# sanje2v/DualSuperResLearningForSemSeg

Measured on AMD Instinct MI355X. Metric: stage-3 train images/sec at 256x512->512x1024, higher is better.
Workload: dtype f32; 1 GPU; DSRL stage 3 (ResNet-101 OS16 + ASPP + SSSR/SISR decoders + FA loss), full train step, random-init weights, 256x512 input -> 512x1024 logits; global_batch=8, per_gpu_batch=8, parallelism=dp1, optimizer=SGD m0.9 wd5e-4 lr0.006

## Files before the change

dualsuperreslearningforsemseg_amd/_lib.py:

```python
import ctypes as C
import os

import torch

_HERE = os.path.dirname(os.path.abspath(__file__))
LIB_PATH = os.path.join(_HERE, 'libdsrl_hip.so')

fp = C.c_void_p
i32 = C.c_int
i64 = C.c_int64
u64 = C.c_uint64
u32 = C.c_uint32
f32 = C.c_float
sz = C.c_size_t
stream_t = C.c_void_p

_conv_shape = [i32] * 10


class WgradProblem(C.Structure):
    _fields_ = [('x', C.c_void_p), ('dy', C.c_void_p), ('dw', C.c_void_p)] + [(n, C.c_int32) for n in
                ('ldx', 'lddy', 'N', 'H', 'W', 'C', 'K', 'R', 'S', 'stride', 'pad', 'dil')] + [('x_amax', C.c_void_p), ('dy_amax', C.c_void_p)]


PROTOTYPES = {
    'dsrl_version': (i32, []),
    'dsrl_last_error': (C.c_char_p, []),
    'dsrl_device_check': (i32, [C.POINTER(i32)]),
    'dsrl_conv2d_fwd_workspace_bytes': (sz, _conv_shape),
    'dsrl_conv2d_fwd': (i32, [fp, i32, fp, fp, fp, i32] + _conv_shape + [fp, sz, stream_t]),
    'dsrl_conv2d_fwd_stats_parts': (i32, _conv_shape),
    'dsrl_conv2d_fwd_stats': (i32, [fp, i32, fp, fp, fp, i32] + _conv_shape + [fp, sz, fp, i32, stream_t]),
    'dsrl_conv2d_dgrad_workspace_bytes': (sz, _conv_shape),
    'dsrl_conv2d_transposed_filter_floats': (sz, [i32] * 4),
    'dsrl_conv2d_transpose_filter': (i32, [fp, fp, i32, i32, i32, i32, stream_t]),
    'dsrl_conv2d_transpose_filters_batched': (i32, [fp, i32, i64, stream_t]),
    'dsrl_conv2d_filters_amax_segment_floats': (i32, []),
    'dsrl_conv2d_filters_amax_batched': (i32, [fp, i64, stream_t]),
    'dsrl_conv2d_dgrad': (i32, [fp, i32, fp, fp, fp, i32] + _conv_shape + [fp, sz, stream_t]),
    'dsrl_conv2d_dgrad_stats_parts': (i32, _conv_shape),
    'dsrl_conv2d_dgrad_bnstats': (i32, [fp, i32, fp, fp, fp, i32] + _conv_shape + [fp, sz, fp, i32, fp, i32, fp, fp, i32, fp, i32, i32, stream_t]),
    'dsrl_conv2d_dgrad_accumulate': (i32, [fp, i32, fp, fp, fp, i32] + _conv_shape + [fp, sz, stream_t]),
    'dsrl_conv2d_wgrad_workspace_bytes': (sz, _conv_shape),
    'dsrl_conv2d_wgrad': (i32, [fp, i32, fp, i32, fp] + _conv_shape + [fp, sz, stream_t]),
    'dsrl_conv2d_wgrad_group_table_bytes': (sz, [i32]),
    'dsrl_conv2d_wgrad_group_workspace_bytes': (sz, [fp, i32]),
    'dsrl_conv2d_wgrad_group_plan': (i32, [fp, i32, fp, sz, fp, fp, sz]),
    'dsrl_conv2d_wgrad_group_launch': (i32, [fp, fp, stream_t]),
    'dsrl_amax': (i32, [fp, i32, i64, i32, fp, stream_t]),
    'dsrl_conv2d_fwd_amax': (i32, [fp, i32, fp, fp, fp, fp, fp, fp, i32] + _conv_shape + [fp, sz, fp, i32, stream_t]),
    'dsrl_conv2d_dgrad_amax': (i32, [fp, i32, fp, fp, fp, fp, fp, fp, i32] + _conv_shape + [fp, sz, fp, i32, fp, i32, fp, fp, i32, fp, i32, i32, stream_t]),
    'dsrl_conv2d_split_filters_batched': (i32, [fp, i32, i64, stream_t]),
    'dsrl_planes_lo_offset': (sz, [i64]),
    'dsrl_planes_bytes': (sz, [i64, i32]),
    'dsrl_split_planes': (i32, [fp, i32, i64, i32, fp, fp, i32, stream_t]),
    'dsrl_conv2d_filter_planes_batched': (i32, [fp, i32, i64, stream_t]),
    'dsrl_conv2d_fwd_planes': (i32, [fp, i32, fp, fp, fp, fp, fp, fp, fp, fp, i32] + _conv_shape + [fp, sz, fp, i32, stream_t]),
    'dsrl_conv2d_dgrad_planes': (i32, [fp, i32, fp, fp, fp, fp, fp, fp, fp, fp, i32] + _conv_shape + [fp, sz, fp, i32, fp, i32, fp, fp, i32, fp, i32, i32, stream_t]),
    'dsrl_conv2d_dgrad_planes_drop': (i32, [fp, i32, fp, fp, fp, fp, fp, fp, fp, fp, i32] + _conv_shape + [fp, sz, fp, i32, fp, i32, fp, fp, i32, f32, fp, i32, i32, stream_t]),
    'dsrl_conv2d_wgrad_amax': (i32, [fp, i32, fp, fp, i32, fp, fp] + _conv_shape + [fp, sz, stream_t]),
    'dsrl_conv_precision': (i32, [i32]),
    'dsrl_conv2d_inbounds_macs': (i64, _conv_shape),
    'dsrl_conv2d_rowfold_fwd_workspace_bytes': (sz, [i32] * 9),
    'dsrl_conv2d_rowfold_fwd': (i32, [fp, i32, fp, fp, fp, i32] + [i32] * 9 + [i64, fp, sz, stream_t]),
    'dsrl_conv2d_rowfold_wgrad_workspace_bytes': (sz, [i32] * 9),
    'dsrl_conv2d_rowfold_wgrad': (i32, [fp, i32, fp, i32, fp] + [i32] * 9 + [i64, fp, sz, stream_t]),
    'dsrl_pad_image_nhwc': (i32, [fp, i64, i64, i64, i64, fp] + [i32] * 9 + [stream_t]),
    'dsrl_colsum_workspace_bytes': (sz, [i64, i32]),
    'dsrl_colsum': (i32, [fp, i32, i64, i32, fp, fp, sz, stream_t]),
    'dsrl_bn_workspace_bytes': (sz, [i64, i32]),
    'dsrl_bn_stats_floats': (sz, [i32, i32, i32]),
    'dsrl_bn_stats': (i32, [fp, i32, i64, i32, f32, f32, fp, fp, fp, fp, fp, sz, stream_t]),
    'dsrl_bn_invstd_from_var': (i32, [fp, i32, f32, fp, stream_t]),
    'dsrl_bn_apply': (i32, [fp, i32, fp, i32, i64, i32, fp, fp, fp, fp, fp, i32, i32, f32, u64, u32, fp, stream_t]),
    'dsrl_bn_fused_max_blocks': (i32, [i32]),
    'dsrl_bn_fused_barrier_timeouts': (i32, [C.POINTER(i64)]),
    'dsrl_bn_train_fwd_from_stats': (i32, [fp, i32, fp, i32, i64, i32, f32, f32, fp, fp, fp, fp, fp, fp, fp, i32, i32, f32, u64, u32, fp, i32, fp, stream_t]),
    'dsrl_bn_train_fwd': (i32, [fp, i32, fp, i32, i64, i32, f32, f32, fp, fp, fp, fp, fp, fp, fp, i32, i32, f32, u64, u32, fp, sz, fp, stream_t]),
    'dsrl_bn_bwd': (i32, [fp, i32, fp, i32, fp, i32, fp, i32, fp, i32, i64, i32, fp, fp, fp, fp, fp, i32, f32, i32, fp, sz, fp, stream_t]),
    'dsrl_bn_bwd_from_stats': (i32, [fp, i32, fp, i32, fp, i32, fp, i32, fp, i32, i64, i32, fp, fp, fp, fp, fp, i32, i32, fp, i32, fp, stream_t]),
    'dsrl_bn_bwd_from_stats_drop': (i32, [fp, i32, fp, i32, fp, i32, fp, i32, fp, i32, i64, i32, fp, fp, fp, fp, fp, i32, f32, i32, fp, i32, fp, stream_t]),
    'dsrl_bn_bwd_from_stats_res_parts': (i32, [i64, i32, i32]),
    'dsrl_bn_bwd_from_stats_res': (i32, [fp, i32, fp, i32, fp, i32, fp, i32, fp, i32, i64, i32, fp, fp, fp, fp, fp, i32, f32, i32, fp, i32, fp, fp, i32, fp, fp, fp, i32, stream_t]),
    'dsrl_dropout_fwd': (i32, [fp, i32, fp, i32, i64, i32, f32, u64, u32, stream_t]),
    'dsrl_dropout_bwd': (i32, [fp, i32, fp, i32, i64, i32, f32, u64, u32, stream_t]),
    'dsrl_bilinear_ac_fwd': (i32, [fp, i32, fp, i32, i32, i32, i32, i32, i32, i32, stream_t]),
    'dsrl_bilinear_ac_bwd_workspace_bytes': (sz, [i32] * 6),
    'dsrl_bilinear_ac_bwd': (i32, [fp, i32, fp, i32, i32, i32, i32, i32, i32, i32, fp, sz, stream_t]),
    'dsrl_global_avgpool_fwd': (i32, [fp, i32, fp, i32, i32, i32, stream_t]),
    'dsrl_global_avgpool_bwd': (i32, [fp, fp, i32, i32, i32, i32, stream_t]),
    'dsrl_maxpool3x3s2_fwd': (i32, [fp, fp, fp, i32, i32, i32, i32, stream_t]),
    'dsrl_maxpool3x3s2_bwd': (i32, [fp, fp, fp, i32, i32, i32, i32, stream_t]),
    'dsrl_convt2x2_fwd': (i32, [fp, fp, fp, fp, i32, i32, i32, i32, i32, stream_t]),
    'dsrl_convt2x2_bwd_workspace_bytes': (sz, [i32] * 5),
    'dsrl_convt2x2_bwd': (i32, [fp, fp, fp, fp, fp, fp, i32, i32, i32, i32, i32, fp, sz, stream_t]),
    'dsrl_convt2x2_fwd_ce_supported': (i32, [fp, fp, i32, i32, i32, i32, i32]),
    'dsrl_convt2x2_fwd_ce_workspace_bytes': (sz, [i32, i32, i32]),
    'dsrl_convt2x2_fwd_ce': (i32, [fp, fp, fp, fp, i32, i32, i32, i32, i32, fp, i32, fp, fp, fp, sz, stream_t]),
    'dsrl_convt2x2_bwd_ce_supported': (i32, [fp, fp, fp, i32, i32, i32, i32, i32]),
    'dsrl_convt2x2_bwd_ce': (i32, [fp, fp, fp, fp, i32, fp, fp, fp, i32, fp, fp, fp, i32, i32, i32, i32, i32, fp, sz, stream_t]),
    'dsrl_pixel_shuffle_fwd': (i32, [fp, fp, i32, i32, i32, i32, i32, stream_t]),
    'dsrl_pixel_shuffle_bwd': (i32, [fp, fp, i32, i32, i32, i32, i32, stream_t]),
    'dsrl_pointwise_strided_fwd': (i32, [fp, fp, fp, i32, i32, i32, i32, i32, stream_t]),
    'dsrl_pointwise_strided_bwd_workspace_bytes': (sz, [i32] * 5),
    'dsrl_pointwise_strided_bwd': (i32, [fp, fp, fp, fp, fp, i32, i32, i32, i32, i32, i32, fp, sz, stream_t]),
    'dsrl_copy2d': (i32, [fp, i32, fp, i32, i64, i32, stream_t]),
    'dsrl_cat_channels_supported': (i32, [fp, fp, fp, i32, fp, i32, i64]),
    'dsrl_cat_channels': (i32, [fp, fp, fp, i32, fp, i32, i64, fp, stream_t]),
    'dsrl_nchw_to_nhwc': (i32, [fp, fp, i32, i32, i32, i32, i32, stream_t]),
    'dsrl_ce_workspace_bytes': (sz, [i64]),
    'dsrl_ce_fwd': (i32, [fp, i32, fp, i64, i32, i32, fp, fp, sz, stream_t]),
    'dsrl_ce_bwd': (i32, [fp, i32, fp, i64, i32, i32, fp, fp, fp, i32, stream_t]),
    'dsrl_mse_workspace_bytes': (sz, [i64]),
    'dsrl_mse_fwd': (i32, [fp, fp, i64, fp, fp, sz, stream_t]),
    'dsrl_mse_bwd': (i32, [fp, fp, i64, fp, fp, stream_t]),
    'dsrl_ce_fused_workspace_bytes': (sz, [i64]),
    'dsrl_ce_fused': (i32, [fp, i32, fp, i64, i32, i32, fp, i32, fp, fp, fp, sz, stream_t]),
    'dsrl_mse_fused': (i32, [fp, fp, i64, f32, fp, fp, fp, fp, sz, stream_t]),
    'dsrl_loss_mix': (i32, [fp, fp, fp, f32, f32, fp, fp, stream_t]),
    'dsrl_fa_saved_floats': (sz, [i32] * 5),
    'dsrl_fa_workspace_bytes': (sz, [i32] * 5),
    'dsrl_fa_fwd': (i32, [fp, fp, i32, i32, i32, i32, i64, i64, i64, i64, i32, i32, fp, fp, fp, sz, stream_t]),
    'dsrl_fa_bwd': (i32, [fp, fp, i32, i32, i32, i32, i64, i64, i64, i64, i32, i32, fp, fp, fp, fp, fp, sz, stream_t]),
    'dsrl_seg_metrics': (i32, [fp, i32, fp, i64, i32, i32, fp, stream_t]),
    'dsrl_sssr_tail_predict_supported': (i32, [i32] * 6),
    'dsrl_sssr_tail_predict_workspace_bytes': (sz, [i32] * 3),
    'dsrl_sssr_tail_predict': (i32, [fp, i32] + [i32] * 6 + [fp] * 9 + [i32, fp, fp, fp, fp, sz, stream_t]),
    'dsrl_fingerprint_segment_words': (i32, []),
    'dsrl_fingerprint_segments': (i32, [fp, i64, fp, fp, fp, i32, stream_t]),
    'dsrl_class_map_visualize': (i32, [fp, fp, fp, fp, fp, i32, i32, i32, i32, C.c_double, stream_t]),
    'dsrl_prepare_batch': (i32, [fp, fp, fp, C.POINTER(f32), C.POINTER(f32), fp, fp, fp, i32, i32, i32, i32, i32, stream_t]),
    'dsrl_augment_geometry': (i32, [fp, fp, fp, fp, fp, fp, i32, i32, i32, stream_t]),
    'dsrl_prepare_batch_augmented': (i32, [fp, fp, fp, C.POINTER(f32), C.POINTER(f32), fp, fp, fp, i32, i32, i32, i32, i32, fp, stream_t]),
    'dsrl_sgd_step': (i32, [fp, fp, fp, i64, f32, f32, f32, f32, stream_t]),
    'dsrl_sgd_step_dev': (i32, [fp, fp, fp, i64, fp, stream_t]),
    'dsrl_sgd_step_dev_segments': (i32, [fp, fp, fp, fp, i64, fp, stream_t]),
    'dsrl_nan_check': (i32, [fp, i64, fp, stream_t]),
    'dsrl_rng_bind_device_key': (i32, [fp]),
    'dsrl_rng_advance_key': (i32, [fp, stream_t]),
    'dsrl_prof_enable': (i32, [i32]),
    'dsrl_prof_read': (i32, [i32, C.POINTER(i64), C.POINTER(C.c_double), C.POINTER(C.c_double)]),
    'dsrl_prof_read_bytes': (i32, [i32, C.POINTER(C.c_double)]),
    'dsrl_prof_kernel_name': (C.c_char_p, [i32]),
}

_lib = None


class DsrlHipError(RuntimeError):
    pass


def load():
    global _lib
    if _lib is not None:
        return _lib
    if not os.path.isfile(LIB_PATH):
        raise DsrlHipError(f'{LIB_PATH} not found: build it with `python -c "import __graft_entry__ as g; g.build()"` '
                           f'or `make -C {os.path.join(_HERE, "csrc")}` - there is no fallback path')
    lib = C.CDLL(LIB_PATH)
# ... 35 lines not shown
```

dualsuperreslearningforsemseg_amd/csrc/bn.hip:

```cpp
#include "common.h"
#include <algorithm>
#include <initializer_list>
#include <atomic>
#include <mutex>
#include <stdlib.h>

struct SeedArg { unsigned long long value; const unsigned long long* dev; };

namespace dsrl {

constexpr int kMaxRowBlocks = 256;

static int row_blocks(int64_t P) { return (int)std::max<int64_t>(1, std::min<int64_t>(kMaxRowBlocks, ceil_div(P, 32))); }

__global__ __launch_bounds__(256) void bn_partial_kernel(const float* __restrict__ x, int ld, long long P, int C, long long rows_per_block,
                                                          float* __restrict__ part, int nbx) {
    __shared__ float sh[3][256];
    const ChanMap m = chan_map(C, blockIdx.y);
    const long long row0 = blockIdx.x * rows_per_block, row1 = min(P, row0 + rows_per_block);
    float n = 0.f, s1 = 0.f, s2 = 0.f, k0 = 0.f;
    if (m.c >= 0) {
        long long p = row0 + m.slot;
        if (p < row1) k0 = x[p * ld + m.c];
#pragma unroll 4
// ... 613 lines not shown
        if (p < row1) {
            const float4 dv = LD4(dy, p, lddy, q), xv = LD4(x, p, ldx, q);
            float4 yv = make_float4(1.f, 1.f, 1.f, 1.f);
            if (need_y) yv = LD4(y, p, ldy, q);
            g[i] = make_float4(masked_grad(dv.x, yv.x, relu, drop_p, ks), masked_grad(dv.y, yv.y, relu, drop_p, ks),
                               masked_grad(dv.z, yv.z, relu, drop_p, ks), masked_grad(dv.w, yv.w, relu, drop_p, ks));
            xh[i] = make_float4((xv.x - mu[0]) * is[0], (xv.y - mu[1]) * is[1], (xv.z - mu[2]) * is[2], (xv.w - mu[3]) * is[3]);
            sg[0] += g[i].x; sgx[0] += g[i].x * xh[i].x; sg[1] += g[i].y; sgx[1] += g[i].y * xh[i].y;
            sg[2] += g[i].z; sgx[2] += g[i].z * xh[i].z; sg[3] += g[i].w; sgx[3] += g[i].w * xh[i].w;
            if (dres) ST4(dres, p, lddr, q) = g[i];
        } else {
            g[i] = make_float4(0.f, 0.f, 0.f, 0.f); xh[i] = g[i];
        }
    }
#pragma unroll
    for (int sft = 8; sft < 64; sft <<= 1) {
#pragma unroll
        for (int j = 0; j < 4; ++j) { sg[j] += __shfl_xor(sg[j], sft); sgx[j] += __shfl_xor(sgx[j], sft); }
    }
    if ((tid & 63) < 8) {
#pragma unroll
        for (int j = 0; j < 4; ++j) { shw[wave][0][j][l8] = sg[j]; shw[wave][1][j][l8] = sgx[j]; }
    }
    __syncthreads();
    if (tid < 32) {
        const int j = tid & 3, c8 = tid >> 2;
        float a = 0.f, b = 0.f;
#pragma unroll
        for (int w = 0; w < kFusedNW; ++w) { a += shw[w][0][j][c8]; b += shw[w][1][j][c8]; }
        const long long o = (long long)slab * C + grp * 32 + tid;
        st_agent(part + o, a); st_agent(part + (long long)slabs * C + o, b);
    }
    const bool arrived = grid_barrier(gridDim.x);
    {
        const int ch = tid & 31, k = tid >> 5;
        const float* pa = part + grp * 32 + ch;
        const float* pb = pa + (long long)slabs * C;
        double a = 0, b = 0;
        for (int base = k; base < slabs; base += 4 * kFusedNS) {
            float va[4], vb[4];
#pragma unroll
            for (int u = 0; u < 4; ++u) {
                const int sl = min(base + kFusedNS * u, slabs - 1);
                va[u] = ld_agent(pa + (long long)sl * C); vb[u] = ld_agent(pb + (long long)sl * C);
            }
#pragma unroll
            for (int u = 0; u < 4; ++u)
                if (base + kFusedNS * u < slabs) { a += va[u]; b += vb[u]; }
        }
        shm[k][0][ch] = a; shm[k][1][ch] = b;
    }
    __syncthreads();
    if (tid < 32) {
        double a = 0, b = 0;
#pragma unroll
        for (int k = 0; k < kFusedNS; ++k) { a += shm[k][0][tid]; b += shm[k][1][tid]; }
        const float inv_n = 1.f / (float)P;
        fin[0][tid] = !arrived ? __builtin_nanf("") : (training ? (float)a * inv_n : 0.f); fin[1][tid] = training ? (float)b * inv_n : 0.f;
        if (slab == 0) {
            const int c = grp * 32 + tid;
            if (dbeta) dbeta[c] = (float)a;
            if (dgamma) dgamma[c] = (float)b;
        }
    }
    __syncthreads();
    float gi[4], mb[4], mg[4];
#pragma unroll
    for (int j = 0; j < 4; ++j) { gi[j] = gamma[4 * q + j] * is[j]; mb[j] = fin[0][4 * l8 + j]; mg[j] = fin[1][4 * l8 + j]; }
    unsigned am = 0u;
#pragma unroll
    for (int i = 0; i < kFusedMaxPasses; ++i) {
        const int p = row0 + rr + kFusedRL * i;
        if (p >= row1) continue;
        const float4 d = make_float4(gi[0] * (g[i].x - mb[0] - xh[i].x * mg[0]), gi[1] * (g[i].y - mb[1] - xh[i].y * mg[1]),
                                     gi[2] * (g[i].z - mb[2] - xh[i].z * mg[2]), gi[3] * (g[i].w - mb[3] - xh[i].w * mg[3]));
        ST4(dx, p, lddx, q) = d;
        am = abs_bits4(am, d.x, d.y, d.z, d.w);
    }
    amax_publish(am, dx_amax);
}


constexpr int kMergeRows = 4;
template <int THREADS>
__global__ __launch_bounds__(THREADS) void bn_stats_apply_kernel(const float* __restrict__ x, int ldx, float* __restrict__ y, int ldy, int P, int C,
                                                              int groups, int rows_per_slab, float eps, float momentum,
                                                              float* __restrict__ mean_out, float* __restrict__ invstd_out, float* __restrict__ rm, float* __restrict__ rv,
                                                              const float* __restrict__ gamma, const float* __restrict__ beta,
                                                              const float* __restrict__ res, int ldr, int relu, float drop_p, SeedArg seed_arg, unsigned rng_stream,
                                                              const float* __restrict__ part, int nparts, unsigned* __restrict__ y_amax) {
    const unsigned long long seed = seed_arg.dev ? *seed_arg.dev : seed_arg.value;
    constexpr int KG = THREADS / 32, RP = THREADS / 8;
    __shared__ double shm[KG][3][32];
    __shared__ float fin[2][32];
    const int grp = blockIdx.x % groups, slab = blockIdx.x / groups;
    const int tid = threadIdx.x, l8 = tid & 7, rr = tid >> 3;
    const int q = grp * 8 + l8;
    const int row0 = slab * rows_per_slab, row1 = min(P, row0 + rows_per_slab), p0 = row0 + rr;
    float4 xv0 = make_float4(0.f, 0.f, 0.f, 0.f), rv0 = xv0;
    if (p0 < row1) {
        xv0 = LD4(x, p0, ldx, q);
        if (res) rv0 = LD4(res, p0, ldr, q);
    }
    float gmv[4], btv[4];
#pragma unroll
    for (int j = 0; j < 4; ++j) { gmv[j] = gamma[4 * q + j]; btv[j] = beta[4 * q + j]; }
    {
        const int ch = tid & 31, k = tid >> 5;
        const float* pn = part + grp * 32 + ch;
        const float* pm_ = pn + (long long)nparts * C;
        const float* pq = pn + 2ll * nparts * C;
        const float mref = pm_[0];
        double N = 0, S = 0, T = 0;
        struct Batch { float n[kMergeRows], m[kMergeRows], q[kMergeRows]; };
        auto fetch = [&](int base, Batch& b) {
#pragma unroll
            for (int u = 0; u < kMergeRows; ++u) {
                const int sl = min(base + KG * u, nparts - 1);
                b.n[u] = pn[(long long)sl * C]; b.m[u] = pm_[(long long)sl * C]; b.q[u] = pq[(long long)sl * C];
            }
        };
        auto sum = [&](int base, const Batch& b) {
#pragma unroll
            for (int u = 0; u < kMergeRows; ++u) {
                const double nb = base + KG * u < nparts ? (double)b.n[u] : 0.0, d = (double)b.m[u] - (double)mref;
                N += nb; S += nb * d; T += (base + KG * u < nparts ? (double)b.q[u] : 0.0) + nb * d * d;
            }
        };
        Batch b0, b1;
        fetch(k, b0);
        for (int base = k; base < nparts; base += 2 * KG * kMergeRows) {
            const int mid = base + KG * kMergeRows;
            if (mid < nparts) fetch(mid, b1);
            sum(base, b0);
            if (mid < nparts) {
                if (mid + KG * kMergeRows < nparts) fetch(mid + KG * kMergeRows, b0);
                sum(mid, b1);
            }
        }
        shm[k][0][ch] = N; shm[k][1][ch] = S; shm[k][2][ch] = T;
        if (k == 0) fin[0][ch] = mref;
    }
    __syncthreads();
    if (tid < 32) {
        double N = 0, S = 0, T = 0;
#pragma unroll
        for (int k = 0; k < KG; ++k) { N += shm[k][0][tid]; S += shm[k][1][tid]; T += shm[k][2][tid]; }
        const double mu = N > 0 ? (double)fin[0][tid] + S / N : 0.0;
        const double Q = N > 0 ? fmax(T - S * S / N, 0.0) : 0.0;
        const double var = N > 0 ? Q / N : 0.0;
        const float is = (float)(1.0 / sqrt(var + (double)eps));
        fin[0][tid] = (float)mu; fin[1][tid] = is;
        if (slab == 0) {
            const int c = grp * 32 + tid;
            mean_out[c] = (float)mu; invstd_out[c] = is;
            if (rm) rm[c] = (float)((1.0 - momentum) * rm[c] + momentum * mu);
            if (rv) rv[c] = (float)((1.0 - momentum) * rv[c] + momentum * (N > 1 ? Q / (N - 1) : var));
        }
    }
    __syncthreads();
    float sc[4], sf[4];
#pragma unroll
    for (int j = 0; j < 4; ++j) { sc[j] = gmv[j] * fin[1][4 * l8 + j]; sf[j] = btv[j] - fin[0][4 * l8 + j] * sc[j]; }
    const float ks = drop_p > 0.f ? 1.f / (1.f - drop_p) : 1.f;
    unsigned am = 0u;
    auto row = [&](int p, const float4 xv, const float4 r) {
        float v[4] = {fmaf(xv.x, sc[0], sf[0]), fmaf(xv.y, sc[1], sf[1]), fmaf(xv.z, sc[2], sf[2]), fmaf(xv.w, sc[3], sf[3])};
        if (res) { v[0] += r.x; v[1] += r.y; v[2] += r.z; v[3] += r.w; }
        if (relu) {
#pragma unroll
            for (int j = 0; j < 4; ++j) v[j] = fmaxf(v[j], 0.f);
        }
        if (drop_p > 0.f) {
            const unsigned long long e = (unsigned long long)p * C + 4ull * q;
            unsigned r4[4];
            philox4x32_10((unsigned)(e >> 2), (unsigned)(e >> 34), rng_stream, 0u, (unsigned)seed, (unsigned)(seed >> 32), r4);
#pragma unroll
            for (int j = 0; j < 4; ++j) v[j] = ((float)(r4[j] >> 8) * 5.9604644775390625e-08f >= drop_p) ? v[j] * ks : 0.f;
        }
        ST4(y, p, ldy, q) = make_float4(v[0], v[1], v[2], v[3]);
        am = abs_bits4(am, v[0], v[1], v[2], v[3]);
    };
    if (p0 < row1) row(p0, xv0, rv0);
#pragma unroll 4
    for (int p = p0 + RP; p < row1; p += RP) {
        const float4 xv = LD4(x, p, ldx, q);
        float4 r = xv;
        if (res) r = LD4(res, p, ldr, q);
        row(p, xv, r);
    }
    amax_publish(am, y_amax);
}


constexpr int kStatsReduced = 32;
__global__ __launch_bounds__(256) void bn_stats_reduce_kernel(const float* __restrict__ part, int nparts, int C, float* __restrict__ out) {
    __shared__ double shm[8][3][32];
    __shared__ float ref[32];
    const int grp = blockIdx.x, rrow = blockIdx.y, tid = threadIdx.x, ch = tid & 31, k = tid >> 5;
    const int per = (nparts + kStatsReduced - 1) / kStatsReduced, p0 = rrow * per, p1 = min(nparts, p0 + per);
    const float* pn = part + grp * 32 + ch;
    const float* pm_ = pn + (long long)nparts * C;
    const float* pq = pn + 2ll * nparts * C;
    const float mref = p0 < p1 ? pm_[(long long)p0 * C] : 0.f;
    double N = 0, S = 0, T = 0;
    for (int base = p0 + k; base < p1; base += 32) {
        float vn[4], vm[4], vq[4];
#pragma unroll
        for (int u = 0; u < 4; ++u) {
            const int sl = min(base + 8 * u, p1 - 1);
            vn[u] = pn[(long long)sl * C]; vm[u] = pm_[(long long)sl * C]; vq[u] = pq[(long long)sl * C];
        }
#pragma unroll
        for (int u = 0; u < 4; ++u)
            if (base + 8 * u < p1) {
                const double nb = (double)vn[u], d = (double)vm[u] - (double)mref;
                N += nb; S += nb * d; T += (double)vq[u] + nb * d * d;
            }
    }
    shm[k][0][ch] = N; shm[k][1][ch] = S; shm[k][2][ch] = T;
    if (k == 0) ref[ch] = mref;
    __syncthreads();
    if (tid < 32) {
        N = S = T = 0;
#pragma unroll
        for (int kk = 0; kk < 8; ++kk) { N += shm[kk][0][tid]; S += shm[kk][1][tid]; T += shm[kk][2][tid]; }
        const double mu = N > 0 ? (double)ref[tid] + S / N : 0.0, Q = N > 0 ? fmax(T - S * S / N, 0.0) : 0.0;
        float* o = out + (long long)rrow * C + grp * 32 + tid;
        o[0] = (float)N; o[(long long)kStatsReduced * C] = (float)mu; o[2ll * kStatsReduced * C] = (float)Q;
    }
}
__global__ __launch_bounds__(256) void bn_bwd_stats_reduce_kernel(const float* __restrict__ part, int nparts, int C, float* __restrict__ out) {
    __shared__ double shm[8][2][32];
    const int grp = blockIdx.x, rrow = blockIdx.y, tid = threadIdx.x, ch = tid & 31, k = tid >> 5;
    const int per = (nparts + kStatsReduced - 1) / kStatsReduced, p0 = rrow * per, p1 = min(nparts, p0 + per);
    const float* pa = part + grp * 32 + ch;
    const float* pb = pa + (long long)nparts * C;
    double a = 0, b = 0;
    for (int base = p0 + k; base < p1; base += 32) {
        float va[4], vb[4];
#pragma unroll
        for (int u = 0; u < 4; ++u) {
            const int sl = min(base + 8 * u, p1 - 1);
            va[u] = pa[(long long)sl * C]; vb[u] = pb[(long long)sl * C];
        }
#pragma unroll
        for (int u = 0; u < 4; ++u)
            if (base + 8 * u < p1) { a += (double)va[u]; b += (double)vb[u]; }
    }
    shm[k][0][ch] = a; shm[k][1][ch] = b;
    __syncthreads();
    if (tid < 32) {
        a = b = 0;
#pragma unroll
        for (int kk = 0; kk < 8; ++kk) { a += shm[kk][0][tid]; b += shm[kk][1][tid]; }
        float* o = out + (long long)rrow * C + grp * 32 + tid;
        o[0] = (float)a; o[(long long)kStatsReduced * C] = (float)b;
    }
}

struct BnRes2 { const float* x; int ldx; const float* mean; const float* invstd; float* part; int nslabs; };
template <int THREADS, bool RES2 = false>
__global__ __launch_bounds__(THREADS) void bn_bwd_stats_apply_kernel(const float* __restrict__ x, int ldx, const float* __restrict__ y, int ldy,
                                                                  const float* __restrict__ dy, int lddy, float* __restrict__ dx, int lddx,
                                                                  float* __restrict__ dres, int lddr, int P, int C, int groups, int rows_per_slab,
                                                                  const float* __restrict__ mean, const float* __restrict__ invstd, const float* __restrict__ gamma,
                                                                  float* __restrict__ dgamma, float* __restrict__ dbeta, int relu, int training,
                                                                  const float* __restrict__ part, int nparts, unsigned* __restrict__ dx_amax, float ks, const BnRes2 r2) {
    constexpr int KG = THREADS / 32, RP = THREADS / 8;
    __shared__ double shm[KG][2][32];
    __shared__ float fin[2][32];
    const int grp = blockIdx.x % groups, slab = blockIdx.x / groups;
    const int tid = threadIdx.x, l8 = tid & 7, rr = tid >> 3;
    const int q = grp * 8 + l8;
    const int row0 = slab * rows_per_slab, row1 = min(P, row0 + rows_per_slab), p0 = row0 + rr;
    float4 dv0 = make_float4(0.f, 0.f, 0.f, 0.f), xv0 = dv0, yv0 = make_float4(1.f, 1.f, 1.f, 1.f), x2v0 = dv0;
    if (p0 < row1) {
        dv0 = LD4(dy, p0, lddy, q); xv0 = LD4(x, p0, ldx, q);
        if (relu) yv0 = LD4(y, p0, ldy, q);
        if constexpr (RES2) x2v0 = LD4(r2.x, p0, r2.ldx, q);
    }
    float mu2[4] = {0.f, 0.f, 0.f, 0.f}, is2[4] = {0.f, 0.f, 0.f, 0.f}, sg2[4] = {0.f, 0.f, 0.f, 0.f}, sgx2[4] = {0.f, 0.f, 0.f, 0.f};
    if constexpr (RES2) {
#pragma unroll
        for (int j = 0; j < 4; ++j) { mu2[j] = r2.mean[4 * q + j]; is2[j] = r2.invstd[4 * q + j]; }
    }
    float mu[4], is[4], gi[4];
#pragma unroll
    for (int j = 0; j < 4; ++j) { mu[j] = mean[4 * q + j]; is[j] = invstd[4 * q + j]; gi[j] = gamma[4 * q + j]; }
    {
        const int ch = tid & 31, k = tid >> 5;
        const float* pa = part + grp * 32 + ch;
        const float* pb = pa + (long long)nparts * C;
        double a = 0, b = 0;
        struct Batch { float a[kMergeRows], b[kMergeRows]; };
        auto fetch = [&](int base, Batch& t) {
#pragma unroll
            for (int u = 0; u < kMergeRows; ++u) {
                const int sl = min(base + KG * u, nparts - 1);
                t.a[u] = pa[(long long)sl * C]; t.b[u] = pb[(long long)sl * C];
            }
        };
        auto sum = [&](int base, const Batch& t) {
#pragma unroll
            for (int u = 0; u < kMergeRows; ++u)
                if (base + KG * u < nparts) { a += t.a[u]; b += t.b[u]; }
        };
        Batch b0, b1;
        fetch(k, b0);
        for (int base = k; base < nparts; base += 2 * KG * kMergeRows) {
            const int mid = base + KG * kMergeRows;
            if (mid < nparts) fetch(mid, b1);
            sum(base, b0);
            if (mid < nparts) {
                if (mid + KG * kMergeRows < nparts) fetch(mid + KG * kMergeRows, b0);
                sum(mid, b1);
            }
        }
        shm[k][0][ch] = a; shm[k][1][ch] = b;
    }
    __syncthreads();
    if (tid < 32) {
        double a = 0, b = 0;
#pragma unroll
        for (int k = 0; k < KG; ++k) { a += shm[k][0][tid]; b += shm[k][1][tid]; }
        const float inv_n = 1.f / (float)P;
        fin[0][tid] = training ? (float)a * inv_n : 0.f; fin[1][tid] = training ? (float)b * inv_n : 0.f;
        if (slab == 0) {
            const int c = grp * 32 + tid;
            if (dbeta) dbeta[c] = (float)a;
            if (dgamma) dgamma[c] = (float)b;
        }
    }
    __syncthreads();
    float mb[4], mg[4];
#pragma unroll
    for (int j = 0; j < 4; ++j) { gi[j] *= is[j]; mb[j] = fin[0][4 * l8 + j]; mg[j] = fin[1][4 * l8 + j]; }
    unsigned am = 0u;
    auto row = [&](int p, const float4 dv, const float4 xv, const float4 yv, const float4 x2v) {
        const float g0 = masked_grad(dv.x, yv.x, relu, 0.f, ks), g1 = masked_grad(dv.y, yv.y, relu, 0.f, ks);
        const float g2 = masked_grad(dv.z, yv.z, relu, 0.f, ks), g3 = masked_grad(dv.w, yv.w, relu, 0.f, ks);
        const float4 d = make_float4(gi[0] * (g0 - mb[0] - (xv.x - mu[0]) * is[0] * mg[0]), gi[1] * (g1 - mb[1] - (xv.y - mu[1]) * is[1] * mg[1]),
                                     gi[2] * (g2 - mb[2] - (xv.z - mu[2]) * is[2] * mg[2]), gi[3] * (g3 - mb[3] - (xv.w - mu[3]) * is[3] * mg[3]));
        ST4(dx, p, lddx, q) = d;
        am = abs_bits4(am, d.x, d.y, d.z, d.w);
        if (dres) ST4(dres, p, lddr, q) = make_float4(g0, g1, g2, g3);
        if constexpr (RES2) {
            sg2[0] += g0; sgx2[0] += g0 * ((x2v.x - mu2[0]) * is2[0]);
            sg2[1] += g1; sgx2[1] += g1 * ((x2v.y - mu2[1]) * is2[1]);
            sg2[2] += g2; sgx2[2] += g2 * ((x2v.z - mu2[2]) * is2[2]);
            sg2[3] += g3; sgx2[3] += g3 * ((x2v.w - mu2[3]) * is2[3]);
        }
    };
    if (p0 < row1) row(p0, dv0, xv0, yv0, x2v0);
#pragma unroll 2
    for (int p = p0 + RP; p < row1; p += RP) {
        const float4 dv = LD4(dy, p, lddy, q), xv = LD4(x, p, ldx, q);
        float4 yv = make_float4(1.f, 1.f, 1.f, 1.f);
        if (relu) yv = LD4(y, p, ldy, q);
        float4 x2v = xv;
        if constexpr (RES2) x2v = LD4(r2.x, p, r2.ldx, q);
        row(p, dv, xv, yv, x2v);
    }
    if constexpr (RES2) {
        __shared__ float r2s[THREADS / 64][2][32];
#pragma unroll
        for (int sft = 8; sft < 64; sft <<= 1)
#pragma unroll
            for (int j = 0; j < 4; ++j) { sg2[j] += __shfl_xor(sg2[j], sft); sgx2[j] += __shfl_xor(sgx2[j], sft); }
        if ((tid & 63) < 8) {
#pragma unroll
            for (int j = 0; j < 4; ++j) { r2s[tid >> 6][0][4 * l8 + j] = sg2[j]; r2s[tid >> 6][1][4 * l8 + j] = sgx2[j]; }
        }
        __syncthreads();
        if (tid < 64) {
            const int v = tid >> 5, c = tid & 31;
            float t = 0.f;
#pragma unroll
            for (int w = 0; w < THREADS / 64; ++w) t += r2s[w][v][c];
            r2.part[((long long)v * r2.nslabs + slab) * C + grp * 32 + c] = t;
        }
    }
    amax_publish(am, dx_amax);
}

constexpr int kFlatThreads = 512;
__device__ inline void flat_reduce(float (*sh)[4 * kFlatThreads], float (*sh2)[kFlatThreads], int nv, int C, int T, int phase0, float* out) {
    const int t = threadIdx.x, G = kFlatThreads / C, c = t % C, r = t / C;
    __syncthreads();
    if (r < G) {
        const int e0 = (c - phase0 + C) % C;
        for (int v = 0; v < nv; ++v) {
            float a = 0.f;
            for (int e = e0 + C * r; e < 4 * T; e += C * G) a += sh[v][e];
            sh2[v][r * C + c] = a;
        }
    }
    __syncthreads();
    const int G2 = G > 16 ? 16 : G;
    if (G > 16 && r < 16) {
        for (int v = 0; v < nv; ++v) {
            float a = 0.f;
            for (int q = r; q < G; q += 16) a += sh2[v][q * C + c];
            sh[v][r * C + c] = a;
        }
    }
    __syncthreads();
    if (t < C)
        for (int v = 0; v < nv; ++v) {
            float a = 0.f;
            for (int q = 0; q < G2; ++q) a += (G > 16 ? sh[v][q * C + t] : sh2[v][q * C + t]);
            out[v] = a;
        }
}
__global__ __launch_bounds__(kFlatThreads) void bn_partial_flat_kernel(const float* __restrict__ x, long long total4, long long P, int C, int T,
                                                                      long long per_block4, float* __restrict__ part, int nbx) {
    __shared__ float sh[3][4 * kFlatThreads];
    __shared__ float sh2[3][kFlatThreads];
    const int t = threadIdx.x;
    const long long b0 = min(total4, blockIdx.x * per_block4), b1 = min(total4, b0 + per_block4);
    const long long r0 = min(P - 1, (4 * b0) / C);
    const int phase0 = (int)((4 * b0) % C);
    float n = 0.f, s1[4] = {0.f, 0.f, 0.f, 0.f}, s2[4] = {0.f, 0.f, 0.f, 0.f};
    if (t < T) {
        float k0[4];
#pragma unroll
        for (int k = 0; k < 4; ++k) k0[k] = x[r0 * C + (phase0 + 4 * t + k) % C];
        const float4* x4 = reinterpret_cast<const float4*>(x);
#pragma unroll 4
        for (long long f = b0 + t; f < b1; f += T) {
            const float4 v = x4[f];
            const float d0 = v.x - k0[0], d1 = v.y - k0[1], d2 = v.z - k0[2], d3 = v.w - k0[3];
            s1[0] += d0; s2[0] += d0 * d0; s1[1] += d1; s2[1] += d1 * d1; s1[2] += d2; s2[2] += d2 * d2; s1[3] += d3; s2[3] += d3 * d3;
            n += 1.f;
        }
    }
#pragma unroll
    for (int k = 0; k < 4; ++k) { sh[0][4 * t + k] = n; sh[1][4 * t + k] = s1[k]; sh[2][4 * t + k] = s2[k]; }
    float tot[3];
    flat_reduce(sh, sh2, 3, C, T, phase0, tot);
    if (t < C) {
        float mean = 0.f, m2 = 0.f;
// ... 198 lines not shown
    if (int e = bind_stream_device(st)) return e;
    const int nbx = row_blocks(P);
    const long long rpb = ceil_div(P, nbx);
    if (vec4_ok(C, {ldx}, {x}))
        hipLaunchKernelGGL(bn_partial4_kernel, dim3(nbx, (unsigned)ceil_div(C / 4, 256)), dim3(256), 0, st, x, ldx, (long long)P, C, rpb, (float*)ws, nbx);
    else if (const int T = flat_stride(C, P, {ldx}, {x}))
        hipLaunchKernelGGL(bn_partial_flat_kernel, dim3(nbx), dim3(kFlatThreads), 0, st, x, (long long)(P * C / 4), (long long)P, C, T,
                           (long long)ceil_div(P * C / 4, (int64_t)nbx), (float*)ws, nbx);
    else
        hipLaunchKernelGGL(bn_partial_kernel, dim3(nbx, (unsigned)ceil_div(C, 256)), dim3(256), 0, st, x, ldx, (long long)P, C, rpb, (float*)ws, nbx);
    if (int e = launch_status("bn_partial_kernel")) return e;
    hipLaunchKernelGGL(bn_finalize_kernel, dim3((unsigned)ceil_div(C, 8)), dim3(256), 0, st, (const float*)ws, nbx, C, eps, momentum, mean, invstd, running_mean, running_var);
    return launch_status("bn_finalize_kernel");
}

extern "C" int dsrl_bn_invstd_from_var(const float* running_var, int C, float eps, float* invstd, dsrl_stream_t stream) {
    DSRL_REQUIRE(running_var && invstd && C > 0, DSRL_E_BADARG, "bn_invstd_from_var: bad arguments");
    hipStream_t st = (hipStream_t)stream;
    if (int e = bind_stream_device(st)) return e;
    hipLaunchKernelGGL(invstd_from_var_kernel, dim3((unsigned)ceil_div(C, 256)), dim3(256), 0, st, running_var, C, eps, invstd);
    return launch_status("invstd_from_var_kernel");
}

extern "C" int dsrl_bn_apply(const float* x, int ldx, float* y, int ldy, int64_t P, int C, const float* mean, const float* invstd,
                             const float* gamma, const float* beta, const float* residual, int ldr, int relu, float drop_p,
                             uint64_t seed, uint32_t rng_stream, uint32_t* y_amax, dsrl_stream_t stream) {
    DSRL_REQUIRE(x && y && mean && invstd && gamma && beta && P > 0 && C > 0 && ldx >= C && ldy >= C, DSRL_E_BADARG, "bn_apply: bad arguments");
    DSRL_REQUIRE(drop_p >= 0.f && drop_p < 1.f, DSRL_E_BADARG, "bn_apply: dropout p=%f outside [0,1)", drop_p);
    hipStream_t st = (hipStream_t)stream;
    if (int e = bind_stream_device(st)) return e;
    if (vec4_ok(C, {ldx, ldy, residual ? ldr : 0}, {x, y, residual}))
        hipLaunchKernelGGL(bn_apply4_kernel, apply_grid4(P, C), dim3(256), 0, st, x, ldx, y, ldy, (long long)P, C, mean, invstd, gamma, beta, residual, ldr,
                           relu, drop_p, seed_arg(seed), (unsigned)rng_stream, y_amax);
    else if (const int T = flat_stride(C, P, {ldx, ldy, residual ? ldr : C}, {x, y, residual}))
        hipLaunchKernelGGL(bn_apply_flat_kernel, dim3((unsigned)std::max<int64_t>(1, std::min<int64_t>(2048, ceil_div(P * C / 4, (int64_t)T * 2)))), dim3(kFlatThreads), 0, st,
                           x, y, (long long)(P * C / 4), C, T, mean, invstd, gamma, beta, residual, relu, drop_p, seed_arg(seed), (unsigned)rng_stream, y_amax);
    else
        hipLaunchKernelGGL(bn_apply_kernel, apply_grid(P, C), dim3(256), 0, st, x, ldx, y, ldy, (long long)P, C, mean, invstd, gamma, beta, residual, ldr,
                           relu, drop_p, seed_arg(seed), (unsigned)rng_stream, y_amax);
    return launch_status("bn_apply_kernel");
}

extern "C" int dsrl_bn_fused_max_blocks(int max_blocks) {
    const int prev = g_fused_max_blocks.load();
    if (max_blocks >= -1) g_fused_max_blocks.store(max_blocks);
    return prev;
}

extern "C" int dsrl_bn_fused_barrier_timeouts(int64_t* count) {
    DSRL_REQUIRE(count, DSRL_E_BADARG, "bn_fused_barrier_timeouts: null pointer");
    unsigned int v = 0;
    if (hipMemcpyFromSymbol(&v, HIP_SYMBOL(g_grid_timeouts), sizeof(v)) != hipSuccess) return launch_status("hipMemcpyFromSymbol(g_grid_timeouts)");
    *count = (int64_t)v;
    static unsigned int seen[64] = {0};
    int dev = 0;
    if (hipGetDevice(&dev) != hipSuccess || dev < 0 || dev >= 64) dev = 0;
    if (v != seen[dev]) {
        const unsigned int zero = 0u;
        if (hipMemcpyToSymbol(HIP_SYMBOL(g_grid_count), &zero, sizeof(zero)) != hipSuccess) return launch_status("hipMemcpyToSymbol(g_grid_count)");
        seen[dev] = v;
    }
    return DSRL_OK;
}

extern "C" int dsrl_bn_train_fwd(const float* x, int ldx, float* y, int ldy, int64_t P, int C, float eps, float momentum, float* mean, float* invstd,
                                 float* running_mean, float* running_var, const float* gamma, const float* beta, const float* residual, int ldr,
                                 int relu, float drop_p, uint64_t seed, uint32_t rng_stream, void* ws, size_t ws_bytes, uint32_t* y_amax, dsrl_stream_t stream) {
    DSRL_REQUIRE(x && y && mean && invstd && gamma && beta && ws && P > 0 && C > 0 && ldx >= C && ldy >= C, DSRL_E_BADARG, "bn_train_fwd: bad arguments");
    DSRL_REQUIRE(drop_p >= 0.f && drop_p < 1.f, DSRL_E_BADARG, "bn_train_fwd: dropout p=%f outside [0,1)", drop_p);
    DSRL_REQUIRE(ws_bytes >= dsrl_bn_workspace_bytes(P, C), DSRL_E_WORKSPACE, "bn_train_fwd: workspace too small");
    const FusedPlan f = fused_plan(P, C);
    if (f.ok && vec4_ok(C, {ldx, ldy, residual ? ldr : 0}, {x, y, residual}) && bind_stream_device((hipStream_t)stream) == DSRL_OK &&
        fused_stream_ok((hipStream_t)stream)) {
        hipStream_t st = (hipStream_t)stream;
        hipLaunchKernelGGL(bn_fused_fwd_kernel, dim3(f.blocks), dim3(kFusedThreads), 0, st, x, ldx, y, ldy, (int)P, C, f.groups, f.slabs, f.rows_per_slab, eps, momentum,
                           mean, invstd, running_mean, running_var, gamma, beta, residual, ldr, relu, drop_p, seed_arg(seed), (unsigned)rng_stream,
                           (float*)ws, y_amax);
        return launch_status("bn_fused_fwd_kernel");
    }
    if (int e = dsrl_bn_stats(x, ldx, P, C, eps, momentum, mean, invstd, running_mean, running_var, ws, ws_bytes, stream)) return e;
    return dsrl_bn_apply(x, ldx, y, ldy, P, C, mean, invstd, gamma, beta, residual, ldr, relu, drop_p, seed, rng_stream, y_amax, stream);
}

extern "C" int dsrl_bn_train_fwd_from_stats(const float* x, int ldx, float* y, int ldy, int64_t P, int C, float eps, float momentum, float* mean, float* invstd,
                                            float* running_mean, float* running_var, const float* gamma, const float* beta, const float* residual, int ldr,
                                            int relu, float drop_p, uint64_t seed, uint32_t rng_stream, float* stats, int stats_parts, uint32_t* y_amax,
                                            dsrl_stream_t stream) {
    DSRL_REQUIRE(x && y && mean && invstd && gamma && beta && stats && P > 0 && P < (1ll << 31) && C > 0 && ldx >= C && ldy >= C, DSRL_E_BADARG, "bn_train_fwd_from_stats: bad arguments");
    DSRL_REQUIRE(stats_parts > 0 && stats_parts <= 4096, DSRL_E_BADARG, "bn_train_fwd_from_stats: %d row blocks of partials (1..4096)", stats_parts);
    DSRL_REQUIRE(C % 32 == 0 && vec4_ok(C, {ldx, ldy, residual ? ldr : 0}, {x, y, residual}), DSRL_E_UNSUPPORTED,
                 "bn_train_fwd_from_stats: C (%d) must be a multiple of 32, strides multiples of 4, pointers 16-byte aligned", C);
    DSRL_REQUIRE(drop_p >= 0.f && drop_p < 1.f, DSRL_E_BADARG, "bn_train_fwd_from_stats: dropout p=%f outside [0,1)", drop_p);
    hipStream_t st = (hipStream_t)stream;
    if (int e = bind_stream_device(st)) return e;
    const int groups = C / 32;
    if (stats_parts > 256) {
        float* red = stats + 3ll * stats_parts * C;
        hipLaunchKernelGGL(bn_stats_reduce_kernel, dim3((unsigned)groups, kStatsReduced), dim3(256), 0, st, (const float*)stats, stats_parts, C, red);
        if (int e = launch_status("bn_stats_reduce_kernel")) return e;
        stats = red; stats_parts = kStatsReduced;
    }
    const int T = stats_apply_threads(P, C, stats_parts), rows_per_slab = stats_apply_rows(P, groups, T), slabs = (int)ceil_div(P, (int64_t)rows_per_slab);
    auto go = [&](auto kern) {
        hipLaunchKernelGGL(kern, dim3((unsigned)(groups * slabs)), dim3(T), 0, st, x, ldx, y, ldy, (int)P, C, groups, rows_per_slab, eps, momentum,
                           mean, invstd, running_mean, running_var, gamma, beta, residual, ldr, relu, drop_p, seed_arg(seed), (unsigned)rng_stream, stats, stats_parts, y_amax);
    };
    if (T == 1024) go(bn_stats_apply_kernel<1024>); else if (T == 512) go(bn_stats_apply_kernel<512>); else go(bn_stats_apply_kernel<256>);
    return launch_status("bn_stats_apply_kernel");
}

extern "C" int dsrl_bn_bwd(const float* x, int ldx, const float* y, int ldy, const float* dy, int lddy, float* dx, int lddx,
                           float* dresidual, int lddr, int64_t P, int C, const float* mean, const float* invstd, const float* gamma,
                           float* dgamma, float* dbeta, int relu, float drop_p, int training, void* ws, size_t ws_bytes, uint32_t* dx_amax, dsrl_stream_t stream) {
    DSRL_REQUIRE(x && dy && dx && mean && invstd && gamma && ws && P > 0 && C > 0, DSRL_E_BADARG, "bn_bwd: bad arguments");
    DSRL_REQUIRE(y || !(relu || drop_p > 0.f), DSRL_E_BADARG, "bn_bwd: forward output needed for the relu/dropout mask");
    DSRL_REQUIRE(ws_bytes >= dsrl_bn_workspace_bytes(P, C), DSRL_E_WORKSPACE, "bn_bwd: workspace too small");
    hipStream_t st = (hipStream_t)stream;
    if (int e = bind_stream_device(st)) return e;
    const bool v4 = vec4_ok(C, {ldx, y ? ldy : 0, lddy, lddx, dresidual ? lddr : 0}, {x, y, dy, dx, dresidual});
    const FusedPlan f = fused_plan(P, C);
    if (f.ok && v4 && fused_stream_ok(st)) {
        hipLaunchKernelGGL(bn_fused_bwd_kernel, dim3(f.blocks), dim3(kFusedThreads), 0, st, x, ldx, y, ldy, dy, lddy, dx, lddx, dresidual, lddr, (int)P, C,
                           f.groups, f.slabs, f.rows_per_slab, mean, invstd, gamma, dgamma, dbeta, relu, drop_p, training, (float*)ws, dx_amax);
        return launch_status("bn_fused_bwd_kernel");
    }
    const int nbx = row_blocks(P);
    const long long rpb = ceil_div(P, nbx);
    float* part = (float*)ws;
    float* sums = part + 3ll * nbx * C;
    if (v4)
        hipLaunchKernelGGL(bn_bwd_partial4_kernel, dim3(nbx, (unsigned)ceil_div(C / 4, 256)), dim3(256), 0, st, x, ldx, y, ldy, dy, lddy, (long long)P, C, rpb,
                           mean, invstd, relu, drop_p, part, nbx);
    else if (const int T = flat_stride(C, P, {ldx, y ? ldy : C, lddy}, {x, y, dy}))
        hipLaunchKernelGGL(bn_bwd_partial_flat_kernel, dim3(nbx), dim3(kFlatThreads), 0, st, x, y, dy, (long long)(P * C / 4), C, T,
                           (long long)ceil_div(P * C / 4, (int64_t)nbx), mean, invstd, relu, drop_p, part, nbx);
    else
        hipLaunchKernelGGL(bn_bwd_partial_kernel, dim3(nbx, (unsigned)ceil_div(C, 256)), dim3(256), 0, st, x, ldx, y, ldy, dy, lddy, (long long)P, C, rpb,
                           mean, invstd, relu, drop_p, part, nbx);
    if (int e = launch_status("bn_bwd_partial_kernel")) return e;
    hipLaunchKernelGGL(bn_bwd_finalize_kernel, dim3((unsigned)ceil_div(C, 8)), dim3(256), 0, st, (const float*)part, nbx, C, sums, dgamma, dbeta);
    if (int e = launch_status("bn_bwd_finalize_kernel")) return e;
    if (v4)
        hipLaunchKernelGGL(bn_bwd_apply4_kernel, apply_grid4(P, C), dim3(256), 0, st, x, ldx, y, ldy, dy, lddy, dx, lddx, dresidual, lddr, (long long)P, C,
                           mean, invstd, gamma, (const float*)sums, relu, drop_p, training, dx_amax);
    else
        hipLaunchKernelGGL(bn_bwd_apply_kernel, apply_grid(P, C), dim3(256), 0, st, x, ldx, y, ldy, dy, lddy, dx, lddx, dresidual, lddr, (long long)P, C,
                           mean, invstd, gamma, (const float*)sums, relu, drop_p, training, dx_amax);
    return launch_status("bn_bwd_apply_kernel");
}

extern "C" int dsrl_bn_bwd_from_stats(const float* x, int ldx, const float* y, int ldy, const float* dy, int lddy, float* dx, int lddx,
                                      float* dresidual, int lddr, int64_t P, int C, const float* mean, const float* invstd, const float* gamma,
                                      float* dgamma, float* dbeta, int relu, int training, float* stats, int stats_parts, uint32_t* dx_amax,
                                      dsrl_stream_t stream) {
    return dsrl_bn_bwd_from_stats_drop(x, ldx, y, ldy, dy, lddy, dx, lddx, dresidual, lddr, P, C, mean, invstd, gamma, dgamma, dbeta, relu, 0.f, training, stats, stats_parts,
                                       dx_amax, stream);
}
static int bwd_from_stats_slabs(int64_t P, int C, int stats_parts) {
    const int parts = stats_parts > 256 ? kStatsReduced : stats_parts, groups = C / 32, T = stats_apply_threads(P, C, parts);
    return (int)ceil_div(P, (int64_t)stats_apply_rows(P, groups, T));
}
extern "C" int dsrl_bn_bwd_from_stats_res_parts(int64_t P, int C, int stats_parts) {
    return (P > 0 && P < (1ll << 31) && C > 0 && C % 32 == 0 && stats_parts > 0 && stats_parts <= 4096) ? bwd_from_stats_slabs(P, C, stats_parts) : 0;
}
static int bn_bwd_from_stats_impl(const float* x, int ldx, const float* y, int ldy, const float* dy, int lddy, float* dx, int lddx,
                                  float* dresidual, int lddr, int64_t P, int C, const float* mean, const float* invstd, const float* gamma,
                                  float* dgamma, float* dbeta, int relu, float drop_p, int training, float* stats, int stats_parts, uint32_t* dx_amax,
                                  dsrl_stream_t stream, const BnRes2* res2);
extern "C" int dsrl_bn_bwd_from_stats_drop(const float* x, int ldx, const float* y, int ldy, const float* dy, int lddy, float* dx, int lddx,
                                           float* dresidual, int lddr, int64_t P, int C, const float* mean, const float* invstd, const float* gamma,
                                           float* dgamma, float* dbeta, int relu, float drop_p, int training, float* stats, int stats_parts, uint32_t* dx_amax,
                                           dsrl_stream_t stream) {
    return bn_bwd_from_stats_impl(x, ldx, y, ldy, dy, lddy, dx, lddx, dresidual, lddr, P, C, mean, invstd, gamma, dgamma, dbeta, relu, drop_p, training, stats, stats_parts,
                                  dx_amax, stream, nullptr);
}
extern "C" int dsrl_bn_bwd_from_stats_res(const float* x, int ldx, const float* y, int ldy, const float* dy, int lddy, float* dx, int lddx,
                                          float* dresidual, int lddr, int64_t P, int C, const float* mean, const float* invstd, const float* gamma,
                                          float* dgamma, float* dbeta, int relu, float drop_p, int training, float* stats, int stats_parts, uint32_t* dx_amax,
                                          const float* res_x, int res_ldx, const float* res_mean, const float* res_invstd, float* res_stats, int res_parts,
                                          dsrl_stream_t stream) {
    DSRL_REQUIRE(dresidual && res_x && res_mean && res_invstd && res_stats && res_ldx >= C && res_ldx % 4 == 0 && ((uintptr_t)res_x % 16) == 0, DSRL_E_BADARG,
                 "bn_bwd_from_stats_res: the residual branch's input / statistics / partials buffer are required (stride a multiple of 4, 16-byte aligned)");
    DSRL_REQUIRE(res_parts > 0 && res_parts == dsrl_bn_bwd_from_stats_res_parts(P, C, stats_parts), DSRL_E_BADARG,
                 "bn_bwd_from_stats_res: this launch writes %d row blocks of sums, the caller expects %d (dsrl_bn_bwd_from_stats_res_parts)",
                 dsrl_bn_bwd_from_stats_res_parts(P, C, stats_parts), res_parts);
    const BnRes2 r2{res_x, res_ldx, res_mean, res_invstd, res_stats, res_parts};
    return bn_bwd_from_stats_impl(x, ldx, y, ldy, dy, lddy, dx, lddx, dresidual, lddr, P, C, mean, invstd, gamma, dgamma, dbeta, relu, drop_p, training, stats, stats_parts,
                                  dx_amax, stream, &r2);
}
static int bn_bwd_from_stats_impl(const float* x, int ldx, const float* y, int ldy, const float* dy, int lddy, float* dx, int lddx,
                                  float* dresidual, int lddr, int64_t P, int C, const float* mean, const float* invstd, const float* gamma,
                                  float* dgamma, float* dbeta, int relu, float drop_p, int training, float* stats, int stats_parts, uint32_t* dx_amax,
                                  dsrl_stream_t stream, const BnRes2* res2) {
    DSRL_REQUIRE(drop_p >= 0.f && drop_p < 1.f && (drop_p == 0.f || relu), DSRL_E_BADARG, "bn_bwd_from_stats_drop: dropout p=%f needs the ReLU mask (y > 0)", drop_p);
    const float ks = drop_p > 0.f ? 1.f / (1.f - drop_p) : 1.f;
    DSRL_REQUIRE(x && dy && dx && mean && invstd && gamma && stats && P > 0 && P < (1ll << 31) && C > 0, DSRL_E_BADARG, "bn_bwd_from_stats: bad arguments");
    DSRL_REQUIRE(y || !relu, DSRL_E_BADARG, "bn_bwd_from_stats: forward output needed for the relu mask");
    DSRL_REQUIRE(stats_parts > 0 && stats_parts <= 4096, DSRL_E_BADARG, "bn_bwd_from_stats: %d row blocks of partials (1..4096)", stats_parts);
    DSRL_REQUIRE(C % 32 == 0 && vec4_ok(C, {ldx, y ? ldy : 0, lddy, lddx, dresidual ? lddr : 0}, {x, y, dy, dx, dresidual}), DSRL_E_UNSUPPORTED,
                 "bn_bwd_from_stats: C (%d) must be a multiple of 32, strides multiples of 4, pointers 16-byte aligned", C);
    hipStream_t st = (hipStream_t)stream;
    if (int e = bind_stream_device(st)) return e;
    const int groups = C / 32;
    if (stats_parts > 256) {
        float* red = stats + 2ll * stats_parts * C;
        hipLaunchKernelGGL(bn_bwd_stats_reduce_kernel, dim3((unsigned)groups, kStatsReduced), dim3(256), 0, st, (const float*)stats, stats_parts, C, red);
        if (int e = launch_status("bn_bwd_stats_reduce_kernel")) return e;
        stats = red; stats_parts = kStatsReduced;
    }
    const int T = stats_apply_threads(P, C, stats_parts), rows_per_slab = stats_apply_rows(P, groups, T), slabs = (int)ceil_div(P, (int64_t)rows_per_slab);
    BnRes2 r2{};
    if (res2) { r2 = *res2; DSRL_REQUIRE(r2.nslabs == slabs, DSRL_E_BADARG, "bn_bwd_from_stats_res: %d slabs launched, %d expected", slabs, r2.nslabs); }
    auto go = [&](auto kern) {
        hipLaunchKernelGGL(kern, dim3((unsigned)(groups * slabs)), dim3(T), 0, st, x, ldx, y, ldy, dy, lddy, dx, lddx, dresidual, lddr, (int)P, C,
                           groups, rows_per_slab, mean, invstd, gamma, dgamma, dbeta, relu, training, stats, stats_parts, dx_amax, ks, r2);
    };
    if (res2) { if (T == 1024) go(bn_bwd_stats_apply_kernel<1024, true>); else if (T == 512) go(bn_bwd_stats_apply_kernel<512, true>); else go(bn_bwd_stats_apply_kernel<256, true>); }
    else if (T == 1024) go(bn_bwd_stats_apply_kernel<1024>); else if (T == 512) go(bn_bwd_stats_apply_kernel<512>); else go(bn_bwd_stats_apply_kernel<256>);
    return launch_status("bn_bwd_stats_apply_kernel");
}

extern "C" int dsrl_colsum(const float* x, int ld, int64_t P, int C, float* out, void* ws, size_t ws_bytes, dsrl_stream_t stream) {
    DSRL_REQUIRE(x && out && ws && P > 0 && C > 0 && ld >= C, DSRL_E_BADARG, "colsum: bad arguments");
    DSRL_REQUIRE(ws_bytes >= dsrl_colsum_workspace_bytes(P, C), DSRL_E_WORKSPACE, "colsum: workspace too small");
    hipStream_t st = (hipStream_t)stream;
    if (int e = bind_stream_device(st)) return e;
    const int nbx = row_blocks(P);
    if (vec4_ok(C, {ld}, {x}))
        hipLaunchKernelGGL(colsum_partial4_kernel, dim3(nbx, (unsigned)ceil_div(C / 4, 256)), dim3(256), 0, st, x, ld, (long long)P, C, (long long)ceil_div(P, nbx), (float*)ws);
    else
        hipLaunchKernelGGL(colsum_partial_kernel, dim3(nbx, (unsigned)ceil_div(C, 256)), dim3(256), 0, st, x, ld, (long long)P, C, (long long)ceil_div(P, nbx), (float*)ws);
    if (int e = launch_status("colsum_partial_kernel")) return e;
    hipLaunchKernelGGL(colsum_finalize_kernel, dim3((unsigned)ceil_div(C, 32)), dim3(256), 0, st, (const float*)ws, nbx, C, out);
    return launch_status("colsum_finalize_kernel");
}

__global__ void rng_advance_kernel(unsigned long long* state) {
    if (threadIdx.x == 0 && blockIdx.x == 0) { state[1] += 1ull; state[0] = state[2] * 1000003ull + state[1]; }
}
extern "C" int dsrl_rng_bind_device_key(const uint64_t* dev_key) {
    int dev = 0;
    if (hipGetDevice(&dev) != hipSuccess || dev < 0 || dev >= 64) { set_error("rng_bind_device_key: no current HIP device"); (void)hipGetLastError(); return DSRL_E_LAUNCH; }
    g_rng_dev_key[dev].store((const unsigned long long*)dev_key);
    return DSRL_OK;
}
extern "C" int dsrl_rng_advance_key(uint64_t* state, dsrl_stream_t stream) {
    DSRL_REQUIRE(state && ((uintptr_t)state % 8) == 0, DSRL_E_BADARG, "rng_advance_key: state must be three 8-byte aligned 64-bit words on the device");
    hipStream_t st = (hipStream_t)stream;
    if (int e = bind_stream_device(st)) return e;
    hipLaunchKernelGGL(rng_advance_kernel, dim3(1), dim3(64), 0, st, (unsigned long long*)state);
    return launch_status("rng_advance_kernel");
}

namespace dsrl {
__global__ __launch_bounds__(256) void dropout_flat4_kernel(const float4* __restrict__ x, float4* __restrict__ y, unsigned total4, float p_drop, SeedArg seed_arg,
                                                             unsigned rng_stream) {
    const unsigned long long seed = seed_arg.dev ? *seed_arg.dev : seed_arg.value;
    const float ks = 1.f / (1.f - p_drop);
    for (unsigned i = blockIdx.x * 256u + threadIdx.x; i < total4; i += gridDim.x * 256u) {
        const float4 v = x[i];
        unsigned r[4];
        philox4x32_10(i, 0u, rng_stream, 0u, (unsigned)seed, (unsigned)(seed >> 32), r);
        float4 o;
        o.x = ((float)(r[0] >> 8) * 5.9604644775390625e-08f >= p_drop) ? v.x * ks : 0.f;
        o.y = ((float)(r[1] >> 8) * 5.9604644775390625e-08f >= p_drop) ? v.y * ks : 0.f;
        o.z = ((float)(r[2] >> 8) * 5.9604644775390625e-08f >= p_drop) ? v.z * ks : 0.f;
        o.w = ((float)(r[3] >> 8) * 5.9604644775390625e-08f >= p_drop) ? v.w * ks : 0.f;
        y[i] = o;
    }
}
}

static int dropout_common(const float* x, int ldx, float* y, int ldy, int64_t P, int C, float p, uint64_t seed, uint32_t rng_stream, dsrl_stream_t stream) {
    DSRL_REQUIRE(x && y && P > 0 && C > 0 && p >= 0.f && p < 1.f, DSRL_E_BADARG, "dropout: bad arguments");
    hipStream_t st = (hipStream_t)stream;
    if (int e = bind_stream_device(st)) return e;
    const long long total = (long long)P * C;
    if (ldx == C && ldy == C && total % 4 == 0 && total / 4 < (1ll << 32) && ((uintptr_t)x % 16) == 0 && ((uintptr_t)y % 16) == 0) {
        hipLaunchKernelGGL(dropout_flat4_kernel, dim3((unsigned)std::min<long long>(ceil_div(total / 4, 256), 8192)), dim3(256), 0, st, reinterpret_cast<const float4*>(x),
                           reinterpret_cast<float4*>(y), (unsigned)(total / 4), p, seed_arg(seed), (unsigned)rng_stream);
        return launch_status("dropout_flat4_kernel");
    }
// ... 11 lines not shown
```

dualsuperreslearningforsemseg_amd/csrc/conv_common.h:

```cpp
#pragma once
#include "common.h"

namespace dsrl {

using f32x16 = __attribute__((ext_vector_type(16))) float;
using bf16x8 = __attribute__((ext_vector_type(8))) __bf16;
using bf16x4 = __attribute__((ext_vector_type(4))) __bf16;
using f16x8 = __attribute__((ext_vector_type(8))) _Float16;
using f16x4 = __attribute__((ext_vector_type(4))) _Float16;

template <bool F16> struct Plane;
template <> struct Plane<false> {
    using v4 = bf16x4; using v8 = bf16x8;
    static __device__ __forceinline__ v4 cvt(const float* r) { return v4{(__bf16)r[0], (__bf16)r[1], (__bf16)r[2], (__bf16)r[3]}; }
    static __device__ __forceinline__ void residual(float* r, v4 t) {
#pragma unroll
        for (int e = 0; e < 4; ++e) r[e] -= (float)t[e];
    }
    static __device__ __forceinline__ f32x16 mfma(v8 a, v8 b, f32x16 c) { return __builtin_amdgcn_mfma_f32_32x32x16_bf16(a, b, c, 0, 0, 0); }
};
__device__ __forceinline__ float f16_resid_lo(unsigned t, float r) { float d; asm("v_fma_mix_f32 %0, %1, -1.0, %2 op_sel:[0,0,0] op_sel_hi:[1,0,0]" : "=v"(d) : "v"(t), "v"(r)); return d; }
__device__ __forceinline__ float f16_resid_hi(unsigned t, float r) { float d; asm("v_fma_mix_f32 %0, %1, -1.0, %2 op_sel:[1,0,0] op_sel_hi:[1,0,0]" : "=v"(d) : "v"(t), "v"(r)); return d; }
template <> struct Plane<true> {
    using v4 = f16x4; using v8 = f16x8;
    using f32x4 = __attribute__((ext_vector_type(4))) float;
    using u32x2 = __attribute__((ext_vector_type(2))) unsigned;
    static __device__ __forceinline__ v4 cvt(const float* r) { return __builtin_convertvector((f32x4{r[0], r[1], r[2], r[3]}), v4); }
    static __device__ __forceinline__ void residual(float* r, v4 t) {
        const u32x2 u = __builtin_bit_cast(u32x2, t);
        r[0] = f16_resid_lo(u.x, r[0]); r[1] = f16_resid_hi(u.x, r[1]); r[2] = f16_resid_lo(u.y, r[2]); r[3] = f16_resid_hi(u.y, r[3]);
    }
    static __device__ __forceinline__ f32x16 mfma(v8 a, v8 b, f32x16 c) { return __builtin_amdgcn_mfma_f32_32x32x16_f16(a, b, c, 0, 0, 0); }
};
__device__ __forceinline__ int amax_shift_of(unsigned fetched) {
    const unsigned u = amax_reduce(fetched);
    int ex = (int)((u >> 23) & 0xffu);
    if (ex == 0) ex = 1;
    return 14 - (ex - 127);
}
__device__ __forceinline__ int amax_shift(const unsigned* p) { return amax_shift_of(amax_fetch(p)); }

__device__ __forceinline__ int fast_div(int n, unsigned m, unsigned s) {
    const int q = (int)(__umulhi((unsigned)n, m) >> (s & 31u));
    return s == 255u ? n : q;
}

struct ConvArgs {
    const float* x; const float* w; const float* bias; float* y;
    int ldx, ldy;
    int N, H, W, C;
    int K;
    int R, S, Ho, Wo;
    int stride, pad, dil;
    int M;
    int cchunks;
    int splits;
    long long slab;
    unsigned x_bytes, w_bytes, y_bytes;
    int mtiles, ntiles, xcd_remap;
    int kg;
    int accumulate;
    float* stats;
    const float* bn_x; const float* bn_y; const float* bn_mean; const float* bn_invstd; float* bstats;
    int bn_ldx, bn_ldy, bn_relu;
    float bn_gscale;
    int bn_fast;
    int par, Hh, Wh, pbm;
    const unsigned* amax_a; const unsigned* amax_b;
    int w_split;
    unsigned mHW, sHW, mW, sW, mNT, sNT;
    unsigned a_lo, b_lo;
    int planes;
    float* coop_slab; unsigned* tickets;
};
constexpr int kCoopMaxTiles = (kAmaxShardStride - 1) * kAmaxShards;
__host__ __device__ inline int coop_ticket_word(int t) { return kAmaxShardStride * (t / (kAmaxShardStride - 1)) + 1 + t % (kAmaxShardStride - 1); }
__device__ __forceinline__ int dgrad_pix(const ConvArgs& a, int m) {
    const int t = m / a.pbm, p2 = a.par * a.par, c = t % p2, j = (t / p2) * a.pbm + (m - t * a.pbm);
    const int hw = a.Hh * a.Wh, n = j / hw, r = j - n * hw, hh = r / a.Wh, wh = r - hh * a.Wh;
    const int ph = c / a.par, pw = c - ph * a.par;
    return (n * a.Ho + hh * a.par + ph) * a.Wo + wh * a.par + pw;
}

__device__ inline int xcd_contiguous(int bid, int n) {
    const int q = n / kNumXCD, r = n % kNumXCD, xcd = bid % kNumXCD, local = bid / kNumXCD;
    return (xcd < r ? xcd * (q + 1) : r * (q + 1) + (xcd - r) * q) + local;
}

using u32x4 = __attribute__((ext_vector_type(4))) unsigned int;
constexpr unsigned kOOB = 0x80000000u;
__device__ inline float4 buf_load4(__amdgpu_buffer_rsrc_t r, unsigned off) {
    const u32x4 v = __builtin_amdgcn_raw_buffer_load_b128(r, (int)off, 0, 0);
    return make_float4(__uint_as_float(v.x), __uint_as_float(v.y), __uint_as_float(v.z), __uint_as_float(v.w));
}

struct WgradArgs {
    const float* x; const float* dy; float* dw;
    int ldx, lddy;
    int N, H, W, C, K, R, S, Ho, Wo, stride, pad, dil;
    long long P;
    unsigned x_bytes, dy_bytes;
    int ctiles;
    int psplits;
    long long slab;
    int taps[64]; int ntaps;
    int xcd_remap;
    int kctiles;
    unsigned mHW, sHW, mW, sW;
    int kg;
    int nblocks;
    float* dw_final;
    int rblocks;
    const unsigned* amax_dy; const unsigned* amax_x;
    int no_ident;
};

bool wgrad3_eligible(int N, int H, int W, int C, int K, int R, int S, int stride, int pad, int dil, int npl, bool f16);
void wgrad3_tile(int& bm, int& bn);
int launch_wgrad3(const WgradArgs& a, int npl, hipStream_t st);
int launch_wgrad3_group(const WgradArgs* table, const int* starts, int nprob, int grid, int npl, int dil, hipStream_t st);

bool planes_cfg_supported(int cfg, int kg);
int launch_planes_igemm(const ConvArgs& a, int cfg, bool dgrad, hipStream_t st);
bool sk_supported(int cfg, int kg, int npl, bool f16, bool w_split);
size_t sk_lds_bytes();
int launch_sk_igemm(const ConvArgs& a, bool dgrad, bool str1, int npl, hipStream_t st);
__host__ __device__ inline long long planes_lo_offset(long long elems) { return (elems * 2 + 255) / 256 * 256; }

}
```

dualsuperreslearningforsemseg_amd/csrc/conv_igemm.hip:

```cpp
#include "common.h"
#include "conv_common.h"
#include <algorithm>
#include <atomic>
#include <stdlib.h>
#include <string.h>
#include <mutex>
#include <vector>

namespace dsrl {

static std::atomic<int> g_conv_precision{-1};
constexpr int BK = 32;
constexpr int LDS_LD = 36;

template <int MR, int NR, int WGM, int WGN, bool DGRAD, int MINW = 2, bool = false>
__global__ __launch_bounds__(256, MINW) void conv_igemm_f32_kernel(const ConvArgs a) {
    constexpr int BM = 32 * MR * WGM, BN = 32 * NR * WGN;
    constexpr int A_IT = BM / 32, B_IT = BN / 32;
    extern __shared__ __attribute__((aligned(16))) float smem[];

    const int tid = threadIdx.x;
    const int lane = tid & 63;
    const int wave = __builtin_amdgcn_readfirstlane(tid >> 6);
    const int wm = wave / WGN, wn = wave % WGN;
// ... 1386 lines not shown
        const long long total = (long long)p.M * K;
        if (stats != nullptr) {
            DSRL_REQUIRE(fwd_stats_parts(p, conv_planes(PASS_FWD)) == stats_parts && stats_parts > 0 && ldy % 4 == 0 && ((uintptr_t)y % 16) == 0 &&
                         (bias == nullptr || ((uintptr_t)bias % 16) == 0), DSRL_E_BADARG,
                         "conv2d_fwd_stats: this split-K launch writes %d row blocks of partials (ldy a multiple of 4, y 16-byte aligned), the caller expects %d",
                         fwd_stats_parts(p, conv_planes(PASS_FWD)), stats_parts);
            hipLaunchKernelGGL(splitk_reduce_stats_kernel, dim3((unsigned)(stats_parts * (K / 32))), dim3(256), 0, st,
                               (const float*)ws, p.splits, a.slab, p.M, K, bias, y, ldy, stats);
            return launch_status("splitk_reduce_stats_kernel");
        }
        hipLaunchKernelGGL(splitk_reduce_kernel, dim3((unsigned)std::min<long long>(ceil_div(total, 256), 4096)), dim3(256), 0, st,
                           (const float*)ws, p.splits, a.slab, p.M, K, bias, y, ldy);
        return launch_status("splitk_reduce_kernel");
    }
    if (stats != nullptr) {
        DSRL_REQUIRE(fwd_stats_parts(p, conv_planes(PASS_FWD)) == stats_parts && stats_parts > 0, DSRL_E_BADARG,
                     "conv2d_fwd_stats: this launch writes %d row blocks of partials, the caller expects %d (dsrl_conv2d_fwd_stats_parts)",
                     fwd_stats_parts(p, conv_planes(PASS_FWD)), stats_parts);
        a.stats = stats;
    }
    a.y = y; a.ldy = ldy; a.bias = bias;
    return launch_igemm<false>(a, p.cfg, st);
}

extern "C" int dsrl_conv2d_fwd(const float* x, int ldx, const float* w, const float* bias, float* y, int ldy,
                               int N, int H, int W, int C, int K, int R, int S, int stride, int pad, int dil,
                               void* ws, size_t ws_bytes, dsrl_stream_t stream) {
    return fwd_impl(x, ldx, w, bias, y, ldy, N, H, W, C, K, R, S, stride, pad, dil, ws, ws_bytes, stream, nullptr, 0);
}
extern "C" int dsrl_conv2d_fwd_stats(const float* x, int ldx, const float* w, const float* bias, float* y, int ldy,
                                     int N, int H, int W, int C, int K, int R, int S, int stride, int pad, int dil,
                                     void* ws, size_t ws_bytes, float* stats, int stats_parts, dsrl_stream_t stream) {
    DSRL_REQUIRE(stats != nullptr, DSRL_E_BADARG, "conv2d_fwd_stats: null statistics buffer");
    return fwd_impl(x, ldx, w, bias, y, ldy, N, H, W, C, K, R, S, stride, pad, dil, ws, ws_bytes, stream, stats, stats_parts);
}

static int pad4(int v) { return (v + 3) & ~3; }
static size_t dgrad_wt_bytes(int C, int K, int R, int S) { return align_up((size_t)C * pad4(K) * R * S * sizeof(float), 256); }

extern "C" size_t dsrl_conv2d_dgrad_workspace_bytes(int N, int H, int W, int C, int K, int R, int S, int stride, int pad, int dil) {
    const int Ho = out_size(H, R, stride, pad, dil), Wo = out_size(W, S, stride, pad, dil);
    if (Ho <= 0 || Wo <= 0) return 0;
    return with_amax_scratch(dgrad_wt_bytes(C, K, R, S) + plan_fwd_ws(N, Ho, Wo, pad4(K), C, R, S, H, W));
}

extern "C" size_t dsrl_conv2d_transposed_filter_floats(int C, int K, int R, int S) { return (size_t)C * R * S * pad4(K); }
extern "C" int dsrl_conv2d_transpose_filter(const float* w, float* wt, int C, int K, int R, int S, dsrl_stream_t stream) {
    DSRL_REQUIRE(w && wt && C > 0 && K > 0 && R > 0 && S > 0, DSRL_E_BADARG, "conv2d_transpose_filter: bad arguments");
    hipStream_t st = (hipStream_t)stream;
    if (int e = bind_stream_device(st)) return e;
    const int Kp = pad4(K);
    hipLaunchKernelGGL(weight_transpose_kernel, dim3((unsigned)ceil_div(C, 32), (unsigned)ceil_div(Kp, 32), (unsigned)(R * S)), dim3(256), 0, st, w, wt, K, Kp, R * S, C);
    return launch_status("weight_transpose_kernel");
}

extern "C" int dsrl_conv2d_split_filters_batched(const int64_t* table, int n, int64_t total_tiles, dsrl_stream_t stream) {
    DSRL_REQUIRE(table && n > 0 && total_tiles > 0 && total_tiles < (1ll << 31), DSRL_E_BADARG, "conv2d_split_filters_batched: bad arguments");
    hipStream_t st = (hipStream_t)stream;
    if (int e = bind_stream_device(st)) return e;
    hipLaunchKernelGGL(weight_split_batched_kernel, dim3((unsigned)ceil_div(total_tiles, (int64_t)kWtTilesPerBlock)), dim3(256), 0, st, (const long long*)table, n,
                       (long long)total_tiles);
    return launch_status("weight_split_batched_kernel");
}

extern "C" int dsrl_conv2d_transpose_filters_batched(const int64_t* table, int n, int64_t total_tiles, dsrl_stream_t stream) {
    DSRL_REQUIRE(table && n > 0 && total_tiles > 0 && total_tiles < (1ll << 31), DSRL_E_BADARG, "conv2d_transpose_filters_batched: bad arguments");
    hipStream_t st = (hipStream_t)stream;
    if (int e = bind_stream_device(st)) return e;
    hipLaunchKernelGGL(weight_transpose_batched_kernel, dim3((unsigned)ceil_div(total_tiles, (int64_t)kWtTilesPerBlock)), dim3(256), 0, st, (const long long*)table, n,
                       (long long)total_tiles);
    return launch_status("weight_transpose_batched_kernel");
}

extern "C" int dsrl_conv2d_filters_amax_segment_floats(void) { return kAmaxSegFloats; }
extern "C" int dsrl_conv2d_filters_amax_batched(const int64_t* table, int64_t nseg, dsrl_stream_t stream) {
    DSRL_REQUIRE(table && nseg > 0 && nseg < (1ll << 31), DSRL_E_BADARG, "conv2d_filters_amax_batched: bad arguments");
    hipStream_t st = (hipStream_t)stream;
    if (int e = bind_stream_device(st)) return e;
    hipLaunchKernelGGL(weight_amax_batched_kernel, dim3((unsigned)nseg), dim3(256), 0, st, (const long long*)table);
    return launch_status("weight_amax_batched_kernel");
}

struct DgradBn { const float* x; const float* y; const float* mean; const float* invstd; float* stats; int ldx, ldy, relu; float gscale = 1.f; };
static int dgrad_impl(const float* dy, int lddy, const float* w, const float* wt_in, float* dx, int lddx,
                      int N, int H, int W, int C, int K, int R, int S, int stride, int pad, int dil,
                      void* ws, size_t ws_bytes, dsrl_stream_t stream, int accumulate, const DgradBn* bn = nullptr,
                      const unsigned* dy_amax = nullptr, const unsigned* w_amax = nullptr, const void* wt_split = nullptr,
                      const void* dy_planes = nullptr, const void* wt_planes = nullptr) {
    if (int e = check_conv(dy, w, dx, N, H, W, C, K, R, S, stride, pad, dil)) return e;
    const int Kp = pad4(K);
    DSRL_REQUIRE(lddy % 4 == 0 && ((uintptr_t)dy % 16) == 0, DSRL_E_UNSUPPORTED,
                 "conv2d_dgrad: lddy (%d) must be a multiple of 4 and dy 16-byte aligned", lddy);
    DSRL_REQUIRE(lddy >= Kp && lddx >= C, DSRL_E_BADARG, "conv2d_dgrad: ld smaller than (padded) channel count");
    hipStream_t st = (hipStream_t)stream;
    if (int e = bind_stream_device(st)) return e;
    const int Ho = out_size(H, R, stride, pad, dil), Wo = out_size(W, S, stride, pad, dil);
    const FwdPlan p = plan_dgrad(N, Ho, Wo, Kp, C, R, S, H, W, conv_planes(PASS_DGRAD), stride);
    const size_t wtb = dgrad_wt_bytes(C, K, R, S);
    DSRL_REQUIRE(ws && ws_bytes >= wtb + p.ws, DSRL_E_WORKSPACE, "conv2d_dgrad: workspace %zu < %zu", ws_bytes, wtb + p.ws);
    const float* wt = wt_in;
    float* slabs = (float*)((char*)ws + wtb);
    const bool use_planes = conv_f16() && dy_planes != nullptr && wt_planes != nullptr && dy_amax != nullptr && w_amax != nullptr && stride == 1 && K % 8 == 0 &&
                            planes_usable(K, lddy, dy_planes, wt_planes) && planes_cfg_supported((int)p.cfg, p.kg) && !(p.coop && p.splits > 1);
    const bool use_split = conv_f16() && wt_split != nullptr && w_amax != nullptr;
    if (wt == nullptr && use_planes) wt = (const float*)wt_planes;
    if (wt == nullptr && use_split) wt = (const float*)wt_split;
    if (wt == nullptr) {
        hipLaunchKernelGGL(weight_transpose_kernel, dim3((unsigned)ceil_div(C, 32), (unsigned)ceil_div(Kp, 32), (unsigned)(R * S)), dim3(256), 0, st,
                           w, (float*)ws, K, Kp, R * S, C);
        if (int e = launch_status("weight_transpose_kernel")) return e;
        wt = (const float*)ws;
    }
    ConvArgs a{};
    a.x = dy; a.w = wt; a.ldx = lddy; a.N = N; a.H = Ho; a.W = Wo; a.C = Kp; a.K = C; a.R = R; a.S = S; a.Ho = H; a.Wo = W;
    a.stride = stride; a.pad = pad; a.dil = dil; a.M = p.M; a.cchunks = p.cchunks; a.splits = p.splits; a.kg = p.kg; a.slab = (long long)p.M * C;
    {
        const long long xb = span_bytes((long long)N * Ho * Wo, lddy, Kp), wb = (long long)C * R * S * Kp * 4, yb = p.splits > 1 ? (long long)p.M * C * 4 : span_bytes(p.M, lddx, C);
        DSRL_REQUIRE_31(xb, "conv2d_dgrad(dy)"); DSRL_REQUIRE_31(wb, "conv2d_dgrad(w)"); DSRL_REQUIRE_31(yb, "conv2d_dgrad(dx)");
        a.x_bytes = (unsigned)xb; a.w_bytes = (unsigned)wb; a.y_bytes = (unsigned)yb;
    }
    if (conv_f16()) {
        OperandAmax am{dy_amax, w_amax};
        if (int e = resolve_amax(am, dy, lddy, (long long)N * Ho * Wo, Kp, w, C, (long long)K * R * S, C, ws, ws_bytes, wtb + p.ws, st, "conv2d_dgrad")) return e;
        a.amax_a = am.a; a.amax_b = am.b;
        if (wt_split != nullptr && w_amax != nullptr) {
            DSRL_REQUIRE(((uintptr_t)wt_split % 16) == 0, DSRL_E_BADARG, "conv2d_dgrad: unaligned pre-split filter");
            a.w = (const float*)wt_split; a.w_split = 1;
        }
        if (use_planes) {
            const long long pe = (long long)N * Ho * Wo * lddy, we = (long long)C * R * S * K;
            a.planes = conv_planes(PASS_DGRAD); a.w_split = 0;
            a.x = (const float*)dy_planes; a.w = (const float*)wt_planes;
            a.x_bytes = (unsigned)(span_bytes((long long)N * Ho * Wo, lddy, K) / 2); a.w_bytes = (unsigned)(we * 2);
            a.a_lo = (unsigned)planes_lo_offset(pe); a.b_lo = (unsigned)planes_lo_offset(we);
        }
    }
    ProfScope prof(prof_family(PASS_DGRAD), 2.0 * (double)dsrl_conv2d_inbounds_macs(N, H, W, C, K, R, S, stride, pad, dil), 4.0 * ((double)N * H * W * C + (double)K * R * S * C + (double)N * out_size(H, R, stride, pad, dil) * out_size(W, S, stride, pad, dil) * K), st);
    prof.shape("dgrad", N, H, W, C, K, R, stride, pad, dil);
    if (p.splits > 1 && !(p.coop && a.amax_a != nullptr && !a.planes && stride == 1)) {
        DSRL_REQUIRE(bn == nullptr, DSRL_E_UNSUPPORTED, "conv2d_dgrad: BatchNorm sums asked from a split-K launch that reduces through slabs");
        a.y = slabs; a.ldy = C; a.bias = nullptr;
        if (int e = launch_igemm<true>(a, p.cfg, st)) return e;
        const long long total = (long long)p.M * C;
        hipLaunchKernelGGL(splitk_reduce_kernel, dim3((unsigned)std::min<long long>(ceil_div(total, 256), 4096)), dim3(256), 0, st,
                           (const float*)slabs, p.splits, a.slab, p.M, C, (const float*)nullptr, dx, lddx, accumulate);
        return launch_status("splitk_reduce_kernel");
    }
    if (p.splits > 1) {
        a.coop_slab = slabs; a.tickets = const_cast<unsigned*>(a.amax_a);
        a.y_bytes = (unsigned)span_bytes(p.M, lddx, C);
    }
    a.y = dx; a.ldy = lddx; a.bias = nullptr; a.accumulate = accumulate;
    if (stride > 1 && conv_planes(PASS_DGRAD) && H % stride == 0 && W % stride == 0 && (W / stride) % 32 == 0 && knob("DSRL_DGRAD_PARITY", 1)) {
        int bm, bn_; cfg_dims(p.cfg, bm, bn_);
        const long long Mc = (long long)N * (H / stride) * (W / stride);
        if (Mc % bm == 0) { a.par = stride; a.Hh = H / stride; a.Wh = W / stride; a.pbm = bm; }
    }
    if (bn) {
        a.bn_x = bn->x; a.bn_y = bn->y; a.bn_mean = bn->mean; a.bn_invstd = bn->invstd; a.bstats = bn->stats; a.bn_ldx = bn->ldx; a.bn_ldy = bn->ldy; a.bn_relu = bn->relu;
        a.bn_gscale = bn->gscale;
        a.bn_fast = a.par == 0 && C % 4 == 0 && bn->ldx % 4 == 0 && (!bn->relu || bn->ldy % 4 == 0) && ((uintptr_t)bn->x % 16) == 0 && (!bn->relu || ((uintptr_t)bn->y % 16) == 0) &&
                    ((uintptr_t)bn->mean % 16) == 0 && ((uintptr_t)bn->invstd % 16) == 0 && ((uintptr_t)bn->stats % 16) == 0;
    }
    return launch_igemm<true>(a, p.cfg, st);
}

extern "C" int dsrl_conv2d_dgrad(const float* dy, int lddy, const float* w, const float* wt_in, float* dx, int lddx,
                                 int N, int H, int W, int C, int K, int R, int S, int stride, int pad, int dil,
                                 void* ws, size_t ws_bytes, dsrl_stream_t stream) {
    return dgrad_impl(dy, lddy, w, wt_in, dx, lddx, N, H, W, C, K, R, S, stride, pad, dil, ws, ws_bytes, stream, 0);
}
extern "C" int dsrl_conv2d_dgrad_stats_parts(int N, int H, int W, int C, int K, int R, int S, int stride, int pad, int dil) {
    const int Ho = out_size(H, R, stride, pad, dil), Wo = out_size(W, S, stride, pad, dil);
    if (Ho <= 0 || Wo <= 0) return 0;
    const int npl = conv_planes(PASS_DGRAD);
    return fwd_stats_parts(plan_dgrad(N, Ho, Wo, pad4(K), C, R, S, H, W, npl, stride), npl, true);
}
extern "C" int dsrl_conv2d_dgrad_bnstats(const float* dy, int lddy, const float* w, const float* wt_in, float* dx, int lddx,
                                         int N, int H, int W, int C, int K, int R, int S, int stride, int pad, int dil,
                                         void* ws, size_t ws_bytes, const float* bn_x, int bn_ldx, const float* bn_y, int bn_ldy,
                                         const float* bn_mean, const float* bn_invstd, int bn_relu, float* bstats, int stats_parts, int accumulate,
                                         dsrl_stream_t stream) {
    DSRL_REQUIRE(bn_x && bn_mean && bn_invstd && bstats && (bn_y || !bn_relu) && bn_ldx >= C && (!bn_relu || bn_ldy >= C), DSRL_E_BADARG, "conv2d_dgrad_bnstats: bad BatchNorm arguments");
    DSRL_REQUIRE(dsrl_conv2d_dgrad_stats_parts(N, H, W, C, K, R, S, stride, pad, dil) == stats_parts && stats_parts > 0, DSRL_E_BADARG,
                 "conv2d_dgrad_bnstats: this launch writes %d row blocks of partials, the caller expects %d",
                 dsrl_conv2d_dgrad_stats_parts(N, H, W, C, K, R, S, stride, pad, dil), stats_parts);
    DgradBn bn{bn_x, bn_y, bn_mean, bn_invstd, bstats, bn_ldx, bn_ldy, bn_relu};
    return dgrad_impl(dy, lddy, w, wt_in, dx, lddx, N, H, W, C, K, R, S, stride, pad, dil, ws, ws_bytes, stream, accumulate ? 1 : 0, &bn);
}
extern "C" int dsrl_conv2d_dgrad_accumulate(const float* dy, int lddy, const float* w, const float* wt_in, float* dx, int lddx,
                                            int N, int H, int W, int C, int K, int R, int S, int stride, int pad, int dil,
                                            void* ws, size_t ws_bytes, dsrl_stream_t stream) {
    return dgrad_impl(dy, lddy, w, wt_in, dx, lddx, N, H, W, C, K, R, S, stride, pad, dil, ws, ws_bytes, stream, 1);
}

static void launch_wgrad(const WgradArgs& a_in, TileCfg cfg, int bm, int bn, dim3 grid, hipStream_t st) {
    const int npl = conv_planes(PASS_WGRAD);
    const bool f16 = conv_f16();
    if (npl) {
        WgradArgs a = a_in;
        make_magic(a.Ho * a.Wo, a.mHW, a.sHW);
        make_magic(a.Wo, a.mW, a.sW);
        const size_t stages = (size_t)2 * npl * 16 * ((bm * 2 + 64) + (bn * 2 + 64));
        const int kg = a.kg > 1 ? a.kg : 1;
        if (kg > 1) {
            const size_t lds = std::max(stages * kg, (size_t)kg * (bm / 32) * (bn / 32) / 4 * 16384 + 8192);
#define DSRL_LAUNCH_WKG(a_, b_, c_, d_, NPL_, KG_, F16_)                                                                            \
            {                                                                                                                        \
                static const hipError_t attr = hipFuncSetAttribute((const void*)conv_wgrad_split_kernel<a_, b_, c_, d_, NPL_, KG_, F16_>,  \
                                                                   hipFuncAttributeMaxDynamicSharedMemorySize, 144 * 1024);          \
                (void)attr;                                                                                                          \
                hipLaunchKernelGGL((conv_wgrad_split_kernel<a_, b_, c_, d_, NPL_, KG_, F16_>), grid, dim3(256 * KG_), lds, st, a);   \
            }
#define DSRL_WKG_BY_NPL(a_, b_, c_, d_, KG_) { if (f16 && npl == 1) DSRL_LAUNCH_WKG(a_, b_, c_, d_, 1, KG_, true) else if (f16) DSRL_LAUNCH_WKG(a_, b_, c_, d_, 2, KG_, true) else if (npl == 2) DSRL_LAUNCH_WKG(a_, b_, c_, d_, 2, KG_, false) else DSRL_LAUNCH_WKG(a_, b_, c_, d_, 3, KG_, false) }
            if (cfg == T64x64) DSRL_WKG_BY_NPL(1, 1, 2, 2, 2)
            else if (cfg == T128x64) DSRL_WKG_BY_NPL(2, 1, 2, 2, 2)
            else if (cfg == T64x128) DSRL_WKG_BY_NPL(1, 2, 2, 2, 2)
            else DSRL_WKG_BY_NPL(2, 2, 2, 2, 2)
#undef DSRL_WKG_BY_NPL
#undef DSRL_LAUNCH_WKG
            return;
        }
        const size_t lds = stages;
#define DSRL_LAUNCH_WGRAD(a_, b_, c_, d_)                                                                           \
        if (f16 && npl == 1) hipLaunchKernelGGL((conv_wgrad_split_kernel<a_, b_, c_, d_, 1, 1, true>), grid, dim3(256), lds, st, a); \
        else if (f16) hipLaunchKernelGGL((conv_wgrad_split_kernel<a_, b_, c_, d_, 2, 1, true>), grid, dim3(256), lds, st, a); \
        else if (npl == 2) hipLaunchKernelGGL((conv_wgrad_split_kernel<a_, b_, c_, d_, 2>), grid, dim3(256), lds, st, a); \
        else hipLaunchKernelGGL((conv_wgrad_split_kernel<a_, b_, c_, d_, 3>), grid, dim3(256), lds, st, a);
        DSRL_CFG_SWITCH(cfg, DSRL_LAUNCH_WGRAD)
#undef DSRL_LAUNCH_WGRAD
        return;
    }
    const size_t lds = (size_t)32 * (bm + bn) * sizeof(float);
#define DSRL_LAUNCH_WGRAD(a_, b_, c_, d_) hipLaunchKernelGGL((conv_wgrad_f32_kernel<a_, b_, c_, d_>), grid, dim3(256), lds, st, a_in)
    DSRL_CFG_SWITCH(cfg, DSRL_LAUNCH_WGRAD)
#undef DSRL_LAUNCH_WGRAD
}

namespace dsrl {
struct WgPlan { int Ho, Wo; long long P; TileCfg cfg; int bm, bn, ktiles, ctiles, psplits; TapList tl; size_t ws; bool w3; };
static int w3_psplits(long long tiles, long long chunks) {
    const int forced = knob("DSRL_FORCE_PSPLITS", 0);
    if (forced > 0) return (int)std::max<long long>(1, std::min<long long>(forced, chunks));
    long long sp = std::max<long long>(1, 2 * kNumCU / std::max<long long>(tiles, 1));
    sp = std::min(sp, std::max<long long>(1, chunks / 8));
    return (int)std::max<long long>(1, std::min<long long>(sp, 128));
}
static WgPlan plan_wgrad(int N, int H, int W, int C, int K, int R, int S, int stride, int pad, int dil) {
    WgPlan p; p.Ho = out_size(H, R, stride, pad, dil); p.Wo = out_size(W, S, stride, pad, dil);
    p.P = (long long)N * p.Ho * p.Wo;
    p.cfg = pick_cfg_wgrad(K, C);
    int bm, bn; cfg_dims(p.cfg, bm, bn); p.bm = bm; p.bn = bn;
    p.ktiles = (int)ceil_div(K, bm); p.ctiles = (int)ceil_div(C, bn);
    p.tl.n = 0;
    for (int r = 0; r < R; ++r)
        for (int s = 0; s < S; ++s)
            if (valid_count(H, p.Ho, stride, pad, r * dil) > 0 && valid_count(W, p.Wo, stride, pad, s * dil) > 0) p.tl.taps[p.tl.n++] = r * S + s;
    const long long chunks = ceil_div(p.P, 32);
    p.w3 = p.tl.n == 9 && wgrad3_eligible(N, H, W, C, K, R, S, stride, pad, dil, conv_planes(PASS_WGRAD), conv_f16());
    if (p.w3) {
        wgrad3_tile(p.bm, p.bn);
        p.ktiles = (int)ceil_div(K, p.bm); p.ctiles = (int)ceil_div(C, p.bn);
        p.psplits = w3_psplits((long long)p.ktiles * p.ctiles, chunks);
        p.ws = p.psplits > 1 ? (size_t)p.psplits * K * R * S * C * sizeof(float) : 0;
        return p;
    }
// ... 29 lines not shown
    a.x = x; a.dy = dy; a.ldx = ldx; a.lddy = lddy; a.N = N; a.H = H; a.W = W; a.C = C; a.K = K; a.R = R; a.S = S; a.Ho = p.Ho; a.Wo = p.Wo;
    a.stride = stride; a.pad = pad; a.dil = dil; a.P = p.P; a.ctiles = p.ctiles; a.psplits = p.psplits; a.slab = (long long)K * RS * C;
    {
        const long long xb = span_bytes((long long)N * H * W, ldx, C), db = span_bytes(p.P, lddy, pad4(K));
        DSRL_REQUIRE_31(xb, "conv2d_wgrad(x)"); DSRL_REQUIRE_31(db, "conv2d_wgrad(dy)");
        a.x_bytes = (unsigned)xb; a.dy_bytes = (unsigned)db; a.no_ident = wgrad_no_ident();
    }
    a.ntaps = p.tl.n;
    for (int i = 0; i < p.tl.n; ++i) a.taps[i] = p.tl.taps[i];
    if (conv_f16()) {
        OperandAmax am{dy_amax, x_amax};
        if (int e = resolve_amax(am, dy, lddy, p.P, pad4(K), x, ldx, (long long)N * H * W, C, ws, ws_bytes, p.ws, st, "conv2d_wgrad")) return e;
        a.amax_dy = am.a; a.amax_x = am.b;
    }
    if (p.w3) {
        a.psplits = p.psplits; a.kg = 1;
        a.dw = p.psplits > 1 ? (float*)ws : dw;
        a.kctiles = p.ktiles * p.ctiles; a.xcd_remap = knob("DSRL_XCD_REMAP", 1);
        a.nblocks = a.kctiles * a.psplits;
        make_magic(a.Ho * a.Wo, a.mHW, a.sHW);
        make_magic(a.Wo, a.mW, a.sW);
        ProfScope prof(prof_family(PASS_WGRAD), 2.0 * (double)dsrl_conv2d_inbounds_macs(N, H, W, C, K, R, S, stride, pad, dil), 4.0 * ((double)N * H * W * C + (double)K * R * S * C + (double)p.P * K), st);
        prof.shape("wgrad", N, H, W, C, K, R, stride, pad, dil);
        if (int e = launch_wgrad3(a, conv_planes(PASS_WGRAD), st)) return e;
        if (p.psplits > 1) {
            const long long total = (long long)K * p.tl.n * (C / 4);
            hipLaunchKernelGGL(wgrad_reduce_kernel, dim3((unsigned)std::min<long long>(ceil_div(total, 256), 4096)), dim3(256), 0, st,
                               (const float*)ws, p.psplits, a.slab, dw, K, RS, C, p.tl);
            return launch_status("wgrad_reduce_kernel");
        }
        return DSRL_OK;
    }
    int psplits = p.psplits, kg = 1;
    if (conv_planes(PASS_WGRAD)) {
        const int npl = conv_planes(PASS_WGRAD);
        const int maxkg = (p.cfg == T64x64 || p.cfg == T128x64 || p.cfg == T64x128 || p.cfg == T128x128) ? 2 : 1;
        const int forced = knob("DSRL_FORCE_WGRAD_KG", 0);
        kg = forced > 0 ? std::min(forced, maxkg) : ((RS == 1 && psplits >= 4) ? std::min(2, maxkg) : 1);
        if (kg == 3) kg = 2;
        while (kg > 1 && (size_t)kg * 2 * npl * 16 * ((p.bm * 2 + 64) + (p.bn * 2 + 64)) > 144 * 1024) kg /= 2;
        psplits = (int)ceil_div(psplits, kg);
    }
    a.psplits = psplits; a.kg = kg;
    a.dw = psplits > 1 ? (float*)ws : dw;
    a.kctiles = p.ktiles * p.ctiles; a.xcd_remap = knob("DSRL_XCD_REMAP", 1);
    dim3 grid((unsigned)(a.kctiles * p.tl.n * psplits));
    ProfScope prof(prof_family(PASS_WGRAD), 2.0 * (double)dsrl_conv2d_inbounds_macs(N, H, W, C, K, R, S, stride, pad, dil), 4.0 * ((double)N * H * W * C + (double)K * R * S * C + (double)N * out_size(H, R, stride, pad, dil) * out_size(W, S, stride, pad, dil) * K), st);
    prof.shape("wgrad", N, H, W, C, K, R, stride, pad, dil);
    launch_wgrad(a, p.cfg, p.bm, p.bn, grid, st);
    if (int e = launch_status("conv_wgrad kernel")) return e;
    if (psplits > 1) {
        const long long total = (long long)K * p.tl.n * (C / 4);
        hipLaunchKernelGGL(wgrad_reduce_kernel, dim3((unsigned)std::min<long long>(ceil_div(total, 256), 4096)), dim3(256), 0, st,
                           (const float*)ws, psplits, a.slab, dw, K, RS, C, p.tl);
        return launch_status("wgrad_reduce_kernel");
    }
    return DSRL_OK;
}
extern "C" int dsrl_conv2d_wgrad(const float* x, int ldx, const float* dy, int lddy, float* dw,
                                 int N, int H, int W, int C, int K, int R, int S, int stride, int pad, int dil,
                                 void* ws, size_t ws_bytes, dsrl_stream_t stream) {
    return wgrad_impl(x, ldx, dy, lddy, dw, N, H, W, C, K, R, S, stride, pad, dil, ws, ws_bytes, stream, nullptr, nullptr);
}

extern "C" int dsrl_amax(const float* x, int ld, int64_t P, int C, uint32_t* amax, dsrl_stream_t stream) {
    DSRL_REQUIRE(x && amax && ld >= C && C > 0 && P > 0, DSRL_E_BADARG, "amax: bad arguments");
    hipStream_t st = (hipStream_t)stream;
    if (int e = bind_stream_device(st)) return e;
    return launch_amax(x, ld, P, C, amax, st);
}
extern "C" int dsrl_conv2d_fwd_amax(const float* x, int ldx, const uint32_t* x_amax, const float* w, const uint32_t* w_amax, const void* w_split, const float* bias,
                                    float* y, int ldy, int N, int H, int W, int C, int K, int R, int S, int stride, int pad, int dil,
                                    void* ws, size_t ws_bytes, float* stats, int stats_parts, dsrl_stream_t stream) {
    return fwd_impl(x, ldx, w, bias, y, ldy, N, H, W, C, K, R, S, stride, pad, dil, ws, ws_bytes, stream, stats, stats_parts, x_amax, w_amax, w_split);
}
extern "C" int dsrl_conv2d_dgrad_amax(const float* dy, int lddy, const uint32_t* dy_amax, const float* w, const float* wt_in, const uint32_t* w_amax, const void* wt_split,
                                      float* dx, int lddx,
                                      int N, int H, int W, int C, int K, int R, int S, int stride, int pad, int dil,
                                      void* ws, size_t ws_bytes, const float* bn_x, int bn_ldx, const float* bn_y, int bn_ldy,
                                      const float* bn_mean, const float* bn_invstd, int bn_relu, float* bstats, int stats_parts, int accumulate,
                                      dsrl_stream_t stream) {
    if (bstats == nullptr)
        return dgrad_impl(dy, lddy, w, wt_in, dx, lddx, N, H, W, C, K, R, S, stride, pad, dil, ws, ws_bytes, stream, accumulate ? 1 : 0, nullptr, dy_amax, w_amax, wt_split);
    DSRL_REQUIRE(bn_x && bn_mean && bn_invstd && (bn_y || !bn_relu) && bn_ldx >= C && (!bn_relu || bn_ldy >= C), DSRL_E_BADARG, "conv2d_dgrad_amax: bad BatchNorm arguments");
    DSRL_REQUIRE(dsrl_conv2d_dgrad_stats_parts(N, H, W, C, K, R, S, stride, pad, dil) == stats_parts && stats_parts > 0, DSRL_E_BADARG,
                 "conv2d_dgrad_amax: this launch writes %d row blocks of partials, the caller expects %d",
                 dsrl_conv2d_dgrad_stats_parts(N, H, W, C, K, R, S, stride, pad, dil), stats_parts);
    DgradBn bn{bn_x, bn_y, bn_mean, bn_invstd, bstats, bn_ldx, bn_ldy, bn_relu};
    return dgrad_impl(dy, lddy, w, wt_in, dx, lddx, N, H, W, C, K, R, S, stride, pad, dil, ws, ws_bytes, stream, accumulate ? 1 : 0, &bn, dy_amax, w_amax, wt_split);
}
extern "C" int dsrl_conv2d_fwd_planes(const float* x, int ldx, const uint32_t* x_amax, const void* x_planes, const float* w, const uint32_t* w_amax, const void* w_split,
                                      const void* w_planes, const float* bias, float* y, int ldy, int N, int H, int W, int C, int K, int R, int S, int stride, int pad, int dil,
                                      void* ws, size_t ws_bytes, float* stats, int stats_parts, dsrl_stream_t stream) {
    return fwd_impl(x, ldx, w, bias, y, ldy, N, H, W, C, K, R, S, stride, pad, dil, ws, ws_bytes, stream, stats, stats_parts, x_amax, w_amax, w_split, x_planes, w_planes);
}
extern "C" int dsrl_conv2d_dgrad_planes(const float* dy, int lddy, const uint32_t* dy_amax, const void* dy_planes, const float* w, const float* wt_in, const uint32_t* w_amax,
                                        const void* wt_split, const void* wt_planes, float* dx, int lddx,
                                        int N, int H, int W, int C, int K, int R, int S, int stride, int pad, int dil,
                                        void* ws, size_t ws_bytes, const float* bn_x, int bn_ldx, const float* bn_y, int bn_ldy,
                                        const float* bn_mean, const float* bn_invstd, int bn_relu, float* bstats, int stats_parts, int accumulate,
                                        dsrl_stream_t stream) {
    return dsrl_conv2d_dgrad_planes_drop(dy, lddy, dy_amax, dy_planes, w, wt_in, w_amax, wt_split, wt_planes, dx, lddx, N, H, W, C, K, R, S, stride, pad, dil, ws, ws_bytes,
                                         bn_x, bn_ldx, bn_y, bn_ldy, bn_mean, bn_invstd, bn_relu, 0.f, bstats, stats_parts, accumulate, stream);
}
extern "C" int dsrl_conv2d_dgrad_planes_drop(const float* dy, int lddy, const uint32_t* dy_amax, const void* dy_planes, const float* w, const float* wt_in, const uint32_t* w_amax,
                                             const void* wt_split, const void* wt_planes, float* dx, int lddx,
                                             int N, int H, int W, int C, int K, int R, int S, int stride, int pad, int dil,
                                             void* ws, size_t ws_bytes, const float* bn_x, int bn_ldx, const float* bn_y, int bn_ldy,
                                             const float* bn_mean, const float* bn_invstd, int bn_relu, float bn_drop_p, float* bstats, int stats_parts, int accumulate,
                                             dsrl_stream_t stream) {
    DSRL_REQUIRE(bn_drop_p >= 0.f && bn_drop_p < 1.f && (bn_drop_p == 0.f || bn_relu), DSRL_E_BADARG, "conv2d_dgrad_planes_drop: dropout p=%f needs the ReLU mask (y > 0)", bn_drop_p);
    if (bstats == nullptr)
        return dgrad_impl(dy, lddy, w, wt_in, dx, lddx, N, H, W, C, K, R, S, stride, pad, dil, ws, ws_bytes, stream, accumulate ? 1 : 0, nullptr, dy_amax, w_amax, wt_split,
                          dy_planes, wt_planes);
    DSRL_REQUIRE(bn_x && bn_mean && bn_invstd && (bn_y || !bn_relu) && bn_ldx >= C && (!bn_relu || bn_ldy >= C), DSRL_E_BADARG, "conv2d_dgrad_planes: bad BatchNorm arguments");
    DSRL_REQUIRE(dsrl_conv2d_dgrad_stats_parts(N, H, W, C, K, R, S, stride, pad, dil) == stats_parts && stats_parts > 0, DSRL_E_BADARG,
                 "conv2d_dgrad_planes: this launch writes %d row blocks of partials, the caller expects %d",
                 dsrl_conv2d_dgrad_stats_parts(N, H, W, C, K, R, S, stride, pad, dil), stats_parts);
    DgradBn bn{bn_x, bn_y, bn_mean, bn_invstd, bstats, bn_ldx, bn_ldy, bn_relu};
    bn.gscale = bn_drop_p > 0.f ? 1.f / (1.f - bn_drop_p) : 1.f;
    return dgrad_impl(dy, lddy, w, wt_in, dx, lddx, N, H, W, C, K, R, S, stride, pad, dil, ws, ws_bytes, stream, accumulate ? 1 : 0, &bn, dy_amax, w_amax, wt_split,
                      dy_planes, wt_planes);
}
extern "C" int dsrl_conv2d_wgrad_amax(const float* x, int ldx, const uint32_t* x_amax, const float* dy, int lddy, const uint32_t* dy_amax, float* dw,
                                      int N, int H, int W, int C, int K, int R, int S, int stride, int pad, int dil,
                                      void* ws, size_t ws_bytes, dsrl_stream_t stream) {
    return wgrad_impl(x, ldx, dy, lddy, dw, N, H, W, C, K, R, S, stride, pad, dil, ws, ws_bytes, stream, x_amax, dy_amax);
}


namespace dsrl {
constexpr unsigned kGroupMagic = 0x44535247u;
constexpr int kGroupMaxProblems = 512, kGroupMaxLaunches = kNumCfg + 2;
constexpr int kCfgW3 = kNumCfg;
struct GroupLaunch { int cfg, first, count, grid; double flops, bytes; };
struct GroupHeader {
    unsigned magic; int n, nlaunch, npl, f16;
    GroupLaunch launch[kGroupMaxLaunches];
    int rgrid;
    long long args_off, starts_off, rstarts_off, used_bytes;
};
static size_t group_table_bytes(int n) {
    return align_up(sizeof(GroupHeader), 256) + align_up((size_t)n * sizeof(WgradArgs), 256) + 2 * align_up((size_t)(n + 1) * sizeof(int), 256);
}
static int group_target_px() { return std::max(256, knob("DSRL_WGRAD_GROUP_PX", 4096)); }
struct GroupItem { WgradArgs a; TileCfg cfg; int bm, bn; double cost, flops, bytes; size_t slab_bytes; };
static int group_psplits(long long P, int w3_px = 0) {
    const long long chunks = ceil_div(P, 32);
    if (w3_px > 0) {
        const int forced3 = knob("DSRL_FORCE_PSPLITS", 0), px = w3_px;
        long long sp3 = forced3 > 0 ? forced3 : (P + px / 2) / px;
        sp3 = std::max<long long>(1, std::min<long long>(sp3, std::max<long long>(1, chunks / 8)));
        return (int)std::min<long long>(sp3, 256);
    }
    const int forced = knob("DSRL_FORCE_PSPLITS", 0);
    long long sp = forced > 0 ? forced : (P + group_target_px() / 2) / group_target_px();
    sp = std::max<long long>(1, std::min<long long>(sp, std::max<long long>(1, chunks / 4)));
    return (int)std::min<long long>(sp, 256);
}
static int w3_group_px(const dsrl_wgrad_problem*, int, int) { return std::max(256, knob("DSRL_WGRAD3_PX", 2048)); }
static int group_item(const dsrl_wgrad_problem& q, int npl, GroupItem& it, const int* w3_px) {
    const int N = q.N, H = q.H, W = q.W, C = q.C, K = q.K, R = q.R, S = q.S, stride = q.stride, pad = q.pad, dil = q.dil;
    if (int e = check_conv(q.x, q.dy, q.dw, N, H, W, C, K, R, S, stride, pad, dil)) return e;
    DSRL_REQUIRE(C % 4 == 0 && q.ldx % 4 == 0 && q.lddy % 4 == 0 && q.lddy >= pad4(K) && ((uintptr_t)q.x % 16) == 0 && ((uintptr_t)q.dy % 16) == 0 && ((uintptr_t)q.dw % 16) == 0,
                 DSRL_E_UNSUPPORTED, "conv2d_wgrad_group: C (%d), ldx (%d), lddy (%d) must be multiples of 4 (lddy >= K rounded up to 4), pointers 16-byte aligned", C, q.ldx, q.lddy);
    const WgPlan p = plan_wgrad(N, H, W, C, K, R, S, stride, pad, dil);
    DSRL_REQUIRE(p.P < (1ll << 31), DSRL_E_UNSUPPORTED, "conv2d_wgrad_group: more than 2^31 output pixels");
    WgradArgs a{};
    a.x = q.x; a.dy = q.dy; a.ldx = q.ldx; a.lddy = q.lddy; a.N = N; a.H = H; a.W = W; a.C = C; a.K = K; a.R = R; a.S = S; a.Ho = p.Ho; a.Wo = p.Wo;
    a.stride = stride; a.pad = pad; a.dil = dil; a.P = p.P; a.ctiles = p.ctiles; a.slab = (long long)K * R * S * C;
    const long long xb = span_bytes((long long)N * H * W, q.ldx, C), db = span_bytes(p.P, q.lddy, pad4(K));
    DSRL_REQUIRE_31(xb, "conv2d_wgrad_group(x)"); DSRL_REQUIRE_31(db, "conv2d_wgrad_group(dy)");
    a.x_bytes = (unsigned)xb; a.dy_bytes = (unsigned)db; a.no_ident = wgrad_no_ident();
    a.ntaps = p.tl.n;
    for (int i = 0; i < p.tl.n; ++i) a.taps[i] = p.tl.taps[i];
    a.psplits = group_psplits(p.P, p.w3 ? w3_px[dil - 1] : 0);
    a.kg = 1; a.kctiles = p.ktiles * p.ctiles; a.xcd_remap = knob("DSRL_XCD_REMAP", 1);
    a.nblocks = p.w3 ? a.kctiles * a.psplits : a.kctiles * a.ntaps * a.psplits;
    a.dw_final = q.dw; a.dw = q.dw;
    a.rblocks = a.psplits > 1 ? (int)ceil_div((long long)K * a.ntaps * (C / 4), 1024) : 0;
    make_magic(a.Ho * a.Wo, a.mHW, a.sHW);
    make_magic(a.Wo, a.mW, a.sW);
    DSRL_REQUIRE(!conv_f16() || (q.x_amax != nullptr && q.dy_amax != nullptr), DSRL_E_BADARG,
                 "conv2d_wgrad_group: the f16x3 arithmetic needs x_amax / dy_amax of every problem (dsrl_amax measures a tensor)");
    a.amax_x = q.x_amax; a.amax_dy = q.dy_amax;
    it.a = a; it.cfg = p.w3 ? (TileCfg)(kCfgW3 + dil - 1) : p.cfg; it.bm = p.bm; it.bn = p.bn;
    it.cost = (double)p.P / a.psplits * p.bm * p.bn;
    it.flops = 2.0 * (double)dsrl_conv2d_inbounds_macs(N, H, W, C, K, R, S, stride, pad, dil);
    it.bytes = 4.0 * ((double)N * H * W * C + (double)K * R * S * C + (double)p.P * K);
    it.slab_bytes = a.psplits > 1 ? align_up((size_t)a.psplits * a.slab * sizeof(float), 256) : 0;
    (void)npl;
    return DSRL_OK;
}
}

extern "C" size_t dsrl_conv2d_wgrad_group_table_bytes(int n) { return n > 0 ? group_table_bytes(n) : 0; }

extern "C" size_t dsrl_conv2d_wgrad_group_workspace_bytes(const dsrl_wgrad_problem* problems, int n) {
// ... 269 lines not shown
```

dualsuperreslearningforsemseg_amd/csrc/conv_planes.hip:

```cpp
#include "common.h"
#include "conv_common.h"
#include "lds_dma.h"
#include <algorithm>

namespace dsrl {

template <int NPL> struct PlaneMfma;
template <> struct PlaneMfma<2> {
    template <int MR, int NR>
    static __device__ __forceinline__ void run(f32x16 (&acc)[MR][NR], const f16x8 (&fa)[MR][2], const f16x8 (&fb)[NR][2]) {
#pragma unroll
        for (int sum = 1; sum >= 0; --sum)
#pragma unroll
            for (int pa = 0; pa <= sum; ++pa)
#pragma unroll
                for (int i = 0; i < MR; ++i)
#pragma unroll
                    for (int j = 0; j < NR; ++j)
                        acc[i][j] = __builtin_amdgcn_mfma_f32_32x32x16_f16(fa[i][pa], fb[j][sum - pa], acc[i][j], 0, 0, 0);
    }
};
template <> struct PlaneMfma<1> {
    template <int MR, int NR>
    static __device__ __forceinline__ void run(f32x16 (&acc)[MR][NR], const f16x8 (&fa)[MR][1], const f16x8 (&fb)[NR][1]) {
// ... 244 lines not shown
    {
        const int sh = -(sh_a + sh_b);
#pragma unroll
        for (int i = 0; i < MR; ++i)
#pragma unroll
            for (int jj = 0; jj < NR; ++jj)
#pragma unroll
                for (int e = 0; e < 16; ++e) acc[i][jj][e] = __builtin_ldexpf(acc[i][jj][e], sh);
    }
    float mine[KG > 1 ? MR : 1][KG > 1 ? NR : 1][KG > 1 ? EPG : 1];
    if constexpr (KG > 1) {
#pragma unroll
        for (int g = 0; g < KG; ++g)
            if (grp == g) {
#pragma unroll
                for (int i = 0; i < MR; ++i)
#pragma unroll
                    for (int j = 0; j < NR; ++j)
#pragma unroll
                        for (int k = 0; k < EPG; ++k) mine[i][j][k] = acc[i][j][g * EPG + k];
            }
    }
    auto share = [&](int i, int j, int e) -> float { if constexpr (KG > 1) return mine[i][j][e]; else return acc[i][j][e]; };
    auto share_add = [&](int i, int j, int e, float v) { if constexpr (KG > 1) mine[i][j][e] += v; else acc[i][j][e] += v; };
    const int rowg = 8 * ((grp * EPG) >> 2);
    float* yout = a.y + (a.splits > 1 ? (long long)z * a.slab : 0ll);
    const __amdgpu_buffer_rsrc_t yr = __builtin_amdgcn_make_buffer_rsrc((void*)yout, 0, (int)a.y_bytes, 0x00020000);
    const int col = lane & 31, rq = (lane >> 5) * 4 + rowg;
#pragma unroll
    for (int j = 0; j < NR; ++j) {
        const int k = n0 + (wn * NR + j) * 32 + col;
        const bool kok = k < a.K;
        const float bv = (a.bias != nullptr && kok) ? a.bias[k] : 0.f;
#pragma unroll
        for (int i = 0; i < MR; ++i) {
            const int mb32 = m0 + (wm * MR + i) * 32, mb = mb32 + rq;
            if (a.accumulate && a.splits == 1) {
                float old[EPG];
#pragma unroll
                for (int e = 0; e < EPG; ++e) {
                    const int m = mb + (e & 3) + 8 * (e >> 2);
                    const unsigned off = (kok && m < a.M) ? ((unsigned)m * (unsigned)a.ldy + (unsigned)k) * 4u : kOOB;
                    old[e] = __uint_as_float(__builtin_amdgcn_raw_buffer_load_b32(yr, (int)off, 0, 0));
                }
#pragma unroll
                for (int e = 0; e < EPG; ++e) share_add(i, j, e, old[e]);
            }
#pragma unroll
            for (int e = 0; e < EPG; ++e) {
                const int m = mb + (e & 3) + 8 * (e >> 2);
                const unsigned off = (kok && m < a.M) ? ((unsigned)m * (unsigned)a.ldy + (unsigned)k) * 4u : kOOB;
                __builtin_amdgcn_raw_buffer_store_b32(__float_as_uint(share(i, j, e) + bv), yr, (int)off, 0, 0);
            }
        }
    }
    bool bstats_done = false;
    if constexpr (DGRAD && KG == 1) {
        if (a.bstats != nullptr && (a.splits == 1) && a.bn_fast) {
            constexpr int TR = 32 * MR, TC = 32 * NR, CQ = TC / 4, RSTEP = 64 / CQ, NIT = TR / RSTEP, NB = NIT < 8 ? NIT : 8;
            float* wt = reinterpret_cast<float*>(smem) + (size_t)wave * TR * TC;
            __syncthreads();
#pragma unroll
            for (int i = 0; i < MR; ++i)
#pragma unroll
                for (int j = 0; j < NR; ++j)
#pragma unroll
                    for (int e = 0; e < 16; ++e)
                        wt[(i * 32 + (e & 3) + 8 * (e >> 2) + 4 * (lane >> 5)) * TC + j * 32 + (lane & 31)] = acc[i][j][e];
            const int c4 = lane % CQ, r0_ = lane / CQ;
            const int kk = n0 + wn * TC + 4 * c4;
            const bool kok4 = kk < a.K;
            const float4 mu4 = kok4 ? *reinterpret_cast<const float4*>(a.bn_mean + kk) : make_float4(0.f, 0.f, 0.f, 0.f);
            const float4 is4 = kok4 ? *reinterpret_cast<const float4*>(a.bn_invstd + kk) : make_float4(0.f, 0.f, 0.f, 0.f);
            float sg[4] = {0.f, 0.f, 0.f, 0.f}, sgx[4] = {0.f, 0.f, 0.f, 0.f};
            const int mrow0 = m0 + wm * TR;
#pragma unroll
            for (int b0 = 0; b0 < NIT; b0 += NB) {
                float4 xv[NB], yv[NB];
#pragma unroll
                for (int u = 0; u < NB; ++u) {
                    const int m = mrow0 + r0_ + RSTEP * (b0 + u);
                    const bool ok = kok4 && m < a.M;
                    xv[u] = ok ? *reinterpret_cast<const float4*>(a.bn_x + (long long)m * a.bn_ldx + kk) : make_float4(0.f, 0.f, 0.f, 0.f);
                    yv[u] = (ok && a.bn_relu) ? *reinterpret_cast<const float4*>(a.bn_y + (long long)m * a.bn_ldy + kk) : make_float4(1.f, 1.f, 1.f, 1.f);
                }
#pragma unroll
                for (int u = 0; u < NB; ++u) {
                    const int row = r0_ + RSTEP * (b0 + u);
                    if (kok4 && mrow0 + row < a.M) {
                        const float4 gv = *reinterpret_cast<const float4*>(wt + row * TC + 4 * c4);
                        const float gs = a.bn_gscale;
                        const float g0 = (a.bn_relu && !(yv[u].x > 0.f)) ? 0.f : gv.x * gs, g1 = (a.bn_relu && !(yv[u].y > 0.f)) ? 0.f : gv.y * gs;
                        const float g2 = (a.bn_relu && !(yv[u].z > 0.f)) ? 0.f : gv.z * gs, g3 = (a.bn_relu && !(yv[u].w > 0.f)) ? 0.f : gv.w * gs;
                        sg[0] += g0; sgx[0] += g0 * ((xv[u].x - mu4.x) * is4.x);
                        sg[1] += g1; sgx[1] += g1 * ((xv[u].y - mu4.y) * is4.y);
                        sg[2] += g2; sgx[2] += g2 * ((xv[u].z - mu4.z) * is4.z);
                        sg[3] += g3; sgx[3] += g3 * ((xv[u].w - mu4.w) * is4.w);
                    }
                }
            }
#pragma unroll
            for (int sft = CQ; sft < 64; sft <<= 1)
#pragma unroll
                for (int q = 0; q < 4; ++q) { sg[q] += __shfl_xor(sg[q], sft); sgx[q] += __shfl_xor(sgx[q], sft); }
            if (lane < CQ && kok4) {
                const int nparts = a.mtiles * WGM, part = tile_m * WGM + wm;
                float* o = a.bstats + (long long)part * a.K + kk;
                *reinterpret_cast<float4*>(o) = make_float4(sg[0], sg[1], sg[2], sg[3]);
                *reinterpret_cast<float4*>(o + (long long)nparts * a.K) = make_float4(sgx[0], sgx[1], sgx[2], sgx[3]);
            }
            bstats_done = true;
        }
    }
    if (DGRAD && a.bstats != nullptr && a.splits == 1 && !bstats_done) {
        const int nparts = a.mtiles * WGM, part = tile_m * WGM + wm;
        float* ex = reinterpret_cast<float*>(smem) + (size_t)KG * MR * NR * 4 * NT * 4;
#pragma unroll
        for (int j = 0; j < NR; ++j) {
            const int k = n0 + (wn * NR + j) * 32 + col;
            const bool kok = k < a.K;
            const float mu = kok ? a.bn_mean[k] : 0.f, is = kok ? a.bn_invstd[k] : 0.f;
            float sg = 0.f, sgx = 0.f;
#pragma unroll
            for (int i = 0; i < MR; ++i) {
                float xv[EPG], yv[EPG];
                const int mb32 = m0 + (wm * MR + i) * 32;
#pragma unroll
                for (int e = 0; e < EPG; ++e) {
                    const int m = mb32 + rq + (e & 3) + 8 * (e >> 2);
                    const bool ok = kok && m < a.M;
                    const long long px = m;
                    xv[e] = ok ? a.bn_x[px * a.bn_ldx + k] : 0.f;
                    yv[e] = (ok && a.bn_relu) ? a.bn_y[px * a.bn_ldy + k] : 1.f;
                }
#pragma unroll
                for (int e = 0; e < EPG; ++e) {
                    const int m = mb32 + rq + (e & 3) + 8 * (e >> 2);
                    if (kok && m < a.M) {
                        const float g = (a.bn_relu && !(yv[e] > 0.f)) ? 0.f : share(i, j, e) * a.bn_gscale;
                        sg += g; sgx += g * ((xv[e] - mu) * is);
                    }
                }
            }
            sg += __shfl_xor(sg, 32); sgx += __shfl_xor(sgx, 32);
            if (KG == 1) {
                if (lane < 32 && kok) {
                    float* o = a.bstats + (long long)part * a.K + k;
                    o[0] = sg; o[(long long)nparts * a.K] = sgx;
                }
            } else if (lane < 32) {
                ex[(((grp * NW + wave) * NR + j) * 2 + 0) * 32 + lane] = sg;
                ex[(((grp * NW + wave) * NR + j) * 2 + 1) * 32 + lane] = sgx;
            }
        }
        if constexpr (KG > 1) {
            __syncthreads();
            if (grp == 0 && lane < 32) {
#pragma unroll
                for (int j = 0; j < NR; ++j) {
                    const int k = n0 + (wn * NR + j) * 32 + col;
                    float sg = 0.f, sgx = 0.f;
#pragma unroll
                    for (int g = 0; g < KG; ++g) {
                        sg += ex[(((g * NW + wave) * NR + j) * 2 + 0) * 32 + lane];
                        sgx += ex[(((g * NW + wave) * NR + j) * 2 + 1) * 32 + lane];
                    }
                    if (k < a.K) {
                        float* o = a.bstats + (long long)part * a.K + k;
                        o[0] = sg; o[(long long)nparts * a.K] = sgx;
                    }
                }
            }
        }
    }
    const bool stats_wave = !(KG > 1 && grp > 0);
    if (a.stats != nullptr && a.splits == 1) {
        const int nparts = a.mtiles, part = tile_m;
        float* mg = reinterpret_cast<float*>(smem) + (KG > 1 ? (size_t)KG * MR * NR * 4 * NT * 4 : 0);
        float sn[NR], sm[NR], sq[NR];
        if (stats_wave) {
#pragma unroll
            for (int j = 0; j < NR; ++j) {
                const int k = n0 + (wn * NR + j) * 32 + col;
                const bool kok = k < a.K;
                const float bv = (a.bias != nullptr && kok) ? a.bias[k] : 0.f;
                float n = 0.f, sum = 0.f;
#pragma unroll
                for (int i = 0; i < MR; ++i)
#pragma unroll
                    for (int e = 0; e < 16; ++e)
                        if (m0 + (wm * MR + i) * 32 + (lane >> 5) * 4 + (e & 3) + 8 * (e >> 2) < a.M) { n += 1.f; sum += acc[i][j][e] + bv; }
                n += __shfl_xor(n, 32); sum += __shfl_xor(sum, 32);
                const float mean = n > 0.f ? sum / n : 0.f;
                float q = 0.f;
#pragma unroll
                for (int i = 0; i < MR; ++i)
#pragma unroll
                    for (int e = 0; e < 16; ++e)
                        if (m0 + (wm * MR + i) * 32 + (lane >> 5) * 4 + (e & 3) + 8 * (e >> 2) < a.M) { const float d = acc[i][j][e] + bv - mean; q += d * d; }
                q += __shfl_xor(q, 32);
                sn[j] = n; sm[j] = mean; sq[j] = q;
                if (WGM > 1 && wm > 0 && lane < 32) {
                    float* o = mg + ((wm * (WGN * NR) + wn * NR + j) * 3) * 32 + lane;
                    o[0] = n; o[32] = mean; o[64] = q;
                }
            }
        }
        if constexpr (WGM > 1) __syncthreads();
        if (stats_wave && wm == 0 && lane < 32) {
#pragma unroll
            for (int j = 0; j < NR; ++j) {
                const int k = n0 + (wn * NR + j) * 32 + col;
                float na = sn[j], ma = sm[j], qa = sq[j];
#pragma unroll
                for (int w = 1; w < WGM; ++w) {
                    const float* o = mg + ((w * (WGN * NR) + wn * NR + j) * 3) * 32 + lane;
// ... 221 lines not shown
```

dualsuperreslearningforsemseg_amd/csrc/conv_split_kernel.h:

```cpp
#pragma once
#include "common.h"
#include "conv_common.h"

namespace dsrl {

template <int MR, int NR, int WGM, int WGN, bool DGRAD, int NPL, int KG = 1, int ARITH = 0, bool STR1 = false, bool COOP = false>
__global__ __launch_bounds__(64 * WGM * WGN * KG, KG == 1 ? 2 : 1)
void conv_igemm_split_kernel(const ConvArgs a) {
    const int stride = STR1 ? 1 : a.stride, par = STR1 ? 0 : a.par;
    constexpr bool F16 = ARITH != 0, PREB = ARITH == 2;
    constexpr int NT = 64 * WGM * WGN, RP = NT / 4;
    static_assert(NT == 256 || (NT == 512 && KG == 1), "4 waves per K group, or one group of 8 waves");
    static_assert(!F16 || NPL <= 2, "f16x3 carries two fp16 terms per operand, f16x1 one");
    using PT = Plane<F16>;
    using pl4 = typename PT::v4; using pl8 = typename PT::v8;
    const unsigned am_a = F16 ? amax_fetch(a.amax_a) : 0u, am_b = F16 ? amax_fetch(a.amax_b) : 0u;
    int sh_a = 0, sh_b = 0;
    constexpr int BM = 32 * MR * WGM, BN = 32 * NR * WGN;
    constexpr int A_IT = (BM + RP - 1) / RP, B_IT = (BN + RP - 1) / RP;
    constexpr int NV = A_IT + B_IT;
    constexpr bool FS = F16;
    constexpr int ROWB = FS ? 64 : 32;
    constexpr int STAGE = (BM + BN) * NPL * ROWB;
    extern __shared__ __attribute__((aligned(16))) float smem[];
// ... 412 lines not shown
            if constexpr (KG > 1) {
                if (!DGRAD && a.stats != nullptr) {
                    float* xch = reinterpret_cast<float*>(smem);
                    __syncthreads();
#pragma unroll
                    for (int i = 0; i < MR; ++i)
#pragma unroll
                        for (int j = 0; j < NR; ++j)
#pragma unroll
                            for (int k = 0; k < EPG; ++k) xch[((i * NR + j) * 16 + grp * EPG + k) * 256 + tid] = mine[i][j][k];
                    __syncthreads();
                    if (grp == 0) {
#pragma unroll
                        for (int i = 0; i < MR; ++i)
#pragma unroll
                            for (int j = 0; j < NR; ++j)
#pragma unroll
                                for (int e = 0; e < 16; ++e) acc[i][j][e] = xch[((i * NR + j) * 16 + e) * 256 + tid];
                    }
                }
            }
        }
    }
    const bool single = coop || a.splits == 1;
    float* yout = a.y + (!single ? (long long)z * a.slab : 0ll);
    const __amdgpu_buffer_rsrc_t yr = __builtin_amdgcn_make_buffer_rsrc((void*)yout, 0, (int)a.y_bytes, 0x00020000);
    const int col = lane & 31, rq = (lane >> 5) * 4 + rowg;
#pragma unroll
    for (int j = 0; j < NR; ++j) {
        const int k = n0 + (wn * NR + j) * 32 + col;
        const bool kok = k < a.K;
        const float bv = (a.bias != nullptr && kok) ? a.bias[k] : 0.f;
#pragma unroll
        for (int i = 0; i < MR; ++i) {
            const int mb32 = m0 + (wm * MR + i) * 32, mb = mb32 + rq;
            const int pix0 = (DGRAD && par) ? dgrad_pix(a, min(mb32, a.M - 1)) : mb32, pst = (DGRAD && par) ? par : 1;
            if (a.accumulate && single) {
                float old[EPG];
#pragma unroll
                for (int e = 0; e < EPG; ++e) {
                    const int m = mb + (e & 3) + 8 * (e >> 2);
                    const unsigned off = (kok && m < a.M) ? ((unsigned)(pix0 + (m - mb32) * pst) * (unsigned)a.ldy + (unsigned)k) * 4u : kOOB;
                    old[e] = __uint_as_float(__builtin_amdgcn_raw_buffer_load_b32(yr, (int)off, 0, 0));
                }
#pragma unroll
                for (int e = 0; e < EPG; ++e) share_add(i, j, e, old[e]);
            }
#pragma unroll
            for (int e = 0; e < EPG; ++e) {
                const int m = mb + (e & 3) + 8 * (e >> 2);
                const unsigned off = (kok && m < a.M) ? ((unsigned)(pix0 + (m - mb32) * pst) * (unsigned)a.ldy + (unsigned)k) * 4u : kOOB;
                __builtin_amdgcn_raw_buffer_store_b32(__float_as_uint(share(i, j, e) + bv), yr, (int)off, 0, 0);
            }
        }
    }
    bool bstats_done = false;
    if constexpr (DGRAD && KG == 1) {
        if (a.bstats != nullptr && single && a.bn_fast) {
            constexpr int TR = 32 * MR, TC = 32 * NR, CQ = TC / 4, RSTEP = 64 / CQ, NIT = TR / RSTEP, NB = NIT < 8 ? NIT : 8;
            float* wt = reinterpret_cast<float*>(smem) + (size_t)wave * TR * TC;
            __syncthreads();
#pragma unroll
            for (int i = 0; i < MR; ++i)
#pragma unroll
                for (int j = 0; j < NR; ++j)
#pragma unroll
                    for (int e = 0; e < 16; ++e)
                        wt[(i * 32 + (e & 3) + 8 * (e >> 2) + 4 * (lane >> 5)) * TC + j * 32 + (lane & 31)] = acc[i][j][e];
            const int c4 = lane % CQ, r0_ = lane / CQ;
            const int kk = n0 + wn * TC + 4 * c4;
            const bool kok4 = kk < a.K;
            const float4 mu4 = kok4 ? *reinterpret_cast<const float4*>(a.bn_mean + kk) : make_float4(0.f, 0.f, 0.f, 0.f);
            const float4 is4 = kok4 ? *reinterpret_cast<const float4*>(a.bn_invstd + kk) : make_float4(0.f, 0.f, 0.f, 0.f);
            float sg[4] = {0.f, 0.f, 0.f, 0.f}, sgx[4] = {0.f, 0.f, 0.f, 0.f};
            const int mrow0 = m0 + wm * TR;
#pragma unroll
            for (int b0 = 0; b0 < NIT; b0 += NB) {
                float4 xv[NB], yv[NB];
#pragma unroll
                for (int u = 0; u < NB; ++u) {
                    const int m = mrow0 + r0_ + RSTEP * (b0 + u);
                    const bool ok = kok4 && m < a.M;
                    xv[u] = ok ? *reinterpret_cast<const float4*>(a.bn_x + (long long)m * a.bn_ldx + kk) : make_float4(0.f, 0.f, 0.f, 0.f);
                    yv[u] = (ok && a.bn_relu) ? *reinterpret_cast<const float4*>(a.bn_y + (long long)m * a.bn_ldy + kk) : make_float4(1.f, 1.f, 1.f, 1.f);
                }
#pragma unroll
                for (int u = 0; u < NB; ++u) {
                    const int row = r0_ + RSTEP * (b0 + u);
                    if (kok4 && mrow0 + row < a.M) {
                        const float4 gv = *reinterpret_cast<const float4*>(wt + row * TC + 4 * c4);
                        const float gs = a.bn_gscale;
                        const float g0 = (a.bn_relu && !(yv[u].x > 0.f)) ? 0.f : gv.x * gs, g1 = (a.bn_relu && !(yv[u].y > 0.f)) ? 0.f : gv.y * gs;
                        const float g2 = (a.bn_relu && !(yv[u].z > 0.f)) ? 0.f : gv.z * gs, g3 = (a.bn_relu && !(yv[u].w > 0.f)) ? 0.f : gv.w * gs;
                        sg[0] += g0; sgx[0] += g0 * ((xv[u].x - mu4.x) * is4.x);
                        sg[1] += g1; sgx[1] += g1 * ((xv[u].y - mu4.y) * is4.y);
                        sg[2] += g2; sgx[2] += g2 * ((xv[u].z - mu4.z) * is4.z);
                        sg[3] += g3; sgx[3] += g3 * ((xv[u].w - mu4.w) * is4.w);
                    }
                }
            }
#pragma unroll
            for (int sft = CQ; sft < 64; sft <<= 1)
#pragma unroll
                for (int q = 0; q < 4; ++q) { sg[q] += __shfl_xor(sg[q], sft); sgx[q] += __shfl_xor(sgx[q], sft); }
            if (lane < CQ && kok4) {
                const int nparts = a.mtiles * WGM, part = tile_m * WGM + wm;
                float* o = a.bstats + (long long)part * a.K + kk;
                *reinterpret_cast<float4*>(o) = make_float4(sg[0], sg[1], sg[2], sg[3]);
                *reinterpret_cast<float4*>(o + (long long)nparts * a.K) = make_float4(sgx[0], sgx[1], sgx[2], sgx[3]);
            }
            bstats_done = true;
        }
    }
    if (DGRAD && a.bstats != nullptr && single && !bstats_done) {
        const int nparts = a.mtiles * WGM, part = tile_m * WGM + wm;
        float* ex = reinterpret_cast<float*>(smem) + (size_t)KG * MR * NR * 4 * 256 * 4;
#pragma unroll
        for (int j = 0; j < NR; ++j) {
            const int k = n0 + (wn * NR + j) * 32 + col;
            const bool kok = k < a.K;
            const float mu = kok ? a.bn_mean[k] : 0.f, is = kok ? a.bn_invstd[k] : 0.f;
            float sg = 0.f, sgx = 0.f;
#pragma unroll
            for (int i = 0; i < MR; ++i) {
                float xv[EPG], yv[EPG];
                const int mb32 = m0 + (wm * MR + i) * 32;
                const int pix0 = par ? dgrad_pix(a, min(mb32, a.M - 1)) : mb32, pst = par ? par : 1;
#pragma unroll
                for (int e = 0; e < EPG; ++e) {
                    const int m = mb32 + rq + (e & 3) + 8 * (e >> 2);
                    const bool ok = kok && m < a.M;
                    const long long px = pix0 + (m - mb32) * pst;
                    xv[e] = ok ? a.bn_x[px * a.bn_ldx + k] : 0.f;
                    yv[e] = (ok && a.bn_relu) ? a.bn_y[px * a.bn_ldy + k] : 1.f;
                }
#pragma unroll
                for (int e = 0; e < EPG; ++e) {
                    const int m = mb32 + rq + (e & 3) + 8 * (e >> 2);
                    if (kok && m < a.M) {
                        const float g = (a.bn_relu && !(yv[e] > 0.f)) ? 0.f : share(i, j, e) * a.bn_gscale;
                        sg += g; sgx += g * ((xv[e] - mu) * is);
                    }
                }
            }
            sg += __shfl_xor(sg, 32); sgx += __shfl_xor(sgx, 32);
            if (KG == 1) {
                if (lane < 32 && kok) {
                    float* o = a.bstats + (long long)part * a.K + k;
                    o[0] = sg; o[(long long)nparts * a.K] = sgx;
                }
            } else if (lane < 32) {
                ex[(((grp * 4 + wave) * NR + j) * 2 + 0) * 32 + lane] = sg;
                ex[(((grp * 4 + wave) * NR + j) * 2 + 1) * 32 + lane] = sgx;
            }
        }
        if constexpr (KG > 1) {
            __syncthreads();
            if (grp == 0 && lane < 32) {
#pragma unroll
                for (int j = 0; j < NR; ++j) {
                    const int k = n0 + (wn * NR + j) * 32 + col;
                    float sg = 0.f, sgx = 0.f;
#pragma unroll
                    for (int g = 0; g < KG; ++g) {
                        sg += ex[(((g * 4 + wave) * NR + j) * 2 + 0) * 32 + lane];
                        sgx += ex[(((g * 4 + wave) * NR + j) * 2 + 1) * 32 + lane];
                    }
                    if (k < a.K) {
                        float* o = a.bstats + (long long)part * a.K + k;
                        o[0] = sg; o[(long long)nparts * a.K] = sgx;
                    }
                }
            }
        }
    }
    const bool stats_wave = !(KG > 1 && grp > 0);
    if (a.stats != nullptr && single) {
        const int nparts = a.mtiles, part = tile_m;
        float* mg = reinterpret_cast<float*>(smem) + (KG > 1 ? (size_t)KG * MR * NR * 4 * 256 * 4 : 0);
        float sn[NR], sm[NR], sq[NR];
        if (stats_wave) {
#pragma unroll
            for (int j = 0; j < NR; ++j) {
                const int k = n0 + (wn * NR + j) * 32 + col;
                const bool kok = k < a.K;
                const float bv = (a.bias != nullptr && kok) ? a.bias[k] : 0.f;
                float n = 0.f, sum = 0.f;
#pragma unroll
                for (int i = 0; i < MR; ++i)
#pragma unroll
                    for (int e = 0; e < 16; ++e)
                        if (m0 + (wm * MR + i) * 32 + rq + (e & 3) + 8 * (e >> 2) < a.M) { n += 1.f; sum += acc[i][j][e] + bv; }
                n += __shfl_xor(n, 32); sum += __shfl_xor(sum, 32);
                const float mean = n > 0.f ? sum / n : 0.f;
                float q = 0.f;
#pragma unroll
                for (int i = 0; i < MR; ++i)
#pragma unroll
                    for (int e = 0; e < 16; ++e)
                        if (m0 + (wm * MR + i) * 32 + rq + (e & 3) + 8 * (e >> 2) < a.M) { const float d = acc[i][j][e] + bv - mean; q += d * d; }
                q += __shfl_xor(q, 32);
                sn[j] = n; sm[j] = mean; sq[j] = q;
                if (WGM > 1 && wm > 0 && lane < 32) {
                    float* o = mg + ((wm * (WGN * NR) + wn * NR + j) * 3) * 32 + lane;
                    o[0] = n; o[32] = mean; o[64] = q;
                }
            }
        }
        if constexpr (WGM > 1) __syncthreads();
        if (stats_wave && wm == 0 && lane < 32) {
#pragma unroll
            for (int j = 0; j < NR; ++j) {
                const int k = n0 + (wn * NR + j) * 32 + col;
                float na = sn[j], ma = sm[j], qa = sq[j];
#pragma unroll
                for (int w = 1; w < WGM; ++w) {
                    const float* o = mg + ((w * (WGN * NR) + wn * NR + j) * 3) * 32 + lane;
// ... 19 lines not shown
```

dualsuperreslearningforsemseg_amd/functional.py:

```python
import contextlib
import ctypes
import os
import sys
import weakref

import torch

from . import _lib
from ._lib import call, knob, query, DsrlHipError

CL = torch.channels_last


_raw_stream = getattr(torch._C, '_cuda_getCurrentRawStream', None)
_raw_device = getattr(torch._C, '_cuda_getDevice', None)


def _stream():
    if _raw_stream is not None and _raw_device is not None:
        return _raw_stream(_raw_device())
    return torch.cuda.current_stream().cuda_stream


_side = {}
# ... 477 lines not shown

_planes_holders = []


def drop_planes():
    for r in _planes_holders:
        t = r()
        if t is not None and hasattr(t, '_dsrl_planes'):
            try:
                del t._dsrl_planes
            except Exception:
                pass
    _planes_holders.clear()


def filter_planes(w, rec):
    from .filter_operands import table_row
    w = w_cl(w)
    K, C, R, S = w.shape
    nbytes = int(cquery('dsrl_planes_bytes', K * R * S * C, 2))
    wp = torch.empty(nbytes, device=w.device, dtype=torch.uint8)
    wtp = torch.empty(nbytes, device=w.device, dtype=torch.uint8)
    row, tiles = table_row(w.data_ptr(), K, R * S, C, 0, rec.data_ptr(), wtp.data_ptr(), wp.data_ptr(), pad_k=False)
    t = torch.tensor([row], dtype=torch.int64, device=w.device)
    call('dsrl_conv2d_filter_planes_batched', t.data_ptr(), 1, tiles, _stream())
    return wp, wtp


def _is_krsc(w):
    return w.is_contiguous(memory_format=CL) or (w.shape[2] == 1 and w.shape[3] == 1 and w.is_contiguous())


def w_cl(w):
    _need_gpu(w); _f32(w)
    return w if _is_krsc(w) else w.contiguous(memory_format=CL)


def _out_size(n, k, stride, pad, dil):
    return (n + 2 * pad - dil * (k - 1) - 1) // stride + 1


_rng_state = {'seed': 0x5EED, 'step': 0, 'current': 0}


def set_dropout_seed(seed):
    _rng_state['seed'] = int(seed) & 0xFFFFFFFFFFFF
    _rng_state['step'] = 0


def _derive(step):
    return (_rng_state['seed'] * 1000003 + step) & 0xFFFFFFFFFFFFFFFF


def peek_next_seed():
    return _derive(_rng_state['step'] + 1)


def begin_forward(training=True):
    if not training:
        return _rng_state['current']
    _rng_state['step'] += 1
    _rng_state['current'] = _derive(_rng_state['step'])
    return _rng_state['current']


def current_seed():
    return _rng_state['current']


grad_slots_enabled = knob('DSRL_GRAD_SLOTS', True)
outer_grad_slot = knob('DSRL_OUTER_SLOT', True)


class GradSlot:
    __slots__ = ('buf', 'closed', 'link')

    def __init__(self):
        self.buf, self.closed = None, False
        self.link = None


bn_bwd_stats_enabled = knob('DSRL_BN_BWD_STATS', True)
bn_bwd_stats_shared = knob('DSRL_BN_BWD_STATS_SHARED', True)


class BNLink:
    __slots__ = ('x', 'y_ptr', 'y_shape', 'mean', 'invstd', 'relu', 'valid', 'stats', 'parts', 'dx_ptr', 'shared', 'drop_p')

    def __init__(self, shared=False):
        self.x = self.mean = self.invstd = self.stats = None
        self.y_ptr, self.y_shape = 0, None
        self.relu, self.valid, self.parts, self.dx_ptr = False, False, 0, 0
        self.shared = shared
        self.drop_p = 0.0


class _Fork(torch.autograd.Function):
    @staticmethod
    def forward(ctx, x):
        return x.view_as(x)

    @staticmethod
    def backward(ctx, g):
        return g


def fork(x):
    y = _Fork.apply(x)
    a = carried_amax(x)
    if a is not None:
        set_amax(y, a)
    return y


class _Conv2d(torch.autograd.Function):
    @staticmethod
    def forward(ctx, x, w, bias, stride, pad, dil, gslot=None, stats_parts=0, in_link=None):
        ctx.set_materialize_grads(False)
        ctx.gslot = gslot
        ctx.in_link = in_link
        x_in = x
        x, ldx = pm_vec4(x)
        w_param = w
        w = w_cl(w)
        N, Cc, H, W = x.shape
        K, Cw, R, S = w.shape
        if Cw != Cc:
            raise DsrlHipError(f'conv2d: input has {Cc} channels, weight expects {Cw}')
        Ho, Wo = _out_size(H, R, stride, pad, dil), _out_size(W, S, stride, pad, dil)
        y = new_cl((N, K, Ho, Wo), x)
        shp = (N, H, W, Cc, K, R, S, stride, pad, dil)
        ws = _ws(cquery('dsrl_conv2d_fwd_workspace_bytes', *shp), x)
        if bias is not None:
            _need_gpu(bias)
        stats = None
        xa = wa = None
        if f16_mode():
            xa = amax_for(x_in, x, ldx)
            wa = _weight_amax(w_param)
        ctx.amax = (xa, wa)
        if stats_parts > 0:
            stats = torch.empty(cquery('dsrl_bn_stats_floats', 3, int(stats_parts), K), device=x.device, dtype=torch.float32)
        wsp = _weight_split(w_param) if wa is not None else None
        wpl = _weight_planes(w_param) if wa is not None else None
        if wpl is None and wa is not None and planes_wanted(x, ldx, Cc, K, R * S):
            w_param._dsrl_want_planes = True
        xp = planes_for(x_in, x, ldx, xa, R * S) if wpl is not None else None
        call('dsrl_conv2d_fwd_planes', x.data_ptr(), ldx, None if xa is None else xa.data_ptr(), None if xp is None else xp.data_ptr(), w.data_ptr(),
             None if wa is None else wa.data_ptr(), None if wsp is None else wsp.data_ptr(), None if wpl is None else wpl.data_ptr(),
             None if bias is None else bias.data_ptr(), y.data_ptr(), K, *shp, ws.data_ptr(), ws.numel(),
             None if stats is None else stats.data_ptr(), int(stats_parts), _stream())
        ctx.save_for_backward(x, w)
        ctx.shp = shp
        ctx.has_bias = bias is not None
        ctx.bparam = bias if isinstance(bias, torch.nn.Parameter) else None
        ctx.wparam = w_param if isinstance(w_param, torch.nn.Parameter) else None
        if stats is not None:
            ctx.mark_non_differentiable(stats)
            return y, stats
        return y

    @staticmethod
    def backward(ctx, dy, *_unused):
        if dy is None:
            return (None,) * 9
        x, w = ctx.saved_tensors
        shp = ctx.shp
        N, H, W, Cc, K, R, S, stride, pad, dil = shp
        dy_in = dy
        dy, lddy = pm_vec4(dy)
        ldx = _ld_of(x)
        dx = dw = db = None
        st = _stream()
        xa, wa = ctx.amax
        dya = None
        if f16_mode():
            dya = amax_for(dy_in, dy, lddy)
            if xa is None:
                xa = amax_for(x, x, ldx)
            if wa is not None and ctx.wparam is not None and _weight_amax(ctx.wparam) is None:
                wa = None
        p_ = lambda t_: None if t_ is None else t_.data_ptr()
        wtsp = _weight_split(ctx.wparam, True) if (wa is not None and ctx.wparam is not None) else None
        wtpl = _weight_planes(ctx.wparam, True) if (wa is not None and ctx.wparam is not None) else None
        dy_split_ok = planes_mode == 'all' or (_planes_npl() == 1 and dy.shape[0] * dy.shape[1] * dy.shape[2] * dy.shape[3] >= planes_min_elems)
        dyp = planes_for(dy_in, dy, lddy, dya, R * S, split_ok=dy_split_ok) if (wtpl is not None and ctx.needs_input_grad[0] and stride == 1 and K % 8 == 0) else None
        if ctx.needs_input_grad[1]:
            sink = _sink(ctx.wparam) if ctx.wparam is not None and _is_krsc(ctx.wparam) else None
            if sink is not None and wgrad_queue is not None:
                wp = ctx.wparam
                wgrad_queue.add(x, ldx, dy, lddy, sink, shp, lambda wp=wp: wp._dsrl_arena.written(wp), xa, dya)
            elif sink is not None and overlap_wgrad and ctx.needs_input_grad[0]:
                cur, side = torch.cuda.current_stream(), side_stream(x.device)
                side.wait_stream(cur)
                with torch.cuda.stream(side):
                    ws = _ws(cquery('dsrl_conv2d_wgrad_workspace_bytes', *shp), x)
                    call('dsrl_conv2d_wgrad_amax', x.data_ptr(), ldx, p_(xa), dy.data_ptr(), lddy, p_(dya), sink.data_ptr(), *shp, ws.data_ptr(), ws.numel(), side.cuda_stream)
                x.record_stream(side); dy.record_stream(side)
                ctx.wparam._dsrl_arena.written(ctx.wparam, side)
            else:
                dw = sink if sink is not None else torch.empty((K, Cc, R, S), device=x.device, dtype=torch.float32, memory_format=CL)
                ws = _ws(cquery('dsrl_conv2d_wgrad_workspace_bytes', *shp), x)
                call('dsrl_conv2d_wgrad_amax', x.data_ptr(), ldx, p_(xa), dy.data_ptr(), lddy, p_(dya), dw.data_ptr(), *shp, ws.data_ptr(), ws.numel(), st)
                if sink is not None:
                    ctx.wparam._dsrl_arena.written(ctx.wparam)
                    dw = None
        if ctx.needs_input_grad[0]:
            slot = ctx.gslot
            acc = (slot is not None and not slot.closed and slot.buf is not None and tuple(slot.buf.shape) == (N, Cc, H, W)
                   and slot.buf.is_contiguous(memory_format=CL))
            dx = slot.buf if acc else new_cl((N, Cc, H, W), x)
            if slot is not None and slot.link is not None and slot.link is not ctx.in_link and slot.link.stats is not None:
                slot.link.stats = None
            ws = _ws(cquery('dsrl_conv2d_dgrad_workspace_bytes', *shp), x)
            wt_ptr = None
            if ctx.wparam is not None:
                h = getattr(ctx.wparam, '_dsrl_operands', None)
                wt = None if h is None else h[0].fp32_transpose(h[1])
                if wt is not None:
                    wt_ptr = wt.data_ptr()
            link = ctx.in_link
            parts = 0
            final = (not acc and ctx.gslot is None) or (acc and getattr(link, 'shared', False))
            if (link is not None and link.valid and final and link.y_ptr == x.data_ptr() and link.y_shape == (N, Cc, H, W) and Cc % 32 == 0):
                parts = int(query('dsrl_conv2d_dgrad_stats_parts', *shp))
            if parts > 0:
                bstats = torch.empty(cquery('dsrl_bn_stats_floats', 2, parts, Cc), device=x.device, dtype=torch.float32)
                _, bld = pm(link.x)
                call('dsrl_conv2d_dgrad_planes_drop', dy.data_ptr(), lddy, p_(dya), p_(dyp), w.data_ptr(), wt_ptr, p_(wa), p_(wtsp), p_(wtpl), dx.data_ptr(), Cc, *shp,
                     ws.data_ptr(), ws.numel(), link.x.data_ptr(), bld, x.data_ptr(), ldx, link.mean.data_ptr(), link.invstd.data_ptr(), int(link.relu),
                     float(link.drop_p), bstats.data_ptr(), parts, int(acc), st)
                link.stats, link.parts, link.dx_ptr = bstats, parts, dx.data_ptr()
            else:
                call('dsrl_conv2d_dgrad_planes', dy.data_ptr(), lddy, p_(dya), p_(dyp), w.data_ptr(), wt_ptr, p_(wa), p_(wtsp), p_(wtpl), dx.data_ptr(), Cc, *shp,
                     ws.data_ptr(), ws.numel(), None, 0, None, 0, None, None, 0, None, 0, int(acc), st)
            if acc:
                dx = None
            elif slot is not None:
                if slot.buf is None:
                    slot.buf = dx
                else:
                    slot.closed = True
        if ctx.has_bias and ctx.needs_input_grad[2]:
            P = dy.shape[0] * dy.shape[2] * dy.shape[3]
            bsink = _sink_flat(ctx.bparam, K)
            db = bsink if bsink is not None else torch.empty(K, device=x.device, dtype=torch.float32)
            ws = _ws(cquery('dsrl_colsum_workspace_bytes', P, K), x)
            call('dsrl_colsum', dy.data_ptr(), lddy, P, K, db.data_ptr(), ws.data_ptr(), ws.numel(), st)
            if bsink is not None:
                _sunk(ctx.bparam); db = None
            else:
                db = _deliver(ctx.bparam, db)
        if dw is not None:
            dw = _deliver(ctx.wparam, dw)
        return dx, dw, db, None, None, None, None, None, None


class _StemConv(torch.autograd.Function):

    @staticmethod
    def forward(ctx, x, w, stride, pad):
        _need_gpu(x, w); _f32(x); _f32(w)
        N, Cc, H, W = x.shape
        K, _, R, S = w.shape
        Sp = (S + 7) & ~7 if S > 4 else 4
        Cf = Sp * 4
        Ho, Wo = _out_size(H, R, stride, pad, 1), _out_size(W, S, stride, pad, 1)
        Hp = max(H + 2 * pad, (Ho - 1) * stride + R)
        Wp = max(W + 2 * pad, (Wo - 1) * stride + Sp) + 1
        st = _stream()
        xp = torch.empty((N, Hp, Wp, 4), device=x.device, dtype=torch.float32)
        sn, sc, sh, sw = x.stride()
        call('dsrl_pad_image_nhwc', x.data_ptr(), sn, sc, sh, sw, xp.data_ptr(), N, Cc, H, W, 4, pad, pad, Hp, Wp, st)
        w2 = getattr(w, '_dsrl_stem_pad', None)
        if w2 is None or tuple(w2.shape) != (K, R, Sp, 4) or w2.device != x.device:
            w2 = torch.zeros((K, R, Sp, 4), device=x.device, dtype=torch.float32)
            if isinstance(w, torch.nn.Parameter):
                w._dsrl_stem_pad = w2
        w2[:, :, :S, :Cc] = w.detach().permute(0, 2, 3, 1)
        y = new_cl((N, K, Ho, Wo), x)
        macs = cquery('dsrl_conv2d_inbounds_macs', N, H, W, Cc, K, R, S, stride, pad, 1)
        shp = (N, Hp, Wp, Cf, K, R, stride, Ho, Wo)
        ws = _ws(cquery('dsrl_conv2d_rowfold_fwd_workspace_bytes', *shp), x)
        call('dsrl_conv2d_rowfold_fwd', xp.data_ptr(), 4, w2.data_ptr(), None, y.data_ptr(), K, *shp, macs, ws.data_ptr(), ws.numel(), st)
        ctx.save_for_backward(xp)
        ctx.cfg = (shp, macs, tuple(w.shape), Sp)
        ctx.wparam = w if isinstance(w, torch.nn.Parameter) else None
        return y

    @staticmethod
    def backward(ctx, dy):
        xp, = ctx.saved_tensors
        shp, macs, wshape, Sp = ctx.cfg
        K, Cc, R, S = wshape
        if ctx.needs_input_grad[0]:
            raise DsrlHipError('the image stem has no input-gradient kernel (the reference never differentiates w.r.t. the image)')
        dy, lddy = pm_vec4(dy)
        dw2 = torch.empty((K, R, Sp, 4), device=dy.device, dtype=torch.float32)
        ws = _ws(cquery('dsrl_conv2d_rowfold_wgrad_workspace_bytes', *shp), dy)
        call('dsrl_conv2d_rowfold_wgrad', xp.data_ptr(), 4, dy.data_ptr(), lddy, dw2.data_ptr(), *shp, macs, ws.data_ptr(), ws.numel(), _stream())
        dw = _deliver(ctx.wparam, dw2[:, :, :S, :Cc].permute(0, 3, 1, 2))
        return None, dw, None, None


def conv2d(x, weight, bias=None, stride=1, padding=0, dilation=1, grad_slot=None, in_link=None):
    if grad_slot is not None and x.shape[1] % 4 != 0:
        grad_slot.closed = True
        grad_slot = None
    if x.shape[1] < 4 and bias is None and dilation == 1 and not x.requires_grad:
        return _StemConv.apply(x, weight, int(stride), int(padding))
    if x.shape[1] % 4 != 0:
        padc = 4 - x.shape[1] % 4
        x = torch.nn.functional.pad(x, (0, 0, 0, 0, 0, padc))
        weight = torch.nn.functional.pad(weight, (0, 0, 0, 0, 0, padc))
    if in_link is not None and x.shape[1] % 4 == 0 and bn_bwd_stats_enabled:
        return _Conv2d.apply(x, weight, bias, int(stride), int(padding), int(dilation), grad_slot, 0, in_link)
    return _Conv2d.apply(x, weight, bias, int(stride), int(padding), int(dilation), grad_slot)


class _BNAct(torch.autograd.Function):
    @staticmethod
    def forward(ctx, x, gamma, beta, running_mean, running_var, training, momentum, eps, relu, drop_p, seed, rng_stream, residual, rslot=None,
                stats=None, stats_parts=0, out_link=None, res_link=None):
        ctx.rslot = rslot
        ctx.out_link = out_link
        ctx.res_link = res_link if (res_link is not None and res_link.valid and not res_link.relu and residual is not None
                                    and res_link.y_ptr == residual.data_ptr() and res_link.y_shape == tuple(x.shape)) else None
        x, ldx = pm(x)
        _need_gpu(gamma, beta, running_mean, running_var)
        N, Cc, H, W = x.shape
        P = N * H * W
        st = _stream()
        y = new_cl((N, Cc, H, W), x)
        ya = amax_slot(x.device) if f16_mode() else None
        ya_ptr = None if ya is None else ya.data_ptr()
        res_ptr, ldr = None, 0
        if residual is not None:
            residual, ldr = pm(residual)
            res_ptr = residual.data_ptr()
        if training:
            if P <= 1:
                raise ValueError(f'Expected more than 1 value per channel when training, got input size {tuple(x.shape)}')
            ws = _ws(cquery('dsrl_bn_workspace_bytes', P, Cc), x)
            mean = torch.empty(Cc, device=x.device, dtype=torch.float32)
            invstd = torch.empty_like(mean)
            if stats is not None and stats_parts > 0:
                call('dsrl_bn_train_fwd_from_stats', x.data_ptr(), ldx, y.data_ptr(), Cc, P, Cc, float(eps), float(momentum), mean.data_ptr(), invstd.data_ptr(),
                     None if running_mean is None else running_mean.data_ptr(), None if running_var is None else running_var.data_ptr(),
                     gamma.data_ptr(), beta.data_ptr(), res_ptr, ldr, int(relu), float(drop_p), int(seed), int(rng_stream),
                     stats.data_ptr(), int(stats_parts), ya_ptr, st)
            else:
                call('dsrl_bn_train_fwd', x.data_ptr(), ldx, y.data_ptr(), Cc, P, Cc, float(eps), float(momentum), mean.data_ptr(), invstd.data_ptr(),
                     None if running_mean is None else running_mean.data_ptr(), None if running_var is None else running_var.data_ptr(),
                     gamma.data_ptr(), beta.data_ptr(), res_ptr, ldr, int(relu), float(drop_p), int(seed), int(rng_stream),
                     ws.data_ptr(), ws.numel(), ya_ptr, st)
        else:
            mean = running_mean
            invstd = frozen_invstd(running_var, eps)
            if invstd is None:
                invstd = torch.empty(Cc, device=x.device, dtype=torch.float32)
                call('dsrl_bn_invstd_from_var', running_var.data_ptr(), Cc, float(eps), invstd.data_ptr(), st)
            call('dsrl_bn_apply', x.data_ptr(), ldx, y.data_ptr(), Cc, P, Cc, mean.data_ptr(), invstd.data_ptr(), gamma.data_ptr(), beta.data_ptr(),
                 res_ptr, ldr, int(relu), float(drop_p), int(seed), int(rng_stream), ya_ptr, st)
        if ya is not None:
            set_amax(y, ya)
        ctx.save_for_backward(x, y, mean, invstd, gamma)
        if out_link is not None and (drop_p == 0.0 or relu) and Cc % 32 == 0 and ldx == Cc:
            out_link.x, out_link.mean, out_link.invstd, out_link.relu, out_link.valid = x, mean, invstd, bool(relu), True
            out_link.y_ptr, out_link.y_shape, out_link.drop_p = y.data_ptr(), tuple(y.shape), float(drop_p)
        ctx.cfg = (bool(training), bool(relu), float(drop_p), residual is not None)
        ctx.gb = (gamma, beta) if isinstance(gamma, torch.nn.Parameter) and isinstance(beta, torch.nn.Parameter) else None
        return y

    @staticmethod
    def backward(ctx, dy):
        x, y, mean, invstd, gamma = ctx.saved_tensors
        training, relu, drop_p, has_res = ctx.cfg
        dy, lddy = pm(dy)
        _, ldx = pm(x)
        N, Cc, H, W = x.shape
        P = N * H * W
        dx = new_cl((N, Cc, H, W), x)
        dres = new_cl((N, Cc, H, W), x) if has_res else None
        sg = sb = None
        if ctx.gb is not None and ctx.needs_input_grad[1] and ctx.needs_input_grad[2]:
            sg = _sink(ctx.gb[0])
            sb = _sink(ctx.gb[1]) if sg is not None else None
        dgamma = sg if sg is not None else torch.empty(Cc, device=x.device, dtype=torch.float32)
        dbeta = sb if sb is not None else torch.empty(Cc, device=x.device, dtype=torch.float32)
        dxa = amax_slot(x.device) if f16_mode() else None
        dxa_ptr = None if dxa is None else dxa.data_ptr()
        link = ctx.out_link
        if link is not None and link.stats is not None and link.dx_ptr == dy.data_ptr() and lddy == Cc and (drop_p == 0.0 or relu):
            rl = ctx.res_link
            rparts = int(query('dsrl_bn_bwd_from_stats_res_parts', P, Cc, int(link.parts))) if (rl is not None and dres is not None and bn_res_stats_enabled) else 0
            if rparts > 0:
                rstats = torch.empty(cquery('dsrl_bn_stats_floats', 2, rparts, Cc), device=x.device, dtype=torch.float32)
                _, rld = pm(rl.x)
                call('dsrl_bn_bwd_from_stats_res', x.data_ptr(), ldx, y.data_ptr(), Cc, dy.data_ptr(), lddy, dx.data_ptr(), Cc, dres.data_ptr(), Cc, P, Cc,
                     mean.data_ptr(), invstd.data_ptr(), gamma.data_ptr(), dgamma.data_ptr(), dbeta.data_ptr(), int(relu), float(drop_p), int(training),
                     link.stats.data_ptr(), int(link.parts), dxa_ptr, rl.x.data_ptr(), rld, rl.mean.data_ptr(), rl.invstd.data_ptr(), rstats.data_ptr(), rparts, _stream())
                rl.stats, rl.parts, rl.dx_ptr = rstats, rparts, dres.data_ptr()
            else:
                call('dsrl_bn_bwd_from_stats_drop', x.data_ptr(), ldx, y.data_ptr(), Cc, dy.data_ptr(), lddy, dx.data_ptr(), Cc,
                     None if dres is None else dres.data_ptr(), Cc, P, Cc, mean.data_ptr(), invstd.data_ptr(), gamma.data_ptr(),
                     dgamma.data_ptr(), dbeta.data_ptr(), int(relu), float(drop_p), int(training), link.stats.data_ptr(), int(link.parts), dxa_ptr, _stream())
        else:
            ws = _ws(cquery('dsrl_bn_workspace_bytes', P, Cc), x)
            call('dsrl_bn_bwd', x.data_ptr(), ldx, y.data_ptr(), Cc, dy.data_ptr(), lddy, dx.data_ptr(), Cc,
                 None if dres is None else dres.data_ptr(), Cc, P, Cc, mean.data_ptr(), invstd.data_ptr(), gamma.data_ptr(),
                 dgamma.data_ptr(), dbeta.data_ptr(), int(relu), drop_p, int(training), ws.data_ptr(), ws.numel(), dxa_ptr, _stream())
        if dxa is not None:
            set_amax(dx, dxa)
        if sg is not None:
            ctx.gb[0]._dsrl_arena.written(ctx.gb[0]); dgamma = None
        if sb is not None:
            ctx.gb[1]._dsrl_arena.written(ctx.gb[1]); dbeta = None
        if dres is not None and ctx.rslot is not None:
            if ctx.rslot.buf is None:
                ctx.rslot.buf = dres
            else:
                ctx.rslot.closed = True
        return dx, dgamma, dbeta, None, None, None, None, None, None, None, None, None, dres, None, None, None, None, None


bn_res_stats_enabled = knob('DSRL_BN_RES_STATS', True)


def frozen_invstd(running_var, eps):
    held = getattr(running_var, '_dsrl_invstd', None)
    if held is not None and held[1] == float(eps) and held[2] == running_var._version and held[0].device == running_var.device:
        return held[0]
    return None


def batch_norm_act(x, bn, relu=False, drop_p=0.0, seed=0, rng_stream=0, residual=None, residual_grad_slot=None, stats=None, out_link=None, res_link=None):
    training = bn.training or bn.running_mean is None
    if training and bn.running_mean is not None:
        bn._dsrl_batches = getattr(bn, '_dsrl_batches', 0) + 1
        if getattr(bn.running_var, '_dsrl_invstd', None) is not None:
            bn.running_var._dsrl_invstd = None
    momentum = 0.1 if bn.momentum is None else bn.momentum
    return _BNAct.apply(x, bn.weight, bn.bias, bn.running_mean, bn.running_var, training, momentum, bn.eps, relu,
                        drop_p if training or drop_p == 0.0 else 0.0, seed, rng_stream, residual, residual_grad_slot if residual is not None else None,
                        stats[0] if (stats is not None and training) else None, stats[1] if (stats is not None and training) else 0,
                        out_link if bn_bwd_stats_enabled else None, res_link if (bn_bwd_stats_enabled and residual is not None) else None)


conv_bn_stats_enabled = knob('DSRL_CONV_BN_STATS', True)


def conv2d_bn_act(x, weight, bias, stride, padding, dilation, bn, relu=False, drop_p=0.0, seed=0, rng_stream=0, residual=None,
                  grad_slot=None, residual_grad_slot=None, in_link=None, out_link=None, res_link=None):
    training = bn.training or bn.running_mean is None
    K, C = weight.shape[0], x.shape[1]
    if conv_bn_stats_enabled and training and x.is_cuda and C % 4 == 0 and K % 32 == 0:
        N, _, H, W = x.shape
        parts = int(query('dsrl_conv2d_fwd_stats_parts', N, H, W, C, K, weight.shape[2], weight.shape[3], int(stride), int(padding), int(dilation)))
        if parts > 0:
            y, stats = _Conv2d.apply(x, weight, bias, int(stride), int(padding), int(dilation), grad_slot, parts, in_link)
            return batch_norm_act(y, bn, relu=relu, drop_p=drop_p, seed=seed, rng_stream=rng_stream, residual=residual,
                                  residual_grad_slot=residual_grad_slot, stats=(stats, parts), out_link=out_link, res_link=res_link)
    y = (_Conv2d.apply(x, weight, bias, int(stride), int(padding), int(dilation), grad_slot, 0, in_link)
         if (in_link is not None and x.is_cuda and C % 4 == 0) else conv2d(x, weight, bias, stride, padding, dilation, grad_slot=grad_slot))
    return batch_norm_act(y, bn, relu=relu, drop_p=drop_p, seed=seed, rng_stream=rng_stream, residual=residual,
                          residual_grad_slot=residual_grad_slot, out_link=out_link, res_link=res_link)


class _Dropout(torch.autograd.Function):
    @staticmethod
    def forward(ctx, x, p, seed, rng_stream):
        x, ldx = pm(x)
        N, Cc, H, W = x.shape
        y = new_cl((N, Cc, H, W), x)
        call('dsrl_dropout_fwd', x.data_ptr(), ldx, y.data_ptr(), Cc, N * H * W, Cc, float(p), int(seed), int(rng_stream), _stream())
        ctx.cfg = (float(p), int(seed), int(rng_stream))
        return y

    @staticmethod
    def backward(ctx, dy):
        p, seed, rng_stream = ctx.cfg
        dy, ld = pm(dy)
        N, Cc, H, W = dy.shape
        dx = new_cl((N, Cc, H, W), dy)
        call('dsrl_dropout_bwd', dy.data_ptr(), ld, dx.data_ptr(), Cc, N * H * W, Cc, p, seed, rng_stream, _stream())
        return dx, None, None, None


def dropout(x, p, training, seed, rng_stream):
# ... 721 lines not shown
```

include/dsrl_hip.h:

```cpp
#ifndef DSRL_HIP_H
#define DSRL_HIP_H

#include <stddef.h>
#include <stdint.h>

#ifdef __cplusplus
extern "C" {
#endif

#define DSRL_ABI_VERSION 1

#define DSRL_OK 0
#define DSRL_E_BADARG (-1)
#define DSRL_E_UNSUPPORTED (-2)
#define DSRL_E_WORKSPACE (-3)
#define DSRL_E_LAUNCH (-4)

typedef void* dsrl_stream_t;

int dsrl_version(void);
const char* dsrl_last_error(void);
int dsrl_device_check(int* cu_count);

size_t dsrl_conv2d_fwd_workspace_bytes(int N, int H, int W, int C, int K, int R, int S, int stride, int pad, int dil);
// ... 22 lines not shown
                              const float* bn_mean, const float* bn_invstd, int bn_relu, float* bstats, int stats_parts,
                              int accumulate , dsrl_stream_t stream);
int dsrl_conv2d_dgrad_accumulate(const float* dy, int lddy, const float* w, const float* wt , float* dx, int lddx,
                                 int N, int H, int W, int C, int K, int R, int S, int stride, int pad, int dil,
                                 void* ws, size_t ws_bytes, dsrl_stream_t stream);
size_t dsrl_conv2d_wgrad_workspace_bytes(int N, int H, int W, int C, int K, int R, int S, int stride, int pad, int dil);
int dsrl_conv2d_wgrad(const float* x, int ldx, const float* dy, int lddy, float* dw,
                      int N, int H, int W, int C, int K, int R, int S, int stride, int pad, int dil,
                      void* ws, size_t ws_bytes, dsrl_stream_t stream);
typedef struct dsrl_wgrad_problem {
    const float* x; const float* dy; float* dw;
    int32_t ldx, lddy, N, H, W, C, K, R, S, stride, pad, dil;
    const uint32_t* x_amax; const uint32_t* dy_amax;
} dsrl_wgrad_problem;
size_t dsrl_conv2d_wgrad_group_table_bytes(int n);
size_t dsrl_conv2d_wgrad_group_workspace_bytes(const dsrl_wgrad_problem* problems, int n);
int dsrl_conv2d_wgrad_group_plan(const dsrl_wgrad_problem* problems, int n, void* host_table, size_t table_bytes, const void* dev_table,
                                 void* ws, size_t ws_bytes);
int dsrl_conv2d_wgrad_group_launch(const void* host_table, const void* dev_table, dsrl_stream_t stream);
#define DSRL_AMAX_WORDS 256
int dsrl_amax(const float* x, int ld, int64_t P, int C, uint32_t* amax, dsrl_stream_t stream);
int dsrl_conv2d_fwd_amax(const float* x, int ldx, const uint32_t* x_amax, const float* w, const uint32_t* w_amax, const void* w_split ,
                         const float* bias , float* y, int ldy, int N, int H, int W, int C, int K, int R, int S, int stride, int pad, int dil,
                         void* ws, size_t ws_bytes, float* stats , int stats_parts, dsrl_stream_t stream);
int dsrl_conv2d_dgrad_amax(const float* dy, int lddy, const uint32_t* dy_amax, const float* w, const float* wt , const uint32_t* w_amax,
                           const void* wt_split , float* dx, int lddx, int N, int H, int W, int C, int K, int R, int S, int stride, int pad, int dil,
                           void* ws, size_t ws_bytes, const float* bn_x, int bn_ldx, const float* bn_y, int bn_ldy,
                           const float* bn_mean, const float* bn_invstd, int bn_relu, float* bstats , int stats_parts, int accumulate,
                           dsrl_stream_t stream);
size_t dsrl_planes_lo_offset(int64_t elems);
size_t dsrl_planes_bytes(int64_t elems, int nplanes);
int dsrl_split_planes(const float* x, int ld, int64_t P, int C, const uint32_t* amax, void* planes, int nplanes, dsrl_stream_t stream);
int dsrl_conv2d_filter_planes_batched(const int64_t* table, int n, int64_t total_tiles, dsrl_stream_t stream);
int dsrl_conv2d_fwd_planes(const float* x, int ldx, const uint32_t* x_amax, const void* x_planes , const float* w, const uint32_t* w_amax,
                           const void* w_split , const void* w_planes , const float* bias , float* y, int ldy,
                           int N, int H, int W, int C, int K, int R, int S, int stride, int pad, int dil,
                           void* ws, size_t ws_bytes, float* stats , int stats_parts, dsrl_stream_t stream);
int dsrl_conv2d_dgrad_planes(const float* dy, int lddy, const uint32_t* dy_amax, const void* dy_planes , const float* w, const float* wt ,
                             const uint32_t* w_amax, const void* wt_split , const void* wt_planes , float* dx, int lddx,
                             int N, int H, int W, int C, int K, int R, int S, int stride, int pad, int dil,
                             void* ws, size_t ws_bytes, const float* bn_x, int bn_ldx, const float* bn_y, int bn_ldy,
                             const float* bn_mean, const float* bn_invstd, int bn_relu, float* bstats , int stats_parts, int accumulate,
                             dsrl_stream_t stream);
int dsrl_conv2d_dgrad_planes_drop(const float* dy, int lddy, const uint32_t* dy_amax, const void* dy_planes , const float* w, const float* wt ,
                             const uint32_t* w_amax, const void* wt_split , const void* wt_planes , float* dx, int lddx,
                             int N, int H, int W, int C, int K, int R, int S, int stride, int pad, int dil,
                             void* ws, size_t ws_bytes, const float* bn_x, int bn_ldx, const float* bn_y, int bn_ldy,
                             const float* bn_mean, const float* bn_invstd, int bn_relu, float bn_drop_p, float* bstats , int stats_parts, int accumulate,
                             dsrl_stream_t stream);
int dsrl_conv2d_wgrad_amax(const float* x, int ldx, const uint32_t* x_amax, const float* dy, int lddy, const uint32_t* dy_amax, float* dw,
                           int N, int H, int W, int C, int K, int R, int S, int stride, int pad, int dil,
                           void* ws, size_t ws_bytes, dsrl_stream_t stream);
int dsrl_conv_precision(int mode);
int64_t dsrl_conv2d_inbounds_macs(int N, int H, int W, int C, int K, int R, int S, int stride, int pad, int dil);

size_t dsrl_conv2d_rowfold_fwd_workspace_bytes(int N, int H, int W, int Cfold, int K, int R, int stride, int Ho, int Wo);
int dsrl_conv2d_rowfold_fwd(const float* x, int ldx, const float* w, const float* bias , float* y, int ldy,
                            int N, int H, int W, int Cfold, int K, int R, int stride, int Ho, int Wo, int64_t algorithmic_macs,
                            void* ws, size_t ws_bytes, dsrl_stream_t stream);
size_t dsrl_conv2d_rowfold_wgrad_workspace_bytes(int N, int H, int W, int Cfold, int K, int R, int stride, int Ho, int Wo);
int dsrl_conv2d_rowfold_wgrad(const float* x, int ldx, const float* dy, int lddy, float* dw,
                              int N, int H, int W, int Cfold, int K, int R, int stride, int Ho, int Wo, int64_t algorithmic_macs,
                              void* ws, size_t ws_bytes, dsrl_stream_t stream);
int dsrl_pad_image_nhwc(const float* x, int64_t sn, int64_t sc, int64_t sh, int64_t sw, float* y,
                        int N, int C, int H, int W, int Cp, int top, int left, int Hp, int Wp, dsrl_stream_t stream);

size_t dsrl_colsum_workspace_bytes(int64_t P, int C);
int dsrl_colsum(const float* x, int ld, int64_t P, int C, float* out, void* ws, size_t ws_bytes, dsrl_stream_t stream);

size_t dsrl_bn_workspace_bytes(int64_t P, int C);
int dsrl_bn_stats(const float* x, int ldx, int64_t P, int C, float eps, float momentum,
                  float* mean, float* invstd, float* running_mean , float* running_var ,
                  void* ws, size_t ws_bytes, dsrl_stream_t stream);
int dsrl_bn_invstd_from_var(const float* running_var, int C, float eps, float* invstd, dsrl_stream_t stream);
int dsrl_bn_apply(const float* x, int ldx, float* y, int ldy, int64_t P, int C,
                  const float* mean, const float* invstd, const float* gamma, const float* beta,
                  const float* residual , int ldr, int relu, float drop_p, uint64_t seed, uint32_t rng_stream,
                  uint32_t* y_amax , dsrl_stream_t stream);
size_t dsrl_bn_stats_floats(int rows, int parts, int C);
int dsrl_bn_train_fwd_from_stats(const float* x, int ldx, float* y, int ldy, int64_t P, int C, float eps, float momentum, float* mean, float* invstd,
                                 float* running_mean , float* running_var , const float* gamma, const float* beta,
                                 const float* residual , int ldr, int relu, float drop_p, uint64_t seed, uint32_t rng_stream,
                                 float* stats, int stats_parts, uint32_t* y_amax , dsrl_stream_t stream);
int dsrl_bn_fused_max_blocks(int max_blocks);
int dsrl_bn_fused_barrier_timeouts(int64_t* count);
int dsrl_bn_train_fwd(const float* x, int ldx, float* y, int ldy, int64_t P, int C, float eps, float momentum, float* mean, float* invstd,
                      float* running_mean , float* running_var , const float* gamma, const float* beta,
                      const float* residual , int ldr, int relu, float drop_p, uint64_t seed, uint32_t rng_stream,
                      void* ws, size_t ws_bytes, uint32_t* y_amax , dsrl_stream_t stream);
int dsrl_bn_bwd(const float* x, int ldx, const float* y, int ldy, const float* dy, int lddy,
                float* dx, int lddx, float* dresidual , int lddr, int64_t P, int C,
                const float* mean, const float* invstd, const float* gamma,
                float* dgamma, float* dbeta, int relu, float drop_p, int training,
                void* ws, size_t ws_bytes, uint32_t* dx_amax , dsrl_stream_t stream);
int dsrl_bn_bwd_from_stats(const float* x, int ldx, const float* y , int ldy, const float* dy, int lddy, float* dx, int lddx,
                           float* dresidual , int lddr, int64_t P, int C, const float* mean, const float* invstd, const float* gamma,
                           float* dgamma , float* dbeta , int relu, int training, float* stats, int stats_parts,
                           uint32_t* dx_amax , dsrl_stream_t stream);
int dsrl_bn_bwd_from_stats_drop(const float* x, int ldx, const float* y , int ldy, const float* dy, int lddy, float* dx, int lddx,
                           float* dresidual , int lddr, int64_t P, int C, const float* mean, const float* invstd, const float* gamma,
                           float* dgamma , float* dbeta , int relu, float drop_p, int training, float* stats, int stats_parts,
                           uint32_t* dx_amax , dsrl_stream_t stream);
int dsrl_bn_bwd_from_stats_res_parts(int64_t P, int C, int stats_parts);
int dsrl_bn_bwd_from_stats_res(const float* x, int ldx, const float* y , int ldy, const float* dy, int lddy, float* dx, int lddx,
                           float* dresidual, int lddr, int64_t P, int C, const float* mean, const float* invstd, const float* gamma,
                           float* dgamma , float* dbeta , int relu, float drop_p, int training, float* stats, int stats_parts,
                           uint32_t* dx_amax , const float* res_x, int res_ldx, const float* res_mean, const float* res_invstd,
                           float* res_stats, int res_parts, dsrl_stream_t stream);

int dsrl_rng_bind_device_key(const uint64_t* dev_key );
int dsrl_rng_advance_key(uint64_t* state , dsrl_stream_t stream);

int dsrl_dropout_fwd(const float* x, int ldx, float* y, int ldy, int64_t P, int C, float p, uint64_t seed, uint32_t rng_stream, dsrl_stream_t stream);
int dsrl_dropout_bwd(const float* dy, int lddy, float* dx, int lddx, int64_t P, int C, float p, uint64_t seed, uint32_t rng_stream, dsrl_stream_t stream);

int dsrl_bilinear_ac_fwd(const float* x, int ldx, float* y, int ldy, int N, int H, int W, int C, int Ho, int Wo, dsrl_stream_t stream);
size_t dsrl_bilinear_ac_bwd_workspace_bytes(int N, int H, int W, int C, int Ho, int Wo);
int dsrl_bilinear_ac_bwd(const float* dy, int lddy, float* dx, int lddx, int N, int H, int W, int C, int Ho, int Wo,
                         void* ws, size_t ws_bytes, dsrl_stream_t stream);
int dsrl_global_avgpool_fwd(const float* x, int ldx, float* y, int N, int HW, int C, dsrl_stream_t stream);
int dsrl_global_avgpool_bwd(const float* dy, float* dx, int lddx, int N, int HW, int C, dsrl_stream_t stream);
int dsrl_maxpool3x3s2_fwd(const float* x, float* y, uint8_t* argmax, int N, int H, int W, int C, dsrl_stream_t stream);
int dsrl_maxpool3x3s2_bwd(const uint8_t* argmax, const float* dy, float* dx, int N, int H, int W, int C, dsrl_stream_t stream);

int dsrl_convt2x2_fwd(const float* x, const float* w, const float* bias , float* y, int N, int H, int W, int Cin, int Cout, dsrl_stream_t stream);
size_t dsrl_convt2x2_bwd_workspace_bytes(int N, int H, int W, int Cin, int Cout);
int dsrl_convt2x2_bwd(const float* x, const float* w, const float* dy, float* dx, float* dw, float* dbias ,
                      int N, int H, int W, int Cin, int Cout, void* ws, size_t ws_bytes, dsrl_stream_t stream);

int dsrl_convt2x2_fwd_ce_supported(const float* x, const float* y, int N, int H, int W, int Cin, int Cout);
size_t dsrl_convt2x2_fwd_ce_workspace_bytes(int N, int H, int W);
int dsrl_convt2x2_fwd_ce(const float* x, const float* w, const float* bias , float* y, int N, int H, int W, int Cin, int Cout,
                         const uint8_t* target, int ignore_index, float* loss_out, int* nan_flag , void* ws, size_t ws_bytes, dsrl_stream_t stream);

int dsrl_convt2x2_bwd_ce_supported(const float* x, const float* logits, const uint8_t* target, int N, int H, int W, int Cin, int Cout);
int dsrl_convt2x2_bwd_ce(const float* x, const float* w, const float* logits, const uint8_t* target, int ignore_index, const float* ce_count,
                         const float* ft_g , const float* ft_w , int ft_stride, float* dx, float* dw, float* dbias ,
                         int N, int H, int W, int Cin, int Cout, void* ws, size_t ws_bytes, dsrl_stream_t stream);

int dsrl_pixel_shuffle_fwd(const float* x, float* y, int N, int H, int W, int c, int r, dsrl_stream_t stream);
int dsrl_pixel_shuffle_bwd(const float* dy, float* dx, int N, int H, int W, int c, int r, dsrl_stream_t stream);

int dsrl_pointwise_strided_fwd(const float* x, const float* w, float* y, int N, int H, int W, int C, int stride, dsrl_stream_t stream);
size_t dsrl_pointwise_strided_bwd_workspace_bytes(int N, int H, int W, int C, int stride);
int dsrl_pointwise_strided_bwd(const float* x, const float* w, const float* dy, float* dx, float* dw, int accumulate,
                               int N, int H, int W, int C, int stride, void* ws, size_t ws_bytes, dsrl_stream_t stream);

int dsrl_copy2d(const float* src, int ld_src, float* dst, int ld_dst, int64_t P, int C, dsrl_stream_t stream);
int dsrl_cat_channels_supported(const float* const* srcs, const int* lds, const int* cs, int n, const float* dst, int ld_dst, int64_t P);
int dsrl_cat_channels(const float* const* srcs, const int* lds, const int* cs, int n, float* dst, int ld_dst, int64_t P, uint32_t* amax, dsrl_stream_t stream);

int dsrl_nchw_to_nhwc(const float* x, float* y, int N, int C, int H, int W, int Cpad, dsrl_stream_t stream);

size_t dsrl_ce_workspace_bytes(int64_t P);
int dsrl_ce_fwd(const float* logits, int ld, const uint8_t* target, int64_t P, int C, int ignore_index,
                float* loss_out, void* ws, size_t ws_bytes, dsrl_stream_t stream);
int dsrl_ce_bwd(const float* logits, int ld, const uint8_t* target, int64_t P, int C, int ignore_index,
                const float* loss_out, const float* grad_out, float* dlogits, int lddl, dsrl_stream_t stream);
size_t dsrl_mse_workspace_bytes(int64_t n);
int dsrl_mse_fwd(const float* a, const float* b, int64_t n, float* loss_out, void* ws, size_t ws_bytes, dsrl_stream_t stream);
int dsrl_mse_bwd(const float* a, const float* b, int64_t n, const float* grad_out, float* da, dsrl_stream_t stream);
size_t dsrl_ce_fused_workspace_bytes(int64_t P);
int dsrl_ce_fused(const float* logits, int ld, const uint8_t* target, int64_t P, int C, int ignore_index, float* dlogits , int lddl,
                  float* loss_out , int* nan_flag , void* ws, size_t ws_bytes, dsrl_stream_t stream);
int dsrl_mse_fused(const float* a, const float* b, int64_t n, float grad_scale, float* da , float* loss_out, int* nan_flag ,
                   void* ws, size_t ws_bytes, dsrl_stream_t stream);
// ... 62 lines not shown
```

Measured before the change: 486.0 images/s.

## Store ReLU sign bitmask in BN forward and read it in backward

```diff
diff --git a/dualsuperreslearningforsemseg_amd/_lib.py b/dualsuperreslearningforsemseg_amd/_lib.py
--- a/dualsuperreslearningforsemseg_amd/_lib.py
+++ b/dualsuperreslearningforsemseg_amd/_lib.py
@@ -76,6 +76,8 @@
     'dsrl_bn_fused_max_blocks': (i32, [i32]),
     'dsrl_bn_fused_barrier_timeouts': (i32, [C.POINTER(i64)]),
     'dsrl_bn_train_fwd_from_stats': (i32, [fp, i32, fp, i32, i64, i32, f32, f32, fp, fp, fp, fp, fp, fp, fp, i32, i32, f32, u64, u32, fp, i32, fp, stream_t]),
+    'dsrl_bn_mask_words': (sz, [i64, i32]),
+    'dsrl_bn_train_fwd_from_stats_mask': (i32, [fp, i32, fp, i32, i64, i32, f32, f32, fp, fp, fp, fp, fp, fp, fp, i32, i32, f32, u64, u32, fp, i32, fp, fp, stream_t]),
     'dsrl_bn_train_fwd': (i32, [fp, i32, fp, i32, i64, i32, f32, f32, fp, fp, fp, fp, fp, fp, fp, i32, i32, f32, u64, u32, fp, sz, fp, stream_t]),
     'dsrl_bn_bwd': (i32, [fp, i32, fp, i32, fp, i32, fp, i32, fp, i32, i64, i32, fp, fp, fp, fp, fp, i32, f32, i32, fp, sz, fp, stream_t]),
     'dsrl_bn_bwd_from_stats': (i32, [fp, i32, fp, i32, fp, i32, fp, i32, fp, i32, i64, i32, fp, fp, fp, fp, fp, i32, i32, fp, i32, fp, stream_t]),
diff --git a/dualsuperreslearningforsemseg_amd/csrc/bn.hip b/dualsuperreslearningforsemseg_amd/csrc/bn.hip
--- a/dualsuperreslearningforsemseg_amd/csrc/bn.hip
+++ b/dualsuperreslearningforsemseg_amd/csrc/bn.hip
@@ -719,13 +719,14 @@
 
 
 constexpr int kMergeRows = 4;
-template <int THREADS>
+template <int THREADS, bool MASK = false>
 __global__ __launch_bounds__(THREADS) void bn_stats_apply_kernel(const float* __restrict__ x, int ldx, float* __restrict__ y, int ldy, int P, int C,
                                                               int groups, int rows_per_slab, float eps, float momentum,
                                                               float* __restrict__ mean_out, float* __restrict__ invstd_out, float* __restrict__ rm, float* __restrict__ rv,
                                                               const float* __restrict__ gamma, const float* __restrict__ beta,
                                                               const float* __restrict__ res, int ldr, int relu, float drop_p, SeedArg seed_arg, unsigned rng_stream,
-                                                              const float* __restrict__ part, int nparts, unsigned* __restrict__ y_amax) {
+                                                              const float* __restrict__ part, int nparts, unsigned* __restrict__ y_amax,
+                                                              unsigned* __restrict__ mask) {
     const unsigned long long seed = seed_arg.dev ? *seed_arg.dev : seed_arg.value;
     constexpr int KG = THREADS / 32, RP = THREADS / 8;
     __shared__ double shm[KG][3][32];
@@ -817,10 +818,37 @@
         }
         ST4(y, p, ldy, q) = make_float4(v[0], v[1], v[2], v[3]);
         am = abs_bits4(am, v[0], v[1], v[2], v[3]);
+        if constexpr (MASK) {
+            unsigned w = ((v[0] > 0.f ? 1u : 0u) | (v[1] > 0.f ? 2u : 0u) | (v[2] > 0.f ? 4u : 0u) | (v[3] > 0.f ? 8u : 0u)) << (4 * l8);
+            w |= __shfl_xor(w, 1); w |= __shfl_xor(w, 2); w |= __shfl_xor(w, 4);
+            if (l8 == 0) mask[(long long)grp * P + p] = w;
+        }
     };
     if (p0 < row1) row(p0, xv0, rv0);
+    if constexpr (!MASK) {
 #pragma unroll 4
-    for (int p = p0 + RP; p < row1; p += RP) {
+        for (int p = p0 + RP; p < row1; p += RP) {
+            const float4 xv = LD4(x, p, ldx, q);
+            float4 r = xv;
+            if (res) r = LD4(res, p, ldr, q);
+            row(p, xv, r);
+        }
+        amax_publish(am, y_amax);
+        return;
+    }
+    int p = p0 + RP;
+    for (; p + 3 * RP < row1; p += 4 * RP) {
+        float4 xv[4], r[4];
+#pragma unroll
+        for (int u = 0; u < 4; ++u) {
+            xv[u] = LD4(x, p + u * RP, ldx, q);
+            r[u] = xv[u];
+            if (res) r[u] = LD4(res, p + u * RP, ldr, q);
+        }
+#pragma unroll
+        for (int u = 0; u < 4; ++u) row(p + u * RP, xv[u], r[u]);
+    }
+    for (; p < row1; p += RP) {
         const float4 xv = LD4(x, p, ldx, q);
         float4 r = xv;
         if (res) r = LD4(res, p, ldr, q);
@@ -912,9 +940,15 @@
     const int q = grp * 8 + l8;
     const int row0 = slab * rows_per_slab, row1 = min(P, row0 + rows_per_slab), p0 = row0 + rr;
     float4 dv0 = make_float4(0.f, 0.f, 0.f, 0.f), xv0 = dv0, yv0 = make_float4(1.f, 1.f, 1.f, 1.f), x2v0 = dv0;
+    const unsigned* __restrict__ mrow = reinterpret_cast<const unsigned*>(y) + (relu == 2 ? (long long)grp * ldy : 0ll);
+    auto mask_row = [&](int p) {
+        const unsigned w = mrow[p] >> (4 * l8);
+        return make_float4((w & 1u) ? 1.f : 0.f, (w & 2u) ? 1.f : 0.f, (w & 4u) ? 1.f : 0.f, (w & 8u) ? 1.f : 0.f);
+    };
     if (p0 < row1) {
         dv0 = LD4(dy, p0, lddy, q); xv0 = LD4(x, p0, ldx, q);
-        if (relu) yv0 = LD4(y, p0, ldy, q);
+        if (relu == 2) yv0 = mask_row(p0);
+        else if (relu) yv0 = LD4(y, p0, ldy, q);
         if constexpr (RES2) x2v0 = LD4(r2.x, p0, r2.ldx, q);
     }
     float mu2[4] = {0.f, 0.f, 0.f, 0.f}, is2[4] = {0.f, 0.f, 0.f, 0.f}, sg2[4] = {0.f, 0.f, 0.f, 0.f}, sgx2[4] = {0.f, 0.f, 0.f, 0.f};
@@ -994,7 +1028,8 @@
     for (int p = p0 + RP; p < row1; p += RP) {
         const float4 dv = LD4(dy, p, lddy, q), xv = LD4(x, p, ldx, q);
         float4 yv = make_float4(1.f, 1.f, 1.f, 1.f);
-        if (relu) yv = LD4(y, p, ldy, q);
+        if (relu == 2) yv = mask_row(p);
+        else if (relu) yv = LD4(y, p, ldy, q);
         float4 x2v = xv;
         if constexpr (RES2) x2v = LD4(r2.x, p, r2.ldx, q);
         row(p, dv, xv, yv, x2v);
@@ -1359,10 +1394,20 @@
     return dsrl_bn_apply(x, ldx, y, ldy, P, C, mean, invstd, gamma, beta, residual, ldr, relu, drop_p, seed, rng_stream, y_amax, stream);
 }
 
+extern "C" size_t dsrl_bn_mask_words(int64_t P, int C) { return (P > 0 && C > 0 && C % 32 == 0) ? (size_t)(C / 32) * (size_t)P : 0; }
+
 extern "C" int dsrl_bn_train_fwd_from_stats(const float* x, int ldx, float* y, int ldy, int64_t P, int C, float eps, float momentum, float* mean, float* invstd,
                                             float* running_mean, float* running_var, const float* gamma, const float* beta, const float* residual, int ldr,
                                             int relu, float drop_p, uint64_t seed, uint32_t rng_stream, float* stats, int stats_parts, uint32_t* y_amax,
                                             dsrl_stream_t stream) {
+    return dsrl_bn_train_fwd_from_stats_mask(x, ldx, y, ldy, P, C, eps, momentum, mean, invstd, running_mean, running_var, gamma, beta, residual, ldr, relu, drop_p, seed,
+                                             rng_stream, stats, stats_parts, y_amax, nullptr, stream);
+}
+extern "C" int dsrl_bn_train_fwd_from_stats_mask(const float* x, int ldx, float* y, int ldy, int64_t P, int C, float eps, float momentum, float* mean, float* invstd,
+                                                 float* running_mean, float* running_var, const float* gamma, const float* beta, const float* residual, int ldr,
+                                                 int relu, float drop_p, uint64_t seed, uint32_t rng_stream, float* stats, int stats_parts, uint32_t* y_amax,
+                                                 uint32_t* mask, dsrl_stream_t stream) {
+    DSRL_REQUIRE(((uintptr_t)mask % 4) == 0, DSRL_E_BADARG, "bn_train_fwd_from_stats: unaligned mask");
     DSRL_REQUIRE(x && y && mean && invstd && gamma && beta && stats && P > 0 && P < (1ll << 31) && C > 0 && ldx >= C && ldy >= C, DSRL_E_BADARG, "bn_train_fwd_from_stats: bad arguments");
     DSRL_REQUIRE(stats_parts > 0 && stats_parts <= 4096, DSRL_E_BADARG, "bn_train_fwd_from_stats: %d row blocks of partials (1..4096)", stats_parts);
     DSRL_REQUIRE(C % 32 == 0 && vec4_ok(C, {ldx, ldy, residual ? ldr : 0}, {x, y, residual}), DSRL_E_UNSUPPORTED,
@@ -1380,9 +1425,11 @@
     const int T = stats_apply_threads(P, C, stats_parts), rows_per_slab = stats_apply_rows(P, groups, T), slabs = (int)ceil_div(P, (int64_t)rows_per_slab);
     auto go = [&](auto kern) {
         hipLaunchKernelGGL(kern, dim3((unsigned)(groups * slabs)), dim3(T), 0, st, x, ldx, y, ldy, (int)P, C, groups, rows_per_slab, eps, momentum,
-                           mean, invstd, running_mean, running_var, gamma, beta, residual, ldr, relu, drop_p, seed_arg(seed), (unsigned)rng_stream, stats, stats_parts, y_amax);
+                           mean, invstd, running_mean, running_var, gamma, beta, residual, ldr, relu, drop_p, seed_arg(seed), (unsigned)rng_stream, stats, stats_parts, y_amax,
+                           (unsigned*)mask);
     };
-    if (T == 1024) go(bn_stats_apply_kernel<1024>); else if (T == 512) go(bn_stats_apply_kernel<512>); else go(bn_stats_apply_kernel<256>);
+    if (mask) { if (T == 1024) go(bn_stats_apply_kernel<1024, true>); else if (T == 512) go(bn_stats_apply_kernel<512, true>); else go(bn_stats_apply_kernel<256, true>); }
+    else if (T == 1024) go(bn_stats_apply_kernel<1024>); else if (T == 512) go(bn_stats_apply_kernel<512>); else go(bn_stats_apply_kernel<256>);
     return launch_status("bn_stats_apply_kernel");
 }
 
@@ -1474,7 +1521,10 @@
     DSRL_REQUIRE(x && dy && dx && mean && invstd && gamma && stats && P > 0 && P < (1ll << 31) && C > 0, DSRL_E_BADARG, "bn_bwd_from_stats: bad arguments");
     DSRL_REQUIRE(y || !relu, DSRL_E_BADARG, "bn_bwd_from_stats: forward output needed for the relu mask");
     DSRL_REQUIRE(stats_parts > 0 && stats_parts <= 4096, DSRL_E_BADARG, "bn_bwd_from_stats: %d row blocks of partials (1..4096)", stats_parts);
-    DSRL_REQUIRE(C % 32 == 0 && vec4_ok(C, {ldx, y ? ldy : 0, lddy, lddx, dresidual ? lddr : 0}, {x, y, dy, dx, dresidual}), DSRL_E_UNSUPPORTED,
+    const bool bits = relu == 2;
+    DSRL_REQUIRE(relu == 0 || relu == 1 || bits, DSRL_E_BADARG, "bn_bwd_from_stats: relu = %d (0, 1, or 2 = y is the sign mask)", relu);
+    DSRL_REQUIRE(!bits || (ldy >= P && ((uintptr_t)y % 4) == 0), DSRL_E_BADARG, "bn_bwd_from_stats: sign mask with rows of %d words for %lld pixels, or unaligned", ldy, (long long)P);
+    DSRL_REQUIRE(C % 32 == 0 && vec4_ok(C, {ldx, (y && !bits) ? ldy : 0, lddy, lddx, dresidual ? lddr : 0}, {x, bits ? nullptr : y, dy, dx, dresidual}), DSRL_E_UNSUPPORTED,
                  "bn_bwd_from_stats: C (%d) must be a multiple of 32, strides multiples of 4, pointers 16-byte aligned", C);
     hipStream_t st = (hipStream_t)stream;
     if (int e = bind_stream_device(st)) return e;
diff --git a/dualsuperreslearningforsemseg_amd/csrc/conv_common.h b/dualsuperreslearningforsemseg_amd/csrc/conv_common.h
--- a/dualsuperreslearningforsemseg_amd/csrc/conv_common.h
+++ b/dualsuperreslearningforsemseg_amd/csrc/conv_common.h
@@ -82,6 +82,11 @@
     return (n * a.Ho + hh * a.par + ph) * a.Wo + wh * a.par + pw;
 }
 
+__device__ __forceinline__ unsigned bn_mask_word(const ConvArgs& a, int k, long long px) {
+    return reinterpret_cast<const unsigned*>(a.bn_y)[(long long)(k >> 5) * a.bn_ldy + px];
+}
+__device__ __forceinline__ float4 bn_mask4(unsigned w) { return make_float4((w & 1u) ? 1.f : 0.f, (w & 2u) ? 1.f : 0.f, (w & 4u) ? 1.f : 0.f, (w & 8u) ? 1.f : 0.f); }
+
 __device__ inline int xcd_contiguous(int bid, int n) {
     const int q = n / kNumXCD, r = n % kNumXCD, xcd = bid % kNumXCD, local = bid / kNumXCD;
     return (xcd < r ? xcd * (q + 1) : r * (q + 1) + (xcd - r) * q) + local;
diff --git a/dualsuperreslearningforsemseg_amd/csrc/conv_igemm.hip b/dualsuperreslearningforsemseg_amd/csrc/conv_igemm.hip
--- a/dualsuperreslearningforsemseg_amd/csrc/conv_igemm.hip
+++ b/dualsuperreslearningforsemseg_amd/csrc/conv_igemm.hip
@@ -1492,6 +1492,10 @@
 }
 
 struct DgradBn { const float* x; const float* y; const float* mean; const float* invstd; float* stats; int ldx, ldy, relu; float gscale = 1.f; };
+static bool bn_y_ok(const float* y, int ldy, int relu, int N, int H, int W, int C) {
+    if (relu == 2) return y != nullptr && C % 32 == 0 && (long long)ldy >= (long long)N * H * W && ((uintptr_t)y % 4) == 0;
+    return relu == 0 || (relu == 1 && y != nullptr && ldy >= C);
+}
 static int dgrad_impl(const float* dy, int lddy, const float* w, const float* wt_in, float* dx, int lddx,
                       int N, int H, int W, int C, int K, int R, int S, int stride, int pad, int dil,
                       void* ws, size_t ws_bytes, dsrl_stream_t stream, int accumulate, const DgradBn* bn = nullptr,
@@ -1569,7 +1573,8 @@
     if (bn) {
         a.bn_x = bn->x; a.bn_y = bn->y; a.bn_mean = bn->mean; a.bn_invstd = bn->invstd; a.bstats = bn->stats; a.bn_ldx = bn->ldx; a.bn_ldy = bn->ldy; a.bn_relu = bn->relu;
         a.bn_gscale = bn->gscale;
-        a.bn_fast = a.par == 0 && C % 4 == 0 && bn->ldx % 4 == 0 && (!bn->relu || bn->ldy % 4 == 0) && ((uintptr_t)bn->x % 16) == 0 && (!bn->relu || ((uintptr_t)bn->y % 16) == 0) &&
+        const bool y4 = bn->relu != 1 || (bn->ldy % 4 == 0 && ((uintptr_t)bn->y % 16) == 0);
+        a.bn_fast = a.par == 0 && C % 4 == 0 && bn->ldx % 4 == 0 && y4 && ((uintptr_t)bn->x % 16) == 0 &&
                     ((uintptr_t)bn->mean % 16) == 0 && ((uintptr_t)bn->invstd % 16) == 0 && ((uintptr_t)bn->stats % 16) == 0;
     }
     return launch_igemm<true>(a, p.cfg, st);
@@ -1591,7 +1596,7 @@
                                          void* ws, size_t ws_bytes, const float* bn_x, int bn_ldx, const float* bn_y, int bn_ldy,
                                          const float* bn_mean, const float* bn_invstd, int bn_relu, float* bstats, int stats_parts, int accumulate,
                                          dsrl_stream_t stream) {
-    DSRL_REQUIRE(bn_x && bn_mean && bn_invstd && bstats && (bn_y || !bn_relu) && bn_ldx >= C && (!bn_relu || bn_ldy >= C), DSRL_E_BADARG, "conv2d_dgrad_bnstats: bad BatchNorm arguments");
+    DSRL_REQUIRE(bn_x && bn_mean && bn_invstd && bstats && bn_ldx >= C && bn_y_ok(bn_y, bn_ldy, bn_relu, N, H, W, C), DSRL_E_BADARG, "conv2d_dgrad_bnstats: bad BatchNorm arguments");
     DSRL_REQUIRE(dsrl_conv2d_dgrad_stats_parts(N, H, W, C, K, R, S, stride, pad, dil) == stats_parts && stats_parts > 0, DSRL_E_BADARG,
                  "conv2d_dgrad_bnstats: this launch writes %d row blocks of partials, the caller expects %d",
                  dsrl_conv2d_dgrad_stats_parts(N, H, W, C, K, R, S, stride, pad, dil), stats_parts);
@@ -1787,7 +1792,7 @@
                                       dsrl_stream_t stream) {
     if (bstats == nullptr)
         return dgrad_impl(dy, lddy, w, wt_in, dx, lddx, N, H, W, C, K, R, S, stride, pad, dil, ws, ws_bytes, stream, accumulate ? 1 : 0, nullptr, dy_amax, w_amax, wt_split);
-    DSRL_REQUIRE(bn_x && bn_mean && bn_invstd && (bn_y || !bn_relu) && bn_ldx >= C && (!bn_relu || bn_ldy >= C), DSRL_E_BADARG, "conv2d_dgrad_amax: bad BatchNorm arguments");
+    DSRL_REQUIRE(bn_x && bn_mean && bn_invstd && bn_ldx >= C && bn_y_ok(bn_y, bn_ldy, bn_relu, N, H, W, C), DSRL_E_BADARG, "conv2d_dgrad_amax: bad BatchNorm arguments");
     DSRL_REQUIRE(dsrl_conv2d_dgrad_stats_parts(N, H, W, C, K, R, S, stride, pad, dil) == stats_parts && stats_parts > 0, DSRL_E_BADARG,
                  "conv2d_dgrad_amax: this launch writes %d row blocks of partials, the caller expects %d",
                  dsrl_conv2d_dgrad_stats_parts(N, H, W, C, K, R, S, stride, pad, dil), stats_parts);
@@ -1818,7 +1823,7 @@
     if (bstats == nullptr)
         return dgrad_impl(dy, lddy, w, wt_in, dx, lddx, N, H, W, C, K, R, S, stride, pad, dil, ws, ws_bytes, stream, accumulate ? 1 : 0, nullptr, dy_amax, w_amax, wt_split,
                           dy_planes, wt_planes);
-    DSRL_REQUIRE(bn_x && bn_mean && bn_invstd && (bn_y || !bn_relu) && bn_ldx >= C && (!bn_relu || bn_ldy >= C), DSRL_E_BADARG, "conv2d_dgrad_planes: bad BatchNorm arguments");
+    DSRL_REQUIRE(bn_x && bn_mean && bn_invstd && bn_ldx >= C && bn_y_ok(bn_y, bn_ldy, bn_relu, N, H, W, C), DSRL_E_BADARG, "conv2d_dgrad_planes: bad BatchNorm arguments");
     DSRL_REQUIRE(dsrl_conv2d_dgrad_stats_parts(N, H, W, C, K, R, S, stride, pad, dil) == stats_parts && stats_parts > 0, DSRL_E_BADARG,
                  "conv2d_dgrad_planes: this launch writes %d row blocks of partials, the caller expects %d",
                  dsrl_conv2d_dgrad_stats_parts(N, H, W, C, K, R, S, stride, pad, dil), stats_parts);
diff --git a/dualsuperreslearningforsemseg_amd/csrc/conv_planes.hip b/dualsuperreslearningforsemseg_amd/csrc/conv_planes.hip
--- a/dualsuperreslearningforsemseg_amd/csrc/conv_planes.hip
+++ b/dualsuperreslearningforsemseg_amd/csrc/conv_planes.hip
@@ -350,7 +350,8 @@
                     const int m = mrow0 + r0_ + RSTEP * (b0 + u);
                     const bool ok = kok4 && m < a.M;
                     xv[u] = ok ? *reinterpret_cast<const float4*>(a.bn_x + (long long)m * a.bn_ldx + kk) : make_float4(0.f, 0.f, 0.f, 0.f);
-                    yv[u] = (ok && a.bn_relu) ? *reinterpret_cast<const float4*>(a.bn_y + (long long)m * a.bn_ldy + kk) : make_float4(1.f, 1.f, 1.f, 1.f);
+                    if (a.bn_relu == 2) yv[u] = bn_mask4(ok ? bn_mask_word(a, kk, m) >> (kk & 31) : 15u);
+                    else yv[u] = (ok && a.bn_relu) ? *reinterpret_cast<const float4*>(a.bn_y + (long long)m * a.bn_ldy + kk) : make_float4(1.f, 1.f, 1.f, 1.f);
                 }
 #pragma unroll
                 for (int u = 0; u < NB; ++u) {
@@ -399,7 +400,8 @@
                     const bool ok = kok && m < a.M;
                     const long long px = m;
                     xv[e] = ok ? a.bn_x[px * a.bn_ldx + k] : 0.f;
-                    yv[e] = (ok && a.bn_relu) ? a.bn_y[px * a.bn_ldy + k] : 1.f;
+                    if (a.bn_relu == 2) yv[e] = (!ok || ((bn_mask_word(a, k, px) >> (k & 31)) & 1u)) ? 1.f : 0.f;
+                    else yv[e] = (ok && a.bn_relu) ? a.bn_y[px * a.bn_ldy + k] : 1.f;
                 }
 #pragma unroll
                 for (int e = 0; e < EPG; ++e) {
diff --git a/dualsuperreslearningforsemseg_amd/csrc/conv_split_kernel.h b/dualsuperreslearningforsemseg_amd/csrc/conv_split_kernel.h
--- a/dualsuperreslearningforsemseg_amd/csrc/conv_split_kernel.h
+++ b/dualsuperreslearningforsemseg_amd/csrc/conv_split_kernel.h
@@ -518,7 +518,8 @@
                     const int m = mrow0 + r0_ + RSTEP * (b0 + u);
                     const bool ok = kok4 && m < a.M;
                     xv[u] = ok ? *reinterpret_cast<const float4*>(a.bn_x + (long long)m * a.bn_ldx + kk) : make_float4(0.f, 0.f, 0.f, 0.f);
-                    yv[u] = (ok && a.bn_relu) ? *reinterpret_cast<const float4*>(a.bn_y + (long long)m * a.bn_ldy + kk) : make_float4(1.f, 1.f, 1.f, 1.f);
+                    if (a.bn_relu == 2) yv[u] = bn_mask4(ok ? bn_mask_word(a, kk, m) >> (kk & 31) : 15u);
+                    else yv[u] = (ok && a.bn_relu) ? *reinterpret_cast<const float4*>(a.bn_y + (long long)m * a.bn_ldy + kk) : make_float4(1.f, 1.f, 1.f, 1.f);
                 }
 #pragma unroll
                 for (int u = 0; u < NB; ++u) {
@@ -568,7 +569,8 @@
                     const bool ok = kok && m < a.M;
                     const long long px = pix0 + (m - mb32) * pst;
                     xv[e] = ok ? a.bn_x[px * a.bn_ldx + k] : 0.f;
-                    yv[e] = (ok && a.bn_relu) ? a.bn_y[px * a.bn_ldy + k] : 1.f;
+                    if (a.bn_relu == 2) yv[e] = (!ok || ((bn_mask_word(a, k, px) >> (k & 31)) & 1u)) ? 1.f : 0.f;
+                    else yv[e] = (ok && a.bn_relu) ? a.bn_y[px * a.bn_ldy + k] : 1.f;
                 }
 #pragma unroll
                 for (int e = 0; e < EPG; ++e) {
diff --git a/dualsuperreslearningforsemseg_amd/functional.py b/dualsuperreslearningforsemseg_amd/functional.py
--- a/dualsuperreslearningforsemseg_amd/functional.py
+++ b/dualsuperreslearningforsemseg_amd/functional.py
@@ -583,10 +583,11 @@
 
 bn_bwd_stats_enabled = knob('DSRL_BN_BWD_STATS', True)
 bn_bwd_stats_shared = knob('DSRL_BN_BWD_STATS_SHARED', True)
+bn_mask_enabled = knob('DSRL_BN_MASK', True)
 
 
 class BNLink:
-    __slots__ = ('x', 'y_ptr', 'y_shape', 'mean', 'invstd', 'relu', 'valid', 'stats', 'parts', 'dx_ptr', 'shared', 'drop_p')
+    __slots__ = ('x', 'y_ptr', 'y_shape', 'mean', 'invstd', 'relu', 'valid', 'stats', 'parts', 'dx_ptr', 'shared', 'drop_p', 'mask')
 
     def __init__(self, shared=False):
         self.x = self.mean = self.invstd = self.stats = None
@@ -594,6 +595,7 @@
         self.relu, self.valid, self.parts, self.dx_ptr = False, False, 0, 0
         self.shared = shared
         self.drop_p = 0.0
+        self.mask = None
 
 
 class _Fork(torch.autograd.Function):
@@ -728,8 +730,9 @@
             if parts > 0:
                 bstats = torch.empty(cquery('dsrl_bn_stats_floats', 2, parts, Cc), device=x.device, dtype=torch.float32)
                 _, bld = pm(link.x)
+                ym = (link.mask.data_ptr(), N * H * W, 2) if (link.mask is not None and link.relu) else (x.data_ptr(), ldx, int(link.relu))
                 call('dsrl_conv2d_dgrad_planes_drop', dy.data_ptr(), lddy, p_(dya), p_(dyp), w.data_ptr(), wt_ptr, p_(wa), p_(wtsp), p_(wtpl), dx.data_ptr(), Cc, *shp,
-                     ws.data_ptr(), ws.numel(), link.x.data_ptr(), bld, x.data_ptr(), ldx, link.mean.data_ptr(), link.invstd.data_ptr(), int(link.relu),
+                     ws.data_ptr(), ws.numel(), link.x.data_ptr(), bld, ym[0], ym[1], link.mean.data_ptr(), link.invstd.data_ptr(), ym[2],
                      float(link.drop_p), bstats.data_ptr(), parts, int(acc), st)
                 link.stats, link.parts, link.dx_ptr = bstats, parts, dx.data_ptr()
             else:
@@ -839,6 +842,7 @@
         if residual is not None:
             residual, ldr = pm(residual)
             res_ptr = residual.data_ptr()
+        mask = None
         if training:
             if P <= 1:
                 raise ValueError(f'Expected more than 1 value per channel when training, got input size {tuple(x.shape)}')
@@ -846,10 +850,13 @@
             mean = torch.empty(Cc, device=x.device, dtype=torch.float32)
             invstd = torch.empty_like(mean)
             if stats is not None and stats_parts > 0:
-                call('dsrl_bn_train_fwd_from_stats', x.data_ptr(), ldx, y.data_ptr(), Cc, P, Cc, float(eps), float(momentum), mean.data_ptr(), invstd.data_ptr(),
+                if relu and bn_mask_enabled and Cc % 32 == 0:
+                    mask = torch.empty(cquery('dsrl_bn_mask_words', P, Cc), device=x.device, dtype=torch.int32)
+                call('dsrl_bn_train_fwd_from_stats' if mask is None else 'dsrl_bn_train_fwd_from_stats_mask', x.data_ptr(), ldx, y.data_ptr(), Cc, P, Cc,
+                     float(eps), float(momentum), mean.data_ptr(), invstd.data_ptr(),
                      None if running_mean is None else running_mean.data_ptr(), None if running_var is None else running_var.data_ptr(),
                      gamma.data_ptr(), beta.data_ptr(), res_ptr, ldr, int(relu), float(drop_p), int(seed), int(rng_stream),
-                     stats.data_ptr(), int(stats_parts), ya_ptr, st)
+                     stats.data_ptr(), int(stats_parts), ya_ptr, *(() if mask is None else (mask.data_ptr(),)), st)
             else:
                 call('dsrl_bn_train_fwd', x.data_ptr(), ldx, y.data_ptr(), Cc, P, Cc, float(eps), float(momentum), mean.data_ptr(), invstd.data_ptr(),
                      None if running_mean is None else running_mean.data_ptr(), None if running_var is None else running_var.data_ptr(),
@@ -866,8 +873,10 @@
         if ya is not None:
             set_amax(y, ya)
         ctx.save_for_backward(x, y, mean, invstd, gamma)
+        ctx.mask = mask
         if out_link is not None and (drop_p == 0.0 or relu) and Cc % 32 == 0 and ldx == Cc:
             out_link.x, out_link.mean, out_link.invstd, out_link.relu, out_link.valid = x, mean, invstd, bool(relu), True
+            out_link.mask = mask
             out_link.y_ptr, out_link.y_shape, out_link.drop_p = y.data_ptr(), tuple(y.shape), float(drop_p)
         ctx.cfg = (bool(training), bool(relu), float(drop_p), residual is not None)
         ctx.gb = (gamma, beta) if isinstance(gamma, torch.nn.Parameter) and isinstance(beta, torch.nn.Parameter) else None
@@ -894,18 +903,19 @@
         link = ctx.out_link
         if link is not None and link.stats is not None and link.dx_ptr == dy.data_ptr() and lddy == Cc and (drop_p == 0.0 or relu):
             rl = ctx.res_link
+            ym = (ctx.mask.data_ptr(), P, 2) if (ctx.mask is not None and relu) else (y.data_ptr(), Cc, int(relu))
             rparts = int(query('dsrl_bn_bwd_from_stats_res_parts', P, Cc, int(link.parts))) if (rl is not None and dres is not None and bn_res_stats_enabled) else 0
             if rparts > 0:
                 rstats = torch.empty(cquery('dsrl_bn_stats_floats', 2, rparts, Cc), device=x.device, dtype=torch.float32)
                 _, rld = pm(rl.x)
-                call('dsrl_bn_bwd_from_stats_res', x.data_ptr(), ldx, y.data_ptr(), Cc, dy.data_ptr(), lddy, dx.data_ptr(), Cc, dres.data_ptr(), Cc, P, Cc,
-                     mean.data_ptr(), invstd.data_ptr(), gamma.data_ptr(), dgamma.data_ptr(), dbeta.data_ptr(), int(relu), float(drop_p), int(training),
+                call('dsrl_bn_bwd_from_stats_res', x.data_ptr(), ldx, ym[0], ym[1], dy.data_ptr(), lddy, dx.data_ptr(), Cc, dres.data_ptr(), Cc, P, Cc,
+                     mean.data_ptr(), invstd.data_ptr(), gamma.data_ptr(), dgamma.data_ptr(), dbeta.data_ptr(), ym[2], float(drop_p), int(training),
                      link.stats.data_ptr(), int(link.parts), dxa_ptr, rl.x.data_ptr(), rld, rl.mean.data_ptr(), rl.invstd.data_ptr(), rstats.data_ptr(), rparts, _stream())
                 rl.stats, rl.parts, rl.dx_ptr = rstats, rparts, dres.data_ptr()
             else:
-                call('dsrl_bn_bwd_from_stats_drop', x.data_ptr(), ldx, y.data_ptr(), Cc, dy.data_ptr(), lddy, dx.data_ptr(), Cc,
+                call('dsrl_bn_bwd_from_stats_drop', x.data_ptr(), ldx, ym[0], ym[1], dy.data_ptr(), lddy, dx.data_ptr(), Cc,
                      None if dres is None else dres.data_ptr(), Cc, P, Cc, mean.data_ptr(), invstd.data_ptr(), gamma.data_ptr(),
-                     dgamma.data_ptr(), dbeta.data_ptr(), int(relu), float(drop_p), int(training), link.stats.data_ptr(), int(link.parts), dxa_ptr, _stream())
+                     dgamma.data_ptr(), dbeta.data_ptr(), ym[2], float(drop_p), int(training), link.stats.data_ptr(), int(link.parts), dxa_ptr, _stream())
         else:
             ws = _ws(cquery('dsrl_bn_workspace_bytes', P, Cc), x)
             call('dsrl_bn_bwd', x.data_ptr(), ldx, y.data_ptr(), Cc, dy.data_ptr(), lddy, dx.data_ptr(), Cc,
diff --git a/include/dsrl_hip.h b/include/dsrl_hip.h
--- a/include/dsrl_hip.h
+++ b/include/dsrl_hip.h
@@ -128,6 +128,11 @@
                                  float* running_mean , float* running_var , const float* gamma, const float* beta,
                                  const float* residual , int ldr, int relu, float drop_p, uint64_t seed, uint32_t rng_stream,
                                  float* stats, int stats_parts, uint32_t* y_amax , dsrl_stream_t stream);
+size_t dsrl_bn_mask_words(int64_t P, int C);
+int dsrl_bn_train_fwd_from_stats_mask(const float* x, int ldx, float* y, int ldy, int64_t P, int C, float eps, float momentum, float* mean, float* invstd,
+                                      float* running_mean , float* running_var , const float* gamma, const float* beta,
+                                      const float* residual , int ldr, int relu, float drop_p, uint64_t seed, uint32_t rng_stream,
+                                      float* stats, int stats_parts, uint32_t* y_amax , uint32_t* mask , dsrl_stream_t stream);
 int dsrl_bn_fused_max_blocks(int max_blocks);
 int dsrl_bn_fused_barrier_timeouts(int64_t* count);
 int dsrl_bn_train_fwd(const float* x, int ldx, float* y, int ldy, int64_t P, int C, float eps, float momentum, float* mean, float* invstd,
```

After: 492.1 images/s (median of 6 runs). 1.2% higher.
